# MIMUW-RL/space-gym

Measured on AMD Instinct MI355X. Metric: env-steps/sec at batch=65536, GoalContinuous3P-v0, 1/2/4/8 MI355X, higher is better.
Workload: dtype f32

## Files before the change

space_gym_amd/csrc/sg_device.hpp:

```cpp
#ifndef SG_DEVICE_HPP
#define SG_DEVICE_HPP

#include <math.h>
#include <stdint.h>

#include "sg_config.h"

#if defined(__HIPCC__)
#define SG_FN __device__ __forceinline__
#define SG_MFN __device__ __forceinline__
#else
#define SG_FN static inline
#define SG_MFN inline
#endif

#ifndef SG_STAMP
#define SG_STAMP(slot)
#endif

namespace sg {

#if defined(__HIP_DEVICE_COMPILE__)
SG_FN float rsq(float x) { return __builtin_amdgcn_rsqf(x); }
SG_FN float rcp(float x) { return __builtin_amdgcn_rcpf(x); }
SG_FN float fsqrt(float x) { return __builtin_amdgcn_sqrtf(x); }
SG_FN float flog2(float x) { return __builtin_amdgcn_logf(x); }
SG_FN float fexp2(float x) { return __builtin_amdgcn_exp2f(x); }
#else
SG_FN float rsq(float x) { return 1.0f / sqrtf(x); }
SG_FN float rcp(float x) { return 1.0f / x; }
SG_FN float fsqrt(float x) { return sqrtf(x); }
SG_FN float flog2(float x) { return log2f(x); }
SG_FN float fexp2(float x) { return exp2f(x); }
#endif

constexpr float kTwoPi = 6.283185307179586f;

SG_FN void sincos_poly(float r, float &s, float &c) {
    float z = r * r;
    float ps = fmaf(fmaf(-1.9515295891e-4f, z, 8.3321608736e-3f), z, -1.6666654611e-1f);
    s = fmaf(ps * z, r, r);
    float pc = fmaf(fmaf(2.443315711809948e-5f, z, -1.388731625493765e-3f), z, 4.166664568298827e-2f);
    c = fmaf(pc * z, z, fmaf(-0.5f, z, 1.0f));
}

SG_FN void sincos_small(float r, float &s, float &c) {
    float z = r * r;
    s = fmaf(r * z, fmaf(z, 8.295134641230106e-3f, -1.666649580001831e-1f), r);
    c = fmaf(z, fmaf(z, fmaf(z, -1.3838880180093369e-3f, 4.166642666449376e-2f), -0.5f), 1.0f);
}

#if defined(__HIP_DEVICE_COMPILE__)
typedef float f2 __attribute__((ext_vector_type(2)));
SG_FN f2 mk2(float a, float b) { f2 r; r.x = a; r.y = b; return r; }
SG_FN f2 fma2(f2 a, f2 b, f2 c) { return __builtin_elementwise_fma(a, b, c); }
#else
struct f2 { float x, y; };
SG_FN f2 mk2(float a, float b) { f2 r; r.x = a; r.y = b; return r; }
SG_FN f2 operator+(f2 a, f2 b) { return mk2(a.x + b.x, a.y + b.y); }
SG_FN f2 operator-(f2 a, f2 b) { return mk2(a.x - b.x, a.y - b.y); }
SG_FN f2 operator*(f2 a, f2 b) { return mk2(a.x * b.x, a.y * b.y); }
SG_FN f2 operator*(f2 a, float b) { return mk2(a.x * b, a.y * b); }
SG_FN f2 operator*(float a, f2 b) { return mk2(a * b.x, a * b.y); }
SG_FN f2 fma2(f2 a, f2 b, f2 c) { return mk2(fmaf(a.x, b.x, c.x), fmaf(a.y, b.y, c.y)); }
#endif
SG_FN f2 sp2(float a) { return mk2(a, a); }
SG_FN f2 fma2(float a, f2 b, f2 c) { return fma2(sp2(a), b, c); }
SG_FN f2 fma2(f2 a, float b, f2 c) { return fma2(a, sp2(b), c); }
SG_FN f2 fma2(f2 a, float b, float c) { return fma2(a, sp2(b), sp2(c)); }
SG_FN f2 fma2(f2 a, f2 b, float c) { return fma2(a, b, sp2(c)); }

SG_FN void sincos_small2(f2 r, f2 &s, f2 &c) {
    f2 z = r * r;
    s = fma2(r * z, fma2(z, 8.295134641230106e-3f, -1.666649580001831e-1f), r);
    c = fma2(z, fma2(z, fma2(z, -1.3838880180093369e-3f, 4.166642666449376e-2f), -0.5f), 1.0f);
}

SG_FN void sincos_acc(float a, float &s, float &c) {
    float k = rintf(a * 0.6366197723675814f);
    float r = fmaf(-k, 1.57079637050628662109375f, a);
    r = fmaf(-k, -4.37113900018624283e-8f, r);
    float sr, cr;
    sincos_poly(r, sr, cr);
    int q = (int)k & 3;
    float s1 = (q & 1) ? cr : sr, c1 = (q & 1) ? sr : cr;
    s = (q & 2) ? -s1 : s1;
    c = ((q + 1) & 2) ? -c1 : c1;
}

SG_FN float wrap_two_pi(float th) {
    th = th - kTwoPi * floorf(th * (1.0f / kTwoPi));
    th = (th < 0.0f) ? th + kTwoPi : th;
    return (th >= kTwoPi) ? th - kTwoPi : th;
}

SG_FN double rsqrt_f64(double x) {
    double y = (double)rsq((float)x);
    return y * (1.5 - 0.5 * x * y * y);
}

constexpr float C2 = 1.0f / 5, C3 = 3.0f / 10, C4 = 4.0f / 5, C5 = 8.0f / 9;
constexpr float A21 = 1.0f / 5;
constexpr float A31 = 3.0f / 40, A32 = 9.0f / 40;
constexpr float A41 = 44.0f / 45, A42 = -56.0f / 15, A43 = 32.0f / 9;
constexpr float A51 = 19372.0f / 6561, A52 = -25360.0f / 2187, A53 = 64448.0f / 6561, A54 = -212.0f / 729;
constexpr float A61 = 9017.0f / 3168, A62 = -355.0f / 33, A63 = 46732.0f / 5247, A64 = 49.0f / 176,
                A65 = -5103.0f / 18656;
constexpr float B1 = 35.0f / 384, B3 = 500.0f / 1113, B4 = 125.0f / 192, B5 = -2187.0f / 6784, B6 = 11.0f / 84;
constexpr float BETA1 = 35.0f / 384, BETA3 = 50.0f / 159, BETA4 = 25.0f / 192, BETA5 = -243.0f / 6784;
constexpr float E3 = 71.0f / 16695, E4 = -71.0f / 1920, E5 = 17253.0f / 339200, E6 = -22.0f / 525, E7 = 1.0f / 40;
constexpr float P31 = (float)(131558114200.0 / 32700410799.0), P32 = (float)(-68118460800.0 / 10900136933.0),
                P33 = (float)(87487479700.0 / 32700410799.0);
constexpr float P41 = (float)(-1754552775.0 / 470086768.0), P42 = (float)(14199869525.0 / 1410260304.0),
                P43 = (float)(-10690763975.0 / 1880347072.0);
constexpr float P51 = (float)(127303824393.0 / 49829197408.0), P52 = (float)(-318862633887.0 / 49829197408.0),
                P53 = (float)(701980252875.0 / 199316789632.0);
constexpr float P61 = (float)(-282668133.0 / 205662961.0), P62 = (float)(2019193451.0 / 616988883.0),
                P63 = (float)(-1453857185.0 / 822651844.0);
constexpr float P71 = (float)(40617522.0 / 29380423.0), P72 = (float)(-110615467.0 / 29380423.0),
                P73 = (float)(69997945.0 / 29380423.0);
constexpr float kRtol = 1e-3f, kAtol = 1e-6f;
constexpr float kSafety = 0.9f, kMinFactor = 0.2f, kMaxFactor = 10.0f;
#ifndef SG_PROBE_NORM
#define SG_PROBE_NORM 1e-3f
#endif
constexpr float kProbeNorm = SG_PROBE_NORM;
#ifndef SG_PROBE_POS_ERR
#define SG_PROBE_POS_ERR 2e-8f
#endif
constexpr float kProbePosErr = SG_PROBE_POS_ERR;
#ifndef SG_PROBE_POS_ERR_KEPLER
#define SG_PROBE_POS_ERR_KEPLER 1e-6f
#endif
constexpr float kProbePosErrKepler = SG_PROBE_POS_ERR_KEPLER;
constexpr float N5_C2 = 1.0f / 5, N5_C3 = 2.0f / 3;
constexpr float N5_A21 = 1.0f / 50, N5_A31 = -1.0f / 27, N5_A32 = 7.0f / 27;
constexpr float N5_BB1 = 14.0f / 336, N5_BB2 = 100.0f / 336, N5_BB3 = 54.0f / 336;
constexpr float N5_B1 = 14.0f / 336, N5_B2 = 125.0f / 336, N5_B3 = 162.0f / 336, N5_B4 = 35.0f / 336;
constexpr float N5_D1 = (float)(3.0 / 10 - 14.0 / 336), N5_D2 = (float)(-2.0 / 35 - 100.0 / 336), N5_D3 = (float)(9.0 / 35 - 54.0 / 336);
#ifndef SG_FAST_IND
#define SG_FAST_IND 1.5e-6f
#endif
constexpr float kFastInd = SG_FAST_IND;
#ifndef SG_FAST_IND_KEPLER
#define SG_FAST_IND_KEPLER 1e-5f
#endif
constexpr float kFastIndKepler = SG_FAST_IND_KEPLER;
#ifndef SG_FAST_IND_CROSS
#define SG_FAST_IND_CROSS 3e-5f
#endif
constexpr float kFastIndCross = SG_FAST_IND_CROSS;
constexpr float kFastCrossDepth = 1e-5f;
constexpr int kMaxRkAttempts = 12;
constexpr int kRootIters = 2;
constexpr int kRootMaxIters = 28;

struct StepResult {
    double dXd, dYd;
    float dX, dY;
    float vx, vy;
    float t;
    float dth, om;
    int done;
    int event;
    int n_rk;
    int path;
    float probe_err;
    float probe_ep, probe_ev;
};
enum : int { kPathProbe = 0, kPathProbeTerminal = 1, kPathScipyErr = 2, kPathScipyClear = 3, kPathScipy = 4 };

template <bool SMALL>
SG_FN f2 thrust_at(f2 T, f2 Tp, float delta) {
    float sd, cd;
    if (SMALL) sincos_small(delta, sd, cd); else sincos_poly(delta, sd, cd);
    return fma2(T, sp2(cd), Tp * sd);
}
template <int NG>
SG_FN f2 pull(f2 c0, f2 c1, f2 c2, f2 c3, f2 p, float (&r2)[NG > 0 ? NG : 1]) {
    static_assert(NG <= 4, "at most four gravitating circles");
    f2 s = mk2(0.0f, 0.0f);
    if (NG >= 2) {
        const f2 da = c0 - p, db = c1 - p;
        const float ra = fmaf(da.x, da.x, da.y * da.y), rb = fmaf(db.x, db.x, db.y * db.y);
        r2[0] = ra; r2[NG >= 2 ? 1 : 0] = rb;
        const f2 i = mk2(rsq(ra), rsq(rb));
        const f2 w = i * i * i;
        s = fma2(db, sp2(w.y), da * w.x);
    }
    if (NG == 4) {
        const f2 da = c2 - p, db = c3 - p;
        const float ra = fmaf(da.x, da.x, da.y * da.y), rb = fmaf(db.x, db.x, db.y * db.y);
        r2[NG == 4 ? 2 : 0] = ra; r2[NG == 4 ? 3 : 0] = rb;
        const f2 i = mk2(rsq(ra), rsq(rb));
        const f2 w = i * i * i;
        s = fma2(db, sp2(w.y), fma2(da, sp2(w.x), s));
    }
    if (NG & 1) {
        const f2 dc = (NG == 1 ? c0 : c2) - p;
        const float rc = fmaf(dc.x, dc.x, dc.y * dc.y), ic = rsq(rc);
        r2[NG - 1] = rc;
        const float w = ic * ic * ic;
        s = (NG == 1) ? dc * w : fma2(dc, sp2(w), s);
    }
    return s;
}

enum : int { kRkContinue = 0, kRkFinished = 1, kRkEvent = 2, kRkEventDeferred = 3 };

template <int NC, int NG, bool WALLS, bool ACCEL = false>
struct Integrator {
    float t_end, half_world, gm, F, om, alpha, w_limit, x0, y0, nCF, nSF;
    float cax[NC], cay[NC], cR[NC], cR2[NC];
    f2 cq0, cq1, cq2, cq3;
    SG_MFN f2 cq_at(int k) const { return k == 0 ? cq0 : k == 1 ? cq1 : k == 2 ? cq2 : cq3; }
    double cRd[NC];
    float wxp, wyp, wxm, wym;
    float t, X, Y, vx, vy, h_abs;
    double Xd, Yd;
    float k0[4], g[NC + 2];
    f2 gp0;
    bool rejected, probe;
    bool fast;
    bool probe_crossing;
    float th0;
    int n_rk, attempts, path;
    float probe_err, probe_ep, probe_ev;

    struct EventCase {
        float h, t, X, Y, vx, vy, Xn, Yn;
        double Xd, Yd;
        float k0[4], k2[4], k3[4], k4[4], k5[4], k6[4];
        unsigned mask;
        float s_w;
        int n_rk;
        static constexpr int kWords = 8 + 4 + 24 + 3;
    };

    SG_MFN float phase(float tt) const { return ACCEL ? fmaf(om, tt, 0.5f * alpha * tt * tt) : om * tt; }

    SG_MFN void set_constants(float h_total, float half_world_, float gm_, float F_, float om_, float alpha_, float w_limit_,
                              float x0_, float y0_, const float (&cax_)[NC], const float (&cay_)[NC], const float (&cR_)[NC],
                              const double (&cRd_)[NC]) {
        half_world = half_world_; gm = gm_; F = F_; om = om_; alpha = ACCEL ? alpha_ : 0.0f; w_limit = w_limit_;
        x0 = x0_; y0 = y0_;
#pragma unroll
        for (int k = 0; k < NC; k++) { cax[k] = cax_[k]; cay[k] = cay_[k]; cR[k] = cR_[k]; cR2[k] = cR_[k] * cR_[k]; cRd[k] = cRd_[k]; }
        t_end = h_total;
        {
            float rx[4] = {0.0f, 0.0f, 0.0f, 0.0f}, ry[4] = {0.0f, 0.0f, 0.0f, 0.0f};
#pragma unroll
            for (int k = 0; k < NC; k++) {
                rx[k] = cax_[k]; ry[k] = cay_[k];
#if defined(__HIP_DEVICE_COMPILE__)
                asm volatile("" : "+v"(rx[k]), "+v"(ry[k]));
#endif
            }
            const f2 o = mk2(x0, y0);
            cq0 = mk2(rx[0], ry[0]) - o; cq1 = mk2(rx[1], ry[1]) - o; cq2 = mk2(rx[2], ry[2]) - o; cq3 = mk2(rx[3], ry[3]) - o;
        }
        wxp = half_world - x0; wyp = half_world - y0; wxm = half_world + x0; wym = half_world + y0;
    }

    SG_MFN void begin(float h_total, float half_world_, float gm_, float F_, float om_, float alpha_, float w_limit_,
                      float x0_, float y0_, float th0_, float vx0, float vy0, const float (&cax_)[NC],
                      const float (&cay_)[NC], const float (&cR_)[NC], const double (&cRd_)[NC], bool use_probe = true) {
        SG_STAMP(8);
        set_constants(h_total, half_world_, gm_, F_, om_, alpha_, w_limit_, x0_, y0_, cax_, cay_, cR_, cRd_);
        {
            float S0, C0;
            sincos_acc(th0_, S0, C0);
            nCF = -(C0 * F); nSF = -(S0 * F);
        }
        t = 0.0f; X = 0.0f; Y = 0.0f; vx = vx0; vy = vy0;
        Xd = 0.0; Yd = 0.0;
        const f2 T = mk2(nCF, nSF);

        float r2s[NG > 0 ? NG : 1];
        f2 origin = mk2(0.0f, 0.0f);
#if defined(__HIP_DEVICE_COMPILE__)
        asm volatile("" : "+v"(origin));
#endif
        gp0 = pull<NG>(cq0, cq1, cq2, cq3, origin, r2s);
        const f2 a0 = fma2(gm, gp0, T);
        k0[0] = vx; k0[1] = vy; k0[2] = a0.x; k0[3] = a0.y;
        th0 = th0_;
        probe = kProbeNorm > 0.0f && use_probe;
        fast = !ACCEL && probe;
        probe_crossing = false;
        path = kPathScipy; probe_err = probe_ep = probe_ev = 0.0f;
        if (probe) h_abs = t_end; else initial_step();

        SG_STAMP(9);
    #pragma unroll
        for (int k = 0; k < NG; k++) g[k] = r2s[k] - cR2[k];
    #pragma unroll
        for (int k = NG; k < NC; k++) { const f2 c = cq_at(k); g[k] = fmaf(c.x, c.x, c.y * c.y) - cR2[k]; }
        if (WALLS) { g[NC] = fminf(wxp, wyp); g[NC + 1] = fminf(wxm, wym); }

        rejected = false; n_rk = 0; attempts = 0;
    }

    SG_MFN void initial_step() {
        const f2 T = mk2(nCF, nSF), Tp = mk2(-nSF, nCF), V = mk2(k0[0], k0[1]), a0 = mk2(k0[2], k0[3]);
        const f2 is_p = mk2(rcp(fmaf(fabsf(x0), kRtol, kAtol)), rcp(fmaf(fabsf(y0), kRtol, kAtol)));
        const f2 is_v = mk2(rcp(fmaf(fabsf(V.x), kRtol, kAtol)), rcp(fmaf(fabsf(V.y), kRtol, kAtol)));
        const float isth = rcp(fmaf(fabsf(th0), kRtol, kAtol)), isom = rcp(fmaf(fabsf(om), kRtol, kAtol));
        const f2 y_p = mk2(x0, y0) * is_p, y_v = V * is_v;
        const float y_th = th0 * isth, y_om = om * isom;
        const f2 n0 = fma2(y_v, y_v, y_p * y_p);
        const float d0 = fsqrt(fmaf(y_om, y_om, fmaf(y_th, y_th, n0.x + n0.y)) * (1.0f / 6));
        const f2 f_p = V * is_p, f_v = a0 * is_v;
        const float f_th = om * isth, f_om = ACCEL ? alpha * isom : 0.0f;
        const f2 n1 = fma2(f_v, f_v, f_p * f_p);
        const float d1 = fsqrt(fmaf(f_om, f_om, fmaf(f_th, f_th, n1.x + n1.y)) * (1.0f / 6));
        float h0 = (fminf(d0, d1) < 1e-5f) ? 1e-6f : 0.01f * d0 * rcp(d1);
        h0 = fminf(h0, t_end);
        float r2p[NG > 0 ? NG : 1];
        const f2 a1 = fma2(gm, pull<NG>(cq0, cq1, cq2, cq3, V * h0, r2p), thrust_at<!ACCEL>(T, Tp, h0 * om));
        const f2 e_p = (a0 * h0) * is_p, e_v = (a1 - a0) * is_v;
        const float e_th = ACCEL ? h0 * alpha * isth : 0.0f;
        const f2 n2 = fma2(e_v, e_v, e_p * e_p);
        const float d2 = fsqrt(fmaf(e_th, e_th, n2.x + n2.y) * (1.0f / 6)) * rcp(h0);
        const float dm = fmaxf(d1, d2);
        const float h1 = (dm <= 1e-15f) ? fmaxf(1e-6f, h0 * 1e-3f)
                                        : fexp2(0.2f * flog2(0.01f * rcp(dm)));
        h_abs = fminf(fminf(100.0f * h0, h1), t_end);
    }

    SG_MFN bool no_graze(f2 V, f2 Vn, f2 Pn, float h, const float (&gn)[NC + 2]) const {
        const f2 vv0 = V * V, vv1 = Vn * Vn;
        const float v2max = fmaxf(vv0.x + vv0.y, vv1.x + vv1.y);
        const float ah = 1.2f * h * (F + 1.1f), chord = 0.3f * h * h * v2max;
        bool keep = true;
#pragma unroll
        for (int k = 0; k < NC; k++) {
            const f2 c = cq_at(k), cn = c - Pn;
            const float d0 = fmaf(c.x, V.x, c.y * V.y), d1 = fmaf(cn.x, Vn.x, cn.y * Vn.y);
            const bool mono = d0 * d1 > 0.0f && fabsf(d0 + d1) > fmaf(ah, cR[k], 1.2f * h * v2max);
            const float clear = fmaf(0.25f * h * ah, cR[k], g[k] > 0.0f ? chord : 0.0f);
            const bool near = fminf(fabsf(g[k]), fabsf(gn[k])) <= clear;
            keep = keep && !(near && !mono);
        }
        if (WALLS) {
            const f2 s = V + Vn;
            const float clear = 0.125f * h * ah;
            const bool mono_x = V.x * Vn.x > 0.0f && fabsf(s.x) > ah, mono_y = V.y * Vn.y > 0.0f && fabsf(s.y) > ah;
            const bool near_x = fminf(fminf(wxp, wxp - Pn.x), fminf(wxm, wxm + Pn.x)) <= clear;
            const bool near_y = fminf(fminf(wyp, wyp - Pn.y), fminf(wym, wym + Pn.y)) <= clear;
            keep = keep && !(near_x && !mono_x) && !(near_y && !mono_y);
        }
        return keep;
    }

    SG_MFN void nystrom5(float h, f2 P0, f2 V, f2 T, f2 Tp, f2 g1, f2 &rest, f2 &Vn, f2 &w) const {
        const float hh = h * h, hg = hh * gm;
        const float ph = om * h, z4 = ph * ph;
        const f2 ph23 = mk2(N5_C2, N5_C3) * ph, z23 = ph23 * ph23;
        const f2 A23 = fma2(z23, fma2(z23, 1.0f / 720, -1.0f / 24), 0.5f);
        const f2 B23 = ph23 * fma2(z23, fma2(z23, 1.0f / 5040, -1.0f / 120), 1.0f / 6);
        const float A4 = fmaf(z4, fmaf(z4, 1.0f / 720, -1.0f / 24), 0.5f);
        const float B4 = ph * fmaf(z4, fmaf(z4, 1.0f / 5040, -1.0f / 120), 1.0f / 6);
        const float S4 = fmaf(z4, fmaf(z4, fmaf(z4, -1.0f / 5040, 1.0f / 120), -1.0f / 6), 1.0f);
        const f2 p2 = fma2(T, sp2(A23.x), Tp * B23.x), p3 = fma2(T, sp2(A23.y), Tp * B23.y), p4 = fma2(T, sp2(A4), Tp * B4);
        float r2x[NG > 0 ? NG : 1];
        const f2 g2 = pull<NG>(cq0, cq1, cq2, cq3, fma2(hg * N5_A21, g1, fma2((N5_C2 * N5_C2) * hh, p2, fma2(N5_C2 * h, V, P0))), r2x);
        const f2 g3 = pull<NG>(cq0, cq1, cq2, cq3,
                               fma2(hg, fma2(N5_A32, g2, g1 * N5_A31), fma2((N5_C3 * N5_C3) * hh, p3, fma2(N5_C3 * h, V, P0))), r2x);
        rest = fma2(hg, fma2(N5_BB3, g3, fma2(N5_BB2, g2, g1 * N5_BB1)), p4 * hh);
        w = fma2(N5_D3, g3, fma2(N5_D2, g2, g1 * N5_D1)) * hg;
        const f2 g4 = pull<NG>(cq0, cq1, cq2, cq3, fma2(h, V, P0) + (rest + w), r2x);
        Vn = fma2(h * gm, fma2(N5_B4, g4, fma2(N5_B3, g3, fma2(N5_B2, g2, g1 * N5_B1))),
                  fma2(h, fma2(T, sp2(S4), Tp * (ph * A4)), V));
    }

    template <typename SINK>
    SG_MFN int fast_step(StepResult &o, SINK &&sink) {
        const float h = t_end;
        const f2 V = mk2(vx, vy), T = mk2(nCF, nSF), Tp = mk2(-nSF, nCF);
        f2 rest, Vn, w;
        f2 origin = mk2(0.0f, 0.0f);
#if defined(__HIP_DEVICE_COMPILE__)
        asm volatile("" : "+v"(origin));
#endif
        nystrom5(h, origin, V, T, Tp, gp0, rest, Vn, w);
        double Xdn = (double)h * (double)vx + (double)rest.x, Ydn = (double)h * (double)vy + (double)rest.y;
        float Xn = (float)Xdn, Yn = (float)Ydn;
        float ind2 = fmaf(w.x, w.x, w.y * w.y);

        float gn[NC + 2], ggmin, shallow;
        auto end_events = [&]() __attribute__((always_inline)) {
#pragma unroll
            for (int k = 0; k < NC; k++) {
                const f2 c = cq_at(k);
                const float ex = c.x - Xn, ey = c.y - Yn;
                gn[k] = fmaf(ex, ex, ey * ey) - cR2[k];
            }
            gn[NC] = gn[NC + 1] = 1.0f;
            if (WALLS) { gn[NC] = fminf(wxp - Xn, wyp - Yn); gn[NC + 1] = fminf(wxm + Xn, wym + Yn); }
            ggmin = 1.0f; shallow = 3.0e38f;
#pragma unroll
            for (int k = 0; k < NC + (WALLS ? 2 : 0); k++) {
                const float gg = g[k] * gn[k];
                ggmin = fminf(ggmin, gg);
                shallow = fminf(shallow, gg <= 0.0f ? fabsf(gn[k]) : 3.0e38f);
            }
        };
        end_events();
        const float lim = WALLS ? kFastInd : kFastIndKepler;
        probe_ev = 1.0f;
        if (!(ggmin <= 0.0f) && !(ind2 <= lim * lim)) {
            probe_ev = 2.0f;
            const float hs = 0.5f * h;
            f2 rA, VA, wA, rB, wB;
            nystrom5(hs, origin, V, T, Tp, gp0, rA, VA, wA);
            const double XdA = (double)hs * (double)vx + (double)rA.x, YdA = (double)hs * (double)vy + (double)rA.y;
            const f2 PA = mk2((float)XdA, (float)YdA);
            float sd, cd;
            sincos_small(om * hs, sd, cd);
            const f2 T1 = fma2(T, sp2(cd), Tp * sd), Tp1 = mk2(-T1.y, T1.x);
            float r2a[NG > 0 ? NG : 1];
            const f2 gA = pull<NG>(cq0, cq1, cq2, cq3, PA, r2a);
            nystrom5(hs, PA, VA, T1, Tp1, gA, rB, Vn, wB);
            Xdn = XdA + ((double)hs * (double)VA.x + (double)rB.x); Ydn = YdA + ((double)hs * (double)VA.y + (double)rB.y);
            Xn = (float)Xdn; Yn = (float)Ydn;
            ind2 = 16.0f * fmaxf(fmaf(wA.x, wA.x, wA.y * wA.y), fmaf(wB.x, wB.x, wB.y * wB.y));
            w = mk2(fmaxf(fabsf(wA.x), fabsf(wB.x)), fmaxf(fabsf(wA.y), fabsf(wB.y))) * 4.0f;
            end_events();
        }
        probe_err = ind2; probe_ep = fmaxf(fabsf(w.x), fabsf(w.y));

        const bool crossing = ggmin <= 0.0f;
        probe = false;
        if (!crossing) {
            if (!(ind2 <= lim * lim)) {
                path = kPathScipyErr;
                initial_step();
                return kRkContinue;
            }
            if (no_graze(V, Vn, mk2(Xn, Yn), h, gn)) {
                n_rk = 1; path = kPathProbe;
                t = t_end; X = Xn; Y = Yn; Xd = Xdn; Yd = Ydn; vx = Vn.x; vy = Vn.y;
                return kRkFinished;
            }
            path = kPathScipyClear;
        } else if (ind2 <= kFastIndCross * kFastIndCross && shallow >= kFastCrossDepth) {
            probe_crossing = true; path = kPathProbeTerminal;
            if (sink()) {
                o.dXd = 0.0; o.dYd = 0.0; o.dX = 0.0f; o.dY = 0.0f; o.vx = 0.0f; o.vy = 0.0f; o.t = t_end; o.dth = 0.0f; o.om = om;
                o.done = 1; o.event = -1; o.n_rk = 0; o.path = path;
                return kRkEventDeferred;
            }
        } else {
            path = kPathScipyErr;
        }
        initial_step();
        return kRkContinue;
    }

    struct NoSink { SG_MFN bool operator()() const { return false; } };
    template <typename SINK = NoSink>
    SG_MFN int attempt(StepResult &o, SINK &&sink = NoSink()) {
        const bool probing = probe;
        probe = false;
        attempts++;
        h_abs = fmaxf(h_abs, 1e-9f);
        float t_new = t + h_abs;
        if (t_new - t_end > 0.0f) t_new = t_end;
        const float h = t_new - t;
        h_abs = h;
        const f2 V = mk2(vx, vy), P = mk2(X, Y), a0 = mk2(k0[2], k0[3]);
        f2 th1, th2, th3, th4, th5;
        {
            const f2 T = mk2(nCF, nSF), Tp = mk2(-nSF, nCF);
            if (ACCEL) {
                th1 = thrust_at<false>(T, Tp, phase(fmaf(C2, h, t))); th2 = thrust_at<false>(T, Tp, phase(fmaf(C3, h, t)));
                th3 = thrust_at<false>(T, Tp, phase(fmaf(C4, h, t))); th4 = thrust_at<false>(T, Tp, phase(fmaf(C5, h, t)));
                th5 = thrust_at<false>(T, Tp, phase(t + h));
            } else {
                const float ph0 = om * t, phh = om * h;
                f2 s12, c12, s34, c34;
                sincos_small2(fma2(mk2(C2, C3), phh, ph0), s12, c12);
                sincos_small2(fma2(mk2(C4, C5), phh, ph0), s34, c34);
                th1 = fma2(T, sp2(c12.x), Tp * s12.x); th2 = fma2(T, sp2(c12.y), Tp * s12.y);
                th3 = fma2(T, sp2(c34.x), Tp * s34.x); th4 = fma2(T, sp2(c34.y), Tp * s34.y);
                th5 = thrust_at<true>(T, Tp, ph0 + phh);
            }
        }
        float r2x[NG > 0 ? NG : 1], r2n[NG > 0 ? NG : 1];
        const f2 sa1 = a0 * A21;
        const f2 v1 = fma2(h, sa1, V);
        const f2 g1 = pull<NG>(cq0, cq1, cq2, cq3, fma2(h, V * A21, P), r2x);
        const f2 g2 = pull<NG>(cq0, cq1, cq2, cq3, fma2(h, fma2(A32, v1, V * A31), P), r2x);
        const f2 a1 = fma2(gm, g1, th1), a2 = fma2(gm, g2, th2);
        const f2 sa2 = fma2(A32, a1, a0 * A31);
        const f2 v2 = fma2(h, sa2, V);
        const f2 sa3 = fma2(A43, a2, fma2(A42, a1, a0 * A41));
        const f2 v3 = fma2(h, sa3, V);
        const f2 g3 = pull<NG>(cq0, cq1, cq2, cq3, fma2(h, fma2(A43, v2, fma2(A42, v1, V * A41)), P), r2x);
        const f2 g4 = pull<NG>(cq0, cq1, cq2, cq3, fma2(h, fma2(A54, v3, fma2(A53, v2, fma2(A52, v1, V * A51))), P), r2x);
        const f2 a3 = fma2(gm, g3, th3), a4 = fma2(gm, g4, th4);
        const f2 sa4 = fma2(A54, a3, fma2(A53, a2, fma2(A52, a1, a0 * A51)));
        const f2 v4 = fma2(h, sa4, V);
        const f2 sa5 = fma2(A65, a4, fma2(A64, a3, fma2(A63, a2, fma2(A62, a1, a0 * A61))));
        const f2 v5 = fma2(h, sa5, V);
        const f2 nys = fma2(BETA5, a4, fma2(BETA4, a3, fma2(BETA3, a2, a0 * BETA1))) * (h * h);
        const double Xdn = Xd + ((double)h * (double)vx + (double)nys.x);
        const double Ydn = Yd + ((double)h * (double)vy + (double)nys.y);
        const float Xn = (float)Xdn, Yn = (float)Ydn;
        const f2 Pn = mk2(Xn, Yn);
        const f2 g5 = pull<NG>(cq0, cq1, cq2, cq3, fma2(h, fma2(A65, v4, fma2(A64, v3, fma2(A63, v2, fma2(A62, v1, V * A61)))), P), r2x);
        const f2 g6 = pull<NG>(cq0, cq1, cq2, cq3, Pn, r2n);
        const f2 a5 = fma2(gm, g5, th5), a6 = fma2(gm, g6, th5);
        const f2 sa6 = fma2(B6, a5, fma2(B5, a4, fma2(B4, a3, fma2(B3, a2, a0 * B1))));
        const f2 v6 = fma2(h, sa6, V);
        const float vxn = v6.x, vyn = v6.y;

        float err2, abs_ep, abs_ev;
        {
            const f2 e_p = fma2(E7, sa6, fma2(E6, sa5, fma2(E5, sa4, fma2(E4, sa3, sa2 * E3)))) * h;
            const f2 e_v = fma2(E7, a6 - a0, fma2(E6, a5 - a0, fma2(E5, a4 - a0, fma2(E4, a3 - a0, (a2 - a0) * E3))));
            const f2 p0 = mk2(x0, y0) + P, p1 = mk2(x0, y0) + Pn;
            const f2 sc_p = fma2(mk2(fmaxf(fabsf(p0.x), fabsf(p1.x)), fmaxf(fabsf(p0.y), fabsf(p1.y))), kRtol, kAtol);
            const f2 sc_v = fma2(mk2(fmaxf(fabsf(vx), fabsf(vxn)), fmaxf(fabsf(vy), fabsf(vyn))), kRtol, kAtol);
            const f2 q_p = (e_p * h) * mk2(rcp(sc_p.x), rcp(sc_p.y)), q_v = (e_v * h) * mk2(rcp(sc_v.x), rcp(sc_v.y));
            const f2 n = fma2(q_v, q_v, q_p * q_p);
            err2 = n.x + n.y;
            abs_ep = fmaxf(fabsf(e_p.x), fabsf(e_p.y)) * h; abs_ev = fmaxf(fabsf(e_v.x), fabsf(e_v.y)) * h;
        }
        const float err = err2 * (1.0f / 6);

        float gn[NC + 2], gg[NC + 2], ggmin = 1.0f;
        auto end_events = [&]() __attribute__((always_inline)) {
#pragma unroll
            for (int k = 0; k < NG; k++) gn[k] = r2n[k] - cR2[k];
#pragma unroll
            for (int k = NG; k < NC; k++) {
                const f2 c = cq_at(k);
                float ex = c.x - Xn, ey = c.y - Yn;
                gn[k] = fmaf(ex, ex, ey * ey) - cR2[k];
            }
            if (WALLS) { gn[NC] = fminf(wxp - Xn, wyp - Yn); gn[NC + 1] = fminf(wxm + Xn, wym + Yn); }
#pragma unroll
            for (int k = 0; k < NC + (WALLS ? 2 : 0); k++) { gg[k] = g[k] * gn[k]; ggmin = fminf(ggmin, gg[k]); }
        };
        end_events();
        float s_w = 2.0f;
        bool w_event = false;
        if constexpr (ACCEL) {
            const float w0 = fmaf(alpha, t, om), w1 = fmaf(alpha, t_new, om);
            const float gw0 = w_limit - fabsf(w0), gw1 = w_limit - fabsf(w1);
            if ((gw0 <= 0.0f && gw1 >= 0.0f) || (gw0 >= 0.0f && gw1 <= 0.0f)) {
                const float lim = (fabsf(w1) >= fabsf(w0) ? w1 : w0) >= 0.0f ? w_limit : -w_limit;
                const float dw = w1 - w0;
                s_w = (dw != 0.0f) ? fminf(fmaxf((lim - w0) * rcp(dw), 0.0f), 1.0f) : 0.0f;
                w_event = true;
            }
        }

        if (probing) {
            probe_err = err; probe_ep = abs_ep; probe_ev = abs_ev;
            const bool small = err <= kProbeNorm * kProbeNorm && abs_ep <= (WALLS ? kProbePosErr : kProbePosErrKepler);
            const bool crossing = ggmin <= 0.0f || w_event;
            if (small && !crossing) {
                if (no_graze(V, v6, Pn, h, gn)) {
                    n_rk = 1; path = kPathProbe;
                    t = t_new; X = Xn; Y = Yn; Xd = Xdn; Yd = Ydn; vx = vxn; vy = vyn;
                    return kRkFinished;
                }
                path = kPathScipyClear;
            } else if (small) {
                probe_crossing = true; path = kPathProbeTerminal;
                if (sink()) {
                    o.dXd = 0.0; o.dYd = 0.0; o.dX = 0.0f; o.dY = 0.0f; o.vx = 0.0f; o.vy = 0.0f; o.t = t_end; o.dth = 0.0f; o.om = om;
                    o.done = 1; o.event = -1; o.n_rk = 0; o.path = path;
                    return kRkEventDeferred;
// ... 285 lines not shown
    double ir = rsqrt_f64(rx * rx + py_ * py_);
    double v2 = c.k_gm * (2.0 * ir - ob.inv_a);
    double speed = v2 > 0 ? v2 * rsqrt_f64(v2) : 0.0;
    double it = rsqrt_f64(tx * tx + ty * ty);
    double ux = tx * it * speed, uy = ty * it * speed;
    double Vx = ob.cosphi * ux - ob.sinphi * uy, Vy = ob.sinphi * ux + ob.cosphi * uy;
    double rad_pen = fabs(cur_rad - target_rad);
    double vxp = fabs(Vx - (double)vx), vyp = fabs(Vy - (double)vy);
    float act = c.k_Ca * fsqrt(fmaf(engine, engine, thruster * thruster));
    return (float)(c.k_C / (c.k_Cr * rad_pen + vxp + vyp + (double)act + c.k_C));
}

SG_FN Orbit make_orbit(double a, double ecc, double cosphi, double sinphi) {
    Orbit ob;
    ob.a = a; ob.ecc = ecc; ob.cosphi = cosphi; ob.sinphi = sinphi;
    double b2 = a * a * (1.0 - ecc * ecc);
    ob.b = b2 * rsqrt_f64(b2);
    double c2 = a * a - b2;
    ob.c = c2 > 0 ? c2 * rsqrt_f64(c2) : 0.0;
    ob.a_over_b = a / ob.b; ob.b_over_a = ob.b / a; ob.inv_a = 1.0 / a;
    return ob;
}

SG_FN uint32_t mulhi32(uint32_t a, uint32_t b) {
#if defined(__HIP_DEVICE_COMPILE__)
    return __umulhi(a, b);
#else
    return (uint32_t)(((uint64_t)a * b) >> 32);
#endif
}

SG_FN void philox4x32_10(uint32_t k0, uint32_t k1, uint32_t c0, uint32_t c1, uint32_t c2, uint32_t c3, uint32_t (&out)[4]) {
#pragma unroll
    for (int r = 0; r < 10; r++) {
        uint32_t h0 = mulhi32(0xD2511F53u, c0), l0 = 0xD2511F53u * c0;
        uint32_t h1 = mulhi32(0xCD9E8D57u, c2), l1 = 0xCD9E8D57u * c2;
        c0 = h1 ^ c1 ^ k0; c1 = l1;
        c2 = h0 ^ c3 ^ k1; c3 = l0;
        k0 += 0x9E3779B9u; k1 += 0xBB67AE85u;
    }
    out[0] = c0; out[1] = c1; out[2] = c2; out[3] = c3;
}

constexpr uint32_t kStreamReset = 0u, kStreamGoal = 1u, kStreamAction = 2u;

constexpr int kGoalResetBlocks = 5, kKeplerResetBlocks = 3;

SG_FN float u23(uint32_t w) { return ((float)(w >> 9) + 0.5f) * (1.0f / 8388608.0f); }
SG_FN float u16(uint32_t h) { return ((float)(h & 0xffffu) + 0.5f) * (1.0f / 65536.0f); }
SG_FN uint32_t below16(uint32_t h, uint32_t n) { return ((h & 0xffffu) * n) >> 16; }

struct Tiling {
    uint32_t episode, goal_draws;
    uint32_t ship_tile, goal_tile, case_b, flip;
    uint64_t free_counts;
    float cs0, cs1, cs2, cs3;
};

SG_FN uint32_t free_total(uint64_t f) {
    uint64_t s = (f & 0x0f0f0f0f0f0f0f0full) + ((f >> 4) & 0x0f0f0f0f0f0f0f0full);
    return (uint32_t)((s * 0x0101010101010101ull) >> 56);
}
struct FreePrefix { uint64_t even, odd; };
SG_FN FreePrefix free_prefix(uint64_t f) {
    const uint64_t e = f & 0x0f0f0f0f0f0f0f0full, o = (f >> 4) & 0x0f0f0f0f0f0f0f0full;
    const uint64_t pe = e * 0x0101010101010101ull, po = o * 0x0101010101010101ull;
    FreePrefix p;
    p.even = pe + (po << 8);
    p.odd = pe + po;
    return p;
}
SG_FN uint32_t bytes_above(uint64_t x, uint32_t pos) {
    const uint64_t H = 0x8080808080808080ull, L = 0x0101010101010101ull;
    const uint64_t low_gt = (((x & ~H) + (uint64_t)(127u - (pos & 127u)) * L) & H);
    const uint64_t hi = x & H;
    const uint64_t gt = (pos < 128u) ? (hi | low_gt) : (hi & low_gt);
#if defined(__HIP_DEVICE_COMPILE__)
    return (uint32_t)__popcll(gt);
#else
    return (uint32_t)__builtin_popcountll(gt);
#endif
}
SG_FN uint32_t free_at(const FreePrefix &p, uint32_t pos) { return 16u - bytes_above(p.even, pos) - bytes_above(p.odd, pos); }
SG_FN uint64_t free_add(uint64_t f, uint32_t tile) {
    uint32_t cnt = (uint32_t)(f >> (4 * tile)) & 15u;
    return cnt < 15u ? f + (1ull << (4 * tile)) : f;
}
SG_FN uint64_t free_remove(uint64_t f, uint32_t tile) { return f - (1ull << (4 * tile)); }

SG_FN void tile_center(const SgDev &c, const Tiling &T, uint32_t tile, float &x, float &y) {
    uint32_t row = (tile * c.t_cols_rcp16) >> 16, col = tile - row * (uint32_t)c.t_cols;
    const float shift = (col == 1u) ? T.cs1 : (col == 2u) ? T.cs2 : (col == 3u) ? T.cs3 : T.cs0;
    float tx = c.t_x0 + (float)col * 1.5f * c.t_a + shift;
    float y0 = T.case_b ? c.t_y0 - 0.5f * c.t_hex_h : c.t_y0;
    float ycol = (col & 1u) ? 0.5f * c.t_hex_h : 0.0f;
    float ty = y0 - (float)row * c.t_hex_h + (T.case_b ? ycol : -ycol);
    x = T.flip ? ty : tx;
    y = T.flip ? tx : ty;
}

SG_FN void disc_in_tile(const SgDev &c, const Tiling &T, uint32_t tile, float noise_radius, uint32_t w, float &x, float &y) {
    float s, co;
    sincos_acc(kTwoPi * u16(w >> 16), s, co);
    float r = noise_radius * fsqrt(u16(w));
    tile_center(c, T, tile, x, y);
    x = fmaf(r, co, x);
    y = fmaf(r, s, y);
}

SG_FN void choose_goal_tile(const SgDev &c, Tiling &T, bool first, const uint32_t (&w)[4]) {
    if (!first) {
        T.free_counts = free_add(T.free_counts, T.ship_tile);
        T.ship_tile = T.goal_tile;
    }
    if ((w[0] & 0xffu) < 64u) {
        T.goal_tile = T.ship_tile;
    } else {
        const uint32_t n = free_total(T.free_counts), n_cand = n < 3u ? n : 3u;
        const uint32_t cols = (uint32_t)c.t_cols, sr = (T.ship_tile * c.t_cols_rcp16) >> 16, sc = T.ship_tile - sr * cols;
        const uint32_t draws[3] = {w[1] >> 16, w[1], w[2] >> 16};
        uint32_t chosen[3] = {0u, 0u, 0u};
        const uint32_t j0 = below16(draws[0], n);
        chosen[0] = j0;
        const uint32_t v1_old = (j0 == 1u) ? 0u : 1u;
        uint32_t j1 = 0xffffffffu;
        if (n_cand > 1) {
            j1 = 1u + below16(draws[1], n - 1u);
            chosen[1] = (j1 == j0) ? 0u : j1;
        }
        if (n_cand > 2) {
            const uint32_t j2 = 2u + below16(draws[2], n - 2u);
            chosen[2] = (j2 == j1) ? v1_old : (j2 == j0) ? 0u : j2;
        }
        uint32_t best_tile = 0;
        int best_dist = -1;
        const FreePrefix fp = free_prefix(T.free_counts);
#pragma unroll
        for (uint32_t i = 0; i < 3; i++) {
            if (i < n_cand) {
                uint32_t tile = free_at(fp, chosen[i]);
                uint32_t r = (tile * c.t_cols_rcp16) >> 16, cc = tile - r * cols;
                int dist = abs((int)r - (int)sr) + abs((int)cc - (int)sc);
                if (dist > best_dist) { best_dist = dist; best_tile = tile; }
            }
        }
        T.goal_tile = best_tile;
        T.free_counts = free_remove(T.free_counts, best_tile);
    }
}

SG_FN void choose_goal(const SgDev &c, Tiling &T, bool first, const uint32_t (&w)[4], float &gx, float &gy) {
    choose_goal_tile(c, T, first, w);
    disc_in_tile(c, T, T.goal_tile, c.noise_goal, w[3], gx, gy);
}

SG_FN void box_muller(uint32_t w1, uint32_t w2, float &z0, float &z1) {
    float r = fsqrt(-2.0f * 0.6931471805599453f * flog2(u23(w1)));
    float s, co;
    sincos_acc(kTwoPi * u23(w2), s, co);
    z0 = r * co;
    z1 = r * s;
}

struct ShipInit { float x, y, th, vx, vy, om; };

SG_FN void layout_from_words(const SgDev &c, uint32_t flags, uint32_t c01, uint32_t c23, Tiling &T) {
    T.case_b = flags & 1u; T.flip = (flags >> 1) & 1u;
    const float a0 = u16(c01 >> 16), a1 = a0 + u16(c01);
    const float a2 = (c.t_cols > 2) ? a1 + u16(c23 >> 16) : a1, a3 = (c.t_cols > 3) ? a2 + u16(c23) : a2;
    const float k = c.t_free_x * rcp(a3);
    T.cs0 = a0 * k; T.cs1 = a1 * k;
    T.cs2 = (c.t_cols > 2) ? a2 * k : 0.0f; T.cs3 = (c.t_cols > 3) ? a3 * k : 0.0f;
}

template <int N>
SG_FN void tiles_from_words(const SgDev &c, uint32_t flags, uint32_t t01, uint32_t t23, uint32_t t45, Tiling &T,
                            uint32_t (&tiles)[N + 1]) {
    const uint32_t draws[6] = {t01 >> 16, t01, t23 >> 16, t23, t45 >> 16, t45};
    uint64_t perm = 0xfedcba9876543210ull;
    const uint32_t nt = (uint32_t)c.t_tiles;
#pragma unroll
    for (uint32_t i = 0; i <= (uint32_t)N; i++) {
        uint32_t j = i + below16(draws[i], nt - i);
        uint64_t vi = (perm >> (4 * i)) & 15ull, vj = (perm >> (4 * j)) & 15ull;
        perm = (perm & ~((15ull << (4 * i)) | (15ull << (4 * j)))) | (vj << (4 * i)) | (vi << (4 * j));
        tiles[i] = (uint32_t)vj;
    }
    if (N == 2 && ((flags >> 8) & 0xffu) < 64u) {
        const uint32_t d = (flags >> 16) & 3u;
        tiles[0] = (d == 0) ? 1u : (d == 1) ? 2u : (d == 2) ? 0u : 3u;
        tiles[1] = (d < 2) ? 0u : 1u;
        tiles[2] = (d < 2) ? 3u : 2u;
    }
    uint64_t used = 0;
#pragma unroll
    for (int i = 0; i <= N; i++) used |= 1ull << (4 * tiles[i]);
    const uint64_t all = (nt >= 16u) ? 0x1111111111111111ull : (0x1111111111111111ull & ((1ull << (4 * nt)) - 1ull));
    T.free_counts = all & ~used;
    T.ship_tile = tiles[0];
}

SG_FN void kinematics_from_words(const SgDev &c, uint32_t wth, uint32_t b0, uint32_t b1, uint32_t b2, uint32_t b3, ShipInit &s) {
    s.th = kTwoPi * u23(wth);
    float z0, z1, z2, z3;
    box_muller(b0, b1, z0, z1);
    box_muller(b2, b3, z2, z3);
    s.vx = z0 * c.vel_std; s.vy = z1 * c.vel_std;
    s.om = fminf(fmaxf(z2 * c.omega_std, -c.omega_max), c.omega_max);
}

template <int N>
SG_FN void goal_reset(const SgDev &c, uint32_t env_global, Tiling &T, ShipInit &s, float (&px)[N], float (&py)[N],
                      float &gx, float &gy) {
    uint32_t w[4 * kGoalResetBlocks];
#pragma unroll
    for (uint32_t b = 0; b < (uint32_t)kGoalResetBlocks; b++) {
        uint32_t o[4];
        philox4x32_10(c.seed_lo, c.seed_hi, env_global, T.episode, b, kStreamReset, o);
        w[4 * b] = o[0]; w[4 * b + 1] = o[1]; w[4 * b + 2] = o[2]; w[4 * b + 3] = o[3];
    }
    T.goal_draws = 0;
    const uint32_t flags = w[0];
    layout_from_words(c, flags, w[1], w[2], T);
    uint32_t tiles[N + 1];
    tiles_from_words<N>(c, flags, w[3], w[4], w[5], T, tiles);
    disc_in_tile(c, T, tiles[0], c.noise_ship, w[8], s.x, s.y);
#pragma unroll
    for (int j = 0; j < N; j++) disc_in_tile(c, T, tiles[j + 1], c.noise_planet, w[9 + j], px[j], py[j]);
    const uint32_t gw[4] = {flags >> 24, w[6], w[7], w[13]};
    T.goal_tile = 0xffu;
    choose_goal(c, T, true, gw, gx, gy);
    kinematics_from_words(c, w[14], w[16], w[17], w[18], w[19], s);
}

SG_FN void goal_resample(const SgDev &c, uint32_t env_global, Tiling &T, float &gx, float &gy) {
    uint32_t w[4];
    T.goal_draws += 1;
    philox4x32_10(c.seed_lo, c.seed_hi, env_global, T.episode, T.goal_draws, kStreamGoal, w);
    choose_goal(c, T, false, w, gx, gy);
}

SG_FN void kepler_reset(const SgDev &c, uint32_t env_global, uint32_t episode, ShipInit &s, float &phi, float &ecc) {
    uint32_t w[4 * kKeplerResetBlocks];
#pragma unroll
    for (uint32_t b = 0; b < (uint32_t)kKeplerResetBlocks; b++) {
        uint32_t o[4];
        philox4x32_10(c.seed_lo, c.seed_hi, env_global, episode, b, kStreamReset, o);
        w[4 * b] = o[0]; w[4 * b + 1] = o[1]; w[4 * b + 2] = o[2]; w[4 * b + 3] = o[3];
    }
    float sa, ca;
    sincos_acc(kTwoPi * u23(w[0]), sa, ca);
    float dist = fmaf(c.kep_rmax - c.kep_rmin, u23(w[1]), c.kep_rmin);
    s.x = ca * dist; s.y = sa * dist;
    if (c.randomize_orbit) { ecc = u23(w[3]) * 0.7f; phi = u23(w[4]) * kTwoPi; }
    kinematics_from_words(c, w[2], w[8], w[9], w[10], w[11], s);
}

SG_FN void random_action_words(uint32_t seed_lo, uint32_t seed_hi, uint32_t env_global, uint64_t step, uint32_t &w0, uint32_t &w1) {
    uint32_t o[4];
    const uint64_t p = step >> 1;
    philox4x32_10(seed_lo, seed_hi, env_global, (uint32_t)p, (uint32_t)(p >> 32), kStreamAction, o);
    w0 = (step & 1u) ? o[2] : o[0];
    w1 = (step & 1u) ? o[3] : o[1];
}

template <int N>
struct GoalEnv {
    float x, y, th, vx, vy, om;
    float gx, gy;
    float px[N], py[N];
};
struct KeplerEnv {
    float x, y, th, vx, vy, om;
    float phi, ecc;
};

SG_FN void translate_action(float &a0, float &a1, float max_engine_force, float &engine, float &F, float &om) {
    a0 = fminf(fmaxf(a0, -1.0f), 1.0f);
    a1 = fminf(fmaxf(a1, -1.0f), 1.0f);
    engine = (a0 + 1.0f) * 0.5f;
    F = engine * max_engine_force;
    om = a1 * 5.0f;
}

template <bool ACCEL>
SG_FN void steering(const SgDev &c, float a1, float om_cmd, float om_state, float &om0, float &alpha) {
    if (ACCEL && c.steering_acceleration) { om0 = om_state; alpha = (a1 * c.max_thruster_force) * c.inv_moi; }
    else { om0 = om_cmd; alpha = 0.0f; }
}

SG_FN void load_action(bool discrete, const void *actions, int64_t idx, float &a0, float &a1) {
    if (discrete) {
        const int k = static_cast<const int32_t *>(actions)[idx];
        const bool engine = (k == 1) | (k == 4) | (k == 5);
        a0 = engine ? 1.0f : -1.0f;
        a1 = (k == 2 || k == 4) ? -1.0f : (k == 3 || k == 5) ? 1.0f : 0.0f;
    } else {
        const float *p = static_cast<const float *>(actions) + 2 * idx;
        a0 = p[0]; a1 = p[1];
    }
}

template <int N, typename CFG>
SG_FN void goal_observe(const CFG &c, const GoalEnv<N> &e, float (&obs)[7 + 2 * N + 2]) {
    float s, co;
    sincos_acc(e.th, s, co);
    obs[0] = e.x; obs[1] = e.y; obs[2] = co; obs[3] = s; obs[4] = e.vx; obs[5] = e.vy; obs[6] = e.om;
#pragma unroll
    for (int j = 0; j < N; j++) lidar(e.px[j] - e.x, e.py[j] - e.y, c.planet_r, c.two_over_world, obs[7 + 2 * j], obs[8 + 2 * j]);
    obs[7 + 2 * N] = (e.gx - e.x) * c.two_over_world;
    obs[8 + 2 * N] = (e.gy - e.y) * c.two_over_world;
}

template <typename CFG>
SG_FN void kepler_observe(const CFG &c, const KeplerEnv &e, float (&obs)[10]) {
    float s, co;
    sincos_acc(e.th, s, co);
    obs[0] = e.x; obs[1] = e.y; obs[2] = co; obs[3] = s; obs[4] = e.vx; obs[5] = e.vy; obs[6] = e.om;
    obs[7] = c.randomize_orbit ? e.phi : (float)c.k_phi;
    obs[8] = c.randomize_orbit ? e.ecc : (float)c.k_ecc;
    obs[9] = (float)c.k_a;
}

template <int N, bool ACCEL = false>
SG_FN void goal_env_begin(const SgDev &c, const GoalEnv<N> &e, float a0, float a1, Integrator<N, N, true, ACCEL> &I,
                          bool use_probe = true) {
    float engine, F, om, om0, alpha;
    translate_action(a0, a1, c.max_engine_force, engine, F, om);
    steering<ACCEL>(c, a1, om, e.om, om0, alpha);
    float cR[N];
    double cRd[N];
#pragma unroll
    for (int j = 0; j < N; j++) { cR[j] = c.planet_r; cRd[j] = c.planet_r_d; }
    I.begin(c.h, c.half_world, c.gm, F, om0, alpha, c.omega_limit, e.x, e.y, e.th, e.vx, e.vy, e.px, e.py, cR, cRd, use_probe);
}

struct GoalStepConsts {
    double goal_r2, danger_r2, survival, goal_scale, safety_scale, sparse;
    float planet_r, two_over_world;
};
SG_FN GoalStepConsts goal_step_consts(const SgDev &c) {
    GoalStepConsts k;
    k.goal_r2 = c.goal_r2; k.danger_r2 = c.danger_r2; k.survival = c.survival; k.goal_scale = c.goal_scale;
    k.safety_scale = c.safety_scale; k.sparse = c.sparse; k.planet_r = c.planet_r; k.two_over_world = c.two_over_world;
    return k;
}

struct KeplerStepConsts {
    double k_gm, k_C, k_Cr, k_phi, k_ecc, k_a;
    float k_Ca;
    int32_t randomize_orbit;
};
SG_FN KeplerStepConsts kepler_step_consts(const SgDev &c) {
    KeplerStepConsts k;
    k.k_gm = c.k_gm; k.k_C = c.k_C; k.k_Cr = c.k_Cr; k.k_phi = c.k_phi; k.k_ecc = c.k_ecc; k.k_a = c.k_a; k.k_Ca = c.k_Ca;
    k.randomize_orbit = c.randomize_orbit;
    return k;
}

struct GoalRewardProfile {
    double danger_r2, survival, goal_scale, safety_scale, sparse;
};
struct KeplerRewardProfile {
    double k_C, k_Cr;
    float k_Ca;
};
struct GoalRewardView {
    double goal_r2, danger_r2, survival, goal_scale, safety_scale, sparse;
};
SG_FN GoalRewardView goal_reward_view(const SgDev &c, const GoalRewardProfile &p) {
    GoalRewardView v;
    v.goal_r2 = c.goal_r2; v.danger_r2 = p.danger_r2; v.survival = p.survival; v.goal_scale = p.goal_scale;
    v.safety_scale = p.safety_scale; v.sparse = p.sparse;
    return v;
}
struct KeplerRewardView {
    double k_gm, k_C, k_Cr;
    float k_Ca;
};
SG_FN KeplerRewardView kepler_reward_view(const SgDev &c, const KeplerRewardProfile &p) {
    KeplerRewardView v;
    v.k_gm = c.k_gm; v.k_C = p.k_C; v.k_Cr = p.k_Cr; v.k_Ca = p.k_Ca;
    return v;
}

struct StepConsts {
    float max_engine_force, h, half_world, gm, omega_limit, planet_r, max_thruster_force, inv_moi;
    double planet_r_d;
    int32_t steering_acceleration;
};
SG_FN StepConsts step_consts(const SgDev &c) {
    StepConsts k;
    k.max_engine_force = c.max_engine_force; k.h = c.h; k.half_world = c.half_world; k.gm = c.gm; k.omega_limit = c.omega_limit;
    k.planet_r = c.planet_r; k.max_thruster_force = c.max_thruster_force; k.inv_moi = c.inv_moi; k.planet_r_d = c.planet_r_d;
    k.steering_acceleration = c.steering_acceleration;
    return k;
}
template <int N, bool ACCEL = false>
SG_FN void goal_env_begin(const StepConsts &k, const GoalEnv<N> &e, float a0, float a1, Integrator<N, N, true, ACCEL> &I,
                          bool use_probe = true) {
    float engine, F, om, om0, alpha;
    translate_action(a0, a1, k.max_engine_force, engine, F, om);
    if (ACCEL && k.steering_acceleration) { om0 = e.om; alpha = (a1 * k.max_thruster_force) * k.inv_moi; }
    else { om0 = om; alpha = 0.0f; }
    float cR[N];
    double cRd[N];
#pragma unroll
    for (int j = 0; j < N; j++) { cR[j] = k.planet_r; cRd[j] = k.planet_r_d; }
    I.begin(k.h, k.half_world, k.gm, F, om0, alpha, k.omega_limit, e.x, e.y, e.th, e.vx, e.vy, e.px, e.py, cR, cRd, use_probe);
}

template <int N, typename RC>
SG_FN void goal_env_finish_r(const SgDev &c, const RC &rc, GoalEnv<N> &e, const StepResult &r, float (&obs)[7 + 2 * N + 2],
                             float &reward, int &done, int &hit) {
    SG_STAMP(11);
    reward = goal_reward<N>(rc, e.x, e.y, r.dXd, r.dYd, e.px, e.py, e.gx, e.gy, hit);
    SG_STAMP(12);
    e.x = (float)((double)e.x + r.dXd); e.y = (float)((double)e.y + r.dYd); e.vx = r.vx; e.vy = r.vy; e.om = r.om;
    e.th = wrap_two_pi(e.th + r.dth);
    done = r.done;
    goal_observe<N>(c, e, obs);
}
template <int N>
SG_FN void goal_env_finish(const SgDev &c, GoalEnv<N> &e, const StepResult &r, float (&obs)[7 + 2 * N + 2],
                           float &reward, int &done, int &hit) {
    SG_STAMP(11);
    reward = goal_reward<N>(c, e.x, e.y, r.dXd, r.dYd, e.px, e.py, e.gx, e.gy, hit);
    SG_STAMP(12);
    e.x = (float)((double)e.x + r.dXd); e.y = (float)((double)e.y + r.dYd); e.vx = r.vx; e.vy = r.vy; e.om = r.om;
    e.th = wrap_two_pi(e.th + r.dth);
    done = r.done;
    goal_observe<N>(c, e, obs);
}

template <int N, bool ACCEL = false>
SG_FN void goal_env_step(const SgDev &c, GoalEnv<N> &e, float a0, float a1, float (&obs)[7 + 2 * N + 2], float &reward,
                         int &done, int &hit, StepResult &r) {
    Integrator<N, N, true, ACCEL> I;
    goal_env_begin<N, ACCEL>(c, e, a0, a1, I);
    I.run(r);
    goal_env_finish<N>(c, e, r, obs, reward, done, hit);
}

template <int NC, int NG, bool ACCEL>
SG_FN void vector_field(const SgDev &c, float x, float y, float th, float vx, float vy, float om_state, float a0, float a1,
                        const float (&cax)[NC], const float (&cay)[NC], float (&f)[6]) {
    float engine, F, om, om0, alpha, S0, C0;
    static_assert(NC <= 4, "at most four circles");
    translate_action(a0, a1, c.max_engine_force, engine, F, om);
    steering<ACCEL>(c, a1, om, om_state, om0, alpha);
    sincos_acc(th, S0, C0);
    const f2 o = mk2(x, y);
    const f2 cq0 = mk2(cax[0], cay[0]) - o, cq1 = mk2(cax[NC > 1 ? 1 : 0], cay[NC > 1 ? 1 : 0]) - o,
             cq2 = mk2(cax[NC > 2 ? 2 : 0], cay[NC > 2 ? 2 : 0]) - o, cq3 = mk2(cax[NC > 3 ? 3 : 0], cay[NC > 3 ? 3 : 0]) - o;
    f[0] = vx; f[1] = vy; f[2] = om0; f[5] = alpha;
    float r2[NG > 0 ? NG : 1];
    const f2 a = fma2(c.gm, pull<NG>(cq0, cq1, cq2, cq3, mk2(0.0f, 0.0f), r2), mk2(-(C0 * F), -(S0 * F)));
    f[3] = a.x; f[4] = a.y;
}

SG_FN Orbit fixed_orbit(const SgDev &c) {
    Orbit ob;
    ob.a = c.k_a; ob.b = c.k_b; ob.c = c.k_c; ob.ecc = c.k_ecc; ob.cosphi = c.k_cos; ob.sinphi = c.k_sin;
    ob.a_over_b = c.k_a / c.k_b; ob.b_over_a = c.k_b / c.k_a; ob.inv_a = 1.0 / c.k_a;
    return ob;
}

template <bool ACCEL, typename RC>
SG_FN void kepler_env_step_r(const SgDev &c, const RC &rc, const Orbit &ob, KeplerEnv &e, float a0, float a1, float (&obs)[10],
                             float &reward, int &done, StepResult &r, bool use_probe) {
    float engine, F, om, om0, alpha;
    translate_action(a0, a1, c.max_engine_force, engine, F, om);
    steering<ACCEL>(c, a1, om, e.om, om0, alpha);
    const float cax[2] = {0.0f, 0.0f}, cay[2] = {0.0f, 0.0f}, cR[2] = {c.planet_r, c.border_r};
    const double cRd[2] = {c.planet_r_d, (double)c.border_r};
    make_step<2, 1, false, ACCEL>(c.h, c.half_world, c.gm, F, om0, alpha, c.omega_limit, e.x, e.y, e.th, e.vx, e.vy, cax, cay,
                                  cR, cRd, r, use_probe);
    reward = kepler_reward(rc, ob, e.x, e.y, r.dXd, r.dYd, r.vx, r.vy, engine, a1);
    e.x = (float)((double)e.x + r.dXd); e.y = (float)((double)e.y + r.dYd); e.vx = r.vx; e.vy = r.vy; e.om = r.om;
    e.th = wrap_two_pi(e.th + r.dth);
    done = r.done;
    kepler_observe(c, e, obs);
}
template <bool ACCEL = false>
SG_FN void kepler_env_step(const SgDev &c, const Orbit &ob, KeplerEnv &e, float a0, float a1, float (&obs)[10],
                           float &reward, int &done, StepResult &r, bool use_probe = true) {
    kepler_env_step_r<ACCEL>(c, c, ob, e, a0, a1, obs, reward, done, r, use_probe);
}

}
#endif
```

space_gym_amd/csrc/sg_engine.hip:

```cpp
#include <hip/hip_runtime.h>
#include <hip/hip_ext.h>

#include <algorithm>
#include <cmath>
#include <cstdarg>
#include <cstdio>
#include <cstdlib>
#include <cstring>
#include <limits>
#include <new>
#include <string>
#include <tuple>
#include <type_traits>
#include <utility>
#include <vector>

#include "../../include/spacegym.h"

#ifdef SG_STAMPS
constexpr int kStampSlots = 16, kStampWaves = 4096;
__device__ unsigned long long sg_dbg_stamps[kStampSlots * kStampWaves];
#ifdef SG_STAMPS_ACC_ONLY
#define SG_STAMP(slot)
#else
// ... 464 lines not shown
            SG_PASS(0);
#endif
            __builtin_amdgcn_fence(__ATOMIC_SEQ_CST, "wavefront");
            drain(true);
            sub += stride;
            if (sub < sub_end) load_inputs(sub);
            SG_STAMP(1);
            SG_PASS(1);
            StepResult sr = {};
            const int rk = F::first(c, e_cur, a_cur, sr);
            SG_STAMP(2);
            SG_PASS(2);
            const bool deferred = live && rk != kRkFinished;
            const bool full = deferred && (rk != kRkEventDeferred || !auto_reset);
            const bool kept = live && !deferred;
            {
                const uint32_t s = w_rec.slot(deferred, wave);
                if (deferred) Rec::put(rec, s, (uint32_t)i | (full ? kRecFull : 0u) | (rk == kRkEventDeferred ? kRecTerminal : 0u), e_cur, a_cur, ct_cur);
            }
            const int hit = fam.finish(c, b, i, e_cur, a_cur, sr, kept, pend.o, pend.r);
            SG_STAMP(15);
            SG_PASS(3);
            const uint32_t el = ct_cur.x + 1u;
            const int trunc = kept && (int)el >= max_steps;
            const bool known = deferred && !full;
            const bool restart = known || (trunc && auto_reset);
            pend.i = i;
            pend.what = (kept ? 1u : 0u) | (kept && !restart ? 2u : 0u) | (kept || known ? 4u : 0u) | (trunc ? 8u : 0u) |
                        (i - lane + 64 <= num_envs ? 16u : 0u);
            pend.x = e_cur.x; pend.y = e_cur.y; pend.th = e_cur.th; pend.vx = e_cur.vx; pend.vy = e_cur.vy; pend.om = e_cur.om;
            const float2 hi = F::q1_hi(e_cur);
            pend.z = hi.x; pend.w = hi.y;
            pend.el = el; pend.episode = ct_cur.y;
            pend.fin = (uint8_t)(known | trunc); pend.trunc = (uint8_t)trunc;
            {
                const bool resample = kept && hit && !restart;
                const uint32_t s0 = w_rs0.slot(restart, wave);
                uint32_t s1 = 0u;
                if constexpr (F::kResample) s1 = w_sm0.slot(resample, wave);
                if (restart) { L.env[0][s0] = (uint32_t)i; L.episode[0][s0] = ct_cur.y; }
                if (resample) { L.env[1][s1] = (uint32_t)i; L.episode[1][s1] = ct_cur.y; }
            }
            SG_STAMP(3);
            SG_PASS(4);
            continue;
        }
        drain(!more);
        __builtin_amdgcn_fence(__ATOMIC_SEQ_CST, "wavefront");
        const bool pooled = !more;
        if (pooled) {
            if (lane == 0) {
                L.n[0][wave] = w_rec.n; L.n[1][wave] = w_rs0.n;
                if constexpr (F::kResample) L.n[2][wave] = w_sm0.n;
            }
            __syncthreads();
        }
        SG_STAMP(4);
        SG_STAMP_VAL(11, w_rec.n | (w_rs0.n << 16) | ((unsigned long long)w_sm0.n << 32));
        const int role = (wave + (int)blockIdx.x) & 3;
        const uint32_t step = pooled ? kBlock : 64u;
        const uint32_t first_rec = pooled ? (uint32_t)role * 64u : 0u, first_rs = pooled ? (uint32_t)((role + 3) & 3) * 64u : 0u,
                       first_sm = pooled ? (uint32_t)((role + 2) & 3) * 64u : 0u;
#pragma unroll 1
        for (int round = 0; round < 2; round++) {
            if (round == 0) {
                const Pool P = Pool::of(L.n[0], pooled, wave, w_rec.n);
#pragma unroll 1
                for (uint32_t lo = first_rec; lo < P.total; lo += step) {
                    const bool have = lo + (uint32_t)lane < P.total;
                    uint32_t ef;
                    Env e2;
                    float2 a2;
                    uint2 ct2;
                    Rec::get(rec, P.slot(lo + (have ? (uint32_t)lane : 0u)), ef, e2, a2, ct2);
                    const int env = (int)(ef & kRecEnvMask);
                    const bool full2 = (ef & kRecFull) != 0u;
                    float o2[D], rw;
                    int dn2;
                    const int hit2 = fam.replay(c, b, env, e2, a2, (ef & kRecTerminal) != 0u, have, o2, rw, dn2);
                    const uint32_t el = ct2.x + 1u;
                    const int trunc = !dn2 && (int)el >= max_steps;
                    const int fin = dn2 | trunc;
                    const bool restart = have && full2 && fin && auto_reset;
                    if (have) {
                        reward[env] = rw;
                        if (fin && terminal_obs) store_row(terminal_obs, env, o2);
                        if (full2) {
                            if (!restart) {
                                b.q0[env] = make_float4(e2.x, e2.y, e2.th, e2.vx);
                                reinterpret_cast<float2 *>(b.q1 + env)[0] = make_float2(e2.vy, e2.om);
                                b.ctr[env] = make_uint2(el, ct2.y);
                                store_row(obs, env, o2);
                            }
                            done[env] = (uint8_t)fin;
                            truncated[env] = (uint8_t)trunc;
                        }
                    }
                    const bool resample = have && full2 && hit2 && !restart;
                    const uint32_t s0 = w_rs1.slot(restart, wave);
                    uint32_t s1 = 0u;
                    if constexpr (F::kResample) s1 = w_sm1.slot(resample, wave);
                    if (restart) { L.env[2][s0] = (uint32_t)env; L.episode[2][s0] = ct2.y; }
                    if (resample) { L.env[3][s1] = (uint32_t)env; L.episode[3][s1] = ct2.y; }
                }
                SG_STAMP(8);
            } else {
                if (pooled) {
                    if (lane == 0) {
                        L.n[3][wave] = w_rs1.n;
                        if constexpr (F::kResample) L.n[4][wave] = w_sm1.n;
                    }
                    __syncthreads();
                }
                if (!__any(pooled ? (L.n[3][lane & 3] | (F::kResample ? L.n[4][lane & 3] : 0u)) != 0u : (w_rs1.n | w_sm1.n) != 0u)) break;
            }
            const Pool Pr = Pool::of(L.n[1 + 2 * round], pooled, wave, round ? w_rs1.n : w_rs0.n);
#pragma unroll 1
            for (uint32_t lo = first_rs; lo < Pr.total; lo += step) {
                const uint32_t item = lo + (uint32_t)lane;
                if (item < Pr.total) {
                    const uint32_t sl = Pr.slot(item);
                    restart_env(fam, c, b, (int)L.env[2 * round][sl], L.episode[2 * round][sl] + 1u, obs);
                }
            }
            if (round == 0) { SG_STAMP(9); }
            if constexpr (F::kResample) {
                const Pool Ps = Pool::of(L.n[2 + 2 * round], pooled, wave, round ? w_sm1.n : w_sm0.n);
#pragma unroll 1
                for (uint32_t lo = first_sm; lo < Ps.total; lo += step) {
                    const uint32_t item = lo + (uint32_t)lane;
                    if (item < Ps.total) {
                        const uint32_t sl = Ps.slot(item);
                        F::resample(c, b, (int)L.env[2 * round + 1][sl], L.episode[2 * round + 1][sl]);
                    }
                }
            }
            if (round == 0) { SG_STAMP(10); }
        }
        if (pooled) break;
        w_rec.n = 0u; w_rs0.n = 0u; w_sm0.n = 0u; w_rs1.n = 0u; w_sm1.n = 0u;
    }
    SG_STAMP(5);
    SG_STAMP_REAL(7);
    SG_PASS_WRITE();
}

template <int N, bool ACCEL>
struct GoalStep {
    using Env = GoalEnv<N>;
    using Rec = StepRecord<N>;
    using Integ = Integrator<N, N, true, ACCEL>;
    static constexpr int D = 7 + 2 * N + 2;
    static constexpr int kPre = 320, kWordsAt = 256;
    static constexpr bool kResample = true;
    static constexpr bool kTouchParams = true, kFinishAction = false;
    __device__ __forceinline__ explicit GoalStep(const SgDev &) {}
    __device__ __forceinline__ void load(const SgBuffers &b, int jj, float4 *base) const {
        __builtin_amdgcn_global_load_lds((gbl_void *)(b.pl[0] + jj), (lds_void *)(base + 128), 16, 0, 0);
        if constexpr (N > 2) __builtin_amdgcn_global_load_lds((gbl_void *)(b.pl[1] + jj), (lds_void *)(base + 192), 16, 0, 0);
    }
    __device__ __forceinline__ void read(const float4 *blk, int lane, Env &e) const {
        const float4 q0 = blk[lane], q1 = blk[64 + lane], p0 = blk[128 + lane];
        float4 p1 = {};
        if constexpr (N > 2) p1 = blk[192 + lane];
        e.x = q0.x; e.y = q0.y; e.th = q0.z; e.vx = q0.w;
        e.vy = q1.x; e.om = q1.y; e.gx = q1.z; e.gy = q1.w;
        e.px[0] = p0.x; e.py[0] = p0.y; e.px[1] = p0.z; e.py[1] = p0.w;
        if constexpr (N > 2) { e.px[2] = p1.x; e.py[2] = p1.y; }
        if constexpr (N > 3) { e.px[3] = p1.z; e.py[3] = p1.w; }
    }
    __device__ __forceinline__ static float2 q1_hi(const Env &e) { return make_float2(e.gx, e.gy); }
    __device__ __forceinline__ static int first(const SgDev &c, const Env &e, float2 a, StepResult &sr) {
        Integ I;
        goal_env_begin<N, ACCEL>(c, e, a.x, a.y, I);
        return I.first(sr, []() __attribute__((always_inline)) -> bool { return true; });
    }
    __device__ __forceinline__ static void integrate(const SgDev &c, const Env &e, float2 a, StepResult &sr) {
        Integ I;
        goal_env_begin<N, ACCEL>(c, e, a.x, a.y, I);
        I.run(sr);
    }
    __device__ __forceinline__ static void load_env(const SgBuffers &b, int i, Env &e) { load_goal_env<N>(b, i, e); }
    struct Ready {};
    __device__ __forceinline__ Ready load_finisher(const SgDev &, const SgBuffers &, int, const Env &) const { return {}; }
    __device__ __forceinline__ int pair_finish(const SgDev &c, const SgBuffers &b, Ready, Env &e, float2 a, const PairHand &h, bool live,
                                               float (&o)[D], float &r) const {
        return pair_finish_r(c, c, b, Ready{}, e, a, h, live, o, r);
    }
    template <typename RC>
    __device__ __forceinline__ static int pair_finish_r(const SgDev &c, const RC &rc, const SgBuffers &b, Ready, Env &e, float2,
                                                        const PairHand &h, bool live, float (&o)[D], float &r) {
        int hit;
        r = goal_reward<N>(rc, e.x, e.y, h.dXd, h.dYd, e.px, e.py, e.gx, e.gy, hit);
        e.x = (float)((double)e.x + h.dXd); e.y = (float)((double)e.y + h.dYd);
        e.th = h.th; e.vx = h.vx; e.vy = h.vy; e.om = h.om;
        goal_observe<N>(c, e, o);
        count_hits(b.cnt, live && hit);
        return hit;
    }
    __device__ __forceinline__ int finish(const SgDev &c, const SgBuffers &b, int, Env &e, float2, const StepResult &sr, bool kept,
                                          float (&o)[D], float &r) const {
        int dn, hit;
        goal_env_finish<N>(c, e, sr, o, r, dn, hit);
        count_hits(b.cnt, kept && hit);
        return hit;
    }
    template <typename RC>
    __device__ __forceinline__ static int finish_r(const SgDev &c, const RC &rc, const SgBuffers &b, Env &e, float2, const StepResult &sr,
                                                   bool kept, float (&o)[D], float &r) {
        int dn, hit;
        goal_env_finish_r<N>(c, rc, e, sr, o, r, dn, hit);
        count_hits(b.cnt, kept && hit);
        return hit;
    }
    __device__ __forceinline__ int replay(const SgDev &c, const SgBuffers &b, int, Env &e, float2 a, bool terminal, bool have,
                                          float (&o)[D], float &r, int &dn) const {
        StepResult r2;
        {
            Integ I;
            goal_env_begin<N, ACCEL>(c, e, a.x, a.y, I, false);
            I.run(r2);
        }
        if (terminal) r2.done = 1;
        int hit;
        goal_env_finish<N>(c, e, r2, o, r, dn, hit);
        count_hits(b.cnt, have && hit);
        return hit;
    }
    template <typename RC>
    __device__ __forceinline__ static int replay_r(const SgDev &c, const RC &rc, const SgBuffers &b, Env &e, float2 a, bool terminal,
                                                   bool have, float (&o)[D], float &r, int &dn) {
        StepResult r2;
        {
            Integ I;
            goal_env_begin<N, ACCEL>(c, e, a.x, a.y, I, false);
            I.run(r2);
        }
        if (terminal) r2.done = 1;
        int hit;
        goal_env_finish_r<N>(c, rc, e, r2, o, r, dn, hit);
        count_hits(b.cnt, have && hit);
        return hit;
    }
    struct Next {
        Tiling T;
        ShipInit s;
        float px[N], py[N], gx, gy;
    };
    __device__ __forceinline__ static float2 kept_orbit(const SgBuffers &, int) { return make_float2(0.0f, 0.0f); }
    __device__ __forceinline__ static float2 reset_orbit(const SgDev &) { return make_float2(0.0f, 0.0f); }
    __device__ __forceinline__ static void next(const SgDev &c, int env, uint32_t episode, float2, Next &n) {
        n.T.episode = episode;
        goal_reset<N>(c, c.env_index_base + (uint32_t)env, n.T, n.s, n.px, n.py, n.gx, n.gy);
    }
    __device__ __forceinline__ void install(const SgDev &c, const SgBuffers &b, int env, uint32_t episode, const Next &n, Env &e,
                                            float (&o)[D]) const {
        e.x = n.s.x; e.y = n.s.y; e.th = n.s.th; e.vx = n.s.vx; e.vy = n.s.vy; e.om = n.s.om; e.gx = n.gx; e.gy = n.gy;
#pragma unroll
        for (int j = 0; j < N; j++) { e.px[j] = n.px[j]; e.py[j] = n.py[j]; }
        store_goal_ship<N>(b, env, e);
        store_goal_planets<N>(b, env, e);
        store_tiling(b, env, n.T);
        b.ctr[env] = make_uint2(0u, episode);
        goal_observe<N>(c, e, o);
    }
    __device__ __forceinline__ static void empty_queue(const SgBuffers &b, int env, uint32_t episode) { b.ephi[env] = episode; }
    __device__ __forceinline__ static void restart_group(const SgDev &c, const SgBuffers &b, int env, uint32_t episode, int sub,
                                                         float *obs, float2) {
        Env ne;
        goal_restart_group<N>(c, b, env, episode, sub, obs, ne);
    }
    __device__ __forceinline__ static void resample(const SgDev &c, const SgBuffers &b, int env, uint32_t episode) {
        Tiling T = load_tiling(b, env, episode);
        float gx, gy;
        goal_resample(c, c.env_index_base + (uint32_t)env, T, gx, gy);
        reinterpret_cast<float2 *>(b.q1 + env)[1] = make_float2(gx, gy);
        b.aux[env] = pack_aux(T);
    }
    __device__ __forceinline__ static void resample_wave(const SgDev &c, const SgBuffers &b, int i, bool want, uint32_t episode) {
        const unsigned long long need = __ballot(want);
        if (!need) return;
        const int lane = threadIdx.x & 63, grp = lane >> 3, sub = lane & (kGroup - 1);
        const int n_items = __popcll(need), wave_env0 = i - lane;
        for (int base = 0; base < n_items; base += 64 / kGroup) {
            const int item = base + grp;
            const int src = nth_set_lane(need, item < n_items ? item : 0);
            const uint32_t ep = __shfl(episode, src);
            if (item < n_items && sub == 0) resample(c, b, wave_env0 + src, ep);
        }
    }
};

template <int N, bool ACCEL>
__global__ __launch_bounds__(kBlock) void goal_step_kernel(const SgDev *__restrict__ cfg, SgBuffers b, int n_subtiles,
                                                          const void *__restrict__ actions, float *__restrict__ obs,
                                                          float *__restrict__ reward, uint8_t *__restrict__ done,
                                                          uint8_t *__restrict__ truncated, float *__restrict__ terminal_obs,
                                                          int stream_out) {
    step_subtiles<GoalStep<N, ACCEL>>(cfg, b, n_subtiles, actions, obs, reward, done, truncated, terminal_obs, stream_out);
}

template <int N>
struct SpareEpisode {
    static constexpr int kFields = 6 + 2 * N + 2 + 7;
    __device__ __forceinline__ static void put(float *base, int slot, int tid, const ShipInit &s, const float (&px)[N],
                                               const float (&py)[N], float gx, float gy, const Tiling &T) {
        float *p = base + (slot * kFields) * kBlock + tid;
        int f = 0;
        auto w = [&](float v) { p[(f++) * kBlock] = v; };
        w(s.x); w(s.y); w(s.th); w(s.vx); w(s.vy); w(s.om); w(gx); w(gy);
#pragma unroll
        for (int j = 0; j < N; j++) { w(px[j]); w(py[j]); }
        const uint4 a = pack_aux(T);
        w(__uint_as_float(a.y)); w(__uint_as_float(a.z)); w(__uint_as_float(a.w));
        w(T.cs0); w(T.cs1); w(T.cs2); w(T.cs3);
    }
    __device__ __forceinline__ static void put_record(float *base, int slot, int tid, const float4 (&r)[6]) {
        float *p = base + (slot * kFields) * kBlock + tid;
        int f = 0;
        auto w = [&](float v) { p[(f++) * kBlock] = v; };
        w(r[0].x); w(r[0].y); w(r[0].z); w(r[0].w); w(r[1].x); w(r[1].y); w(r[1].z); w(r[1].w);
        w(r[2].x); w(r[2].y); w(r[2].z); w(r[2].w);
        if constexpr (N > 2) { w(r[3].x); w(r[3].y); }
        if constexpr (N > 3) { w(r[3].z); w(r[3].w); }
        w(r[4].x); w(r[4].y); w(r[4].z);
        w(r[5].x); w(r[5].y); w(r[5].z); w(r[5].w);
    }
    __device__ __forceinline__ static void get(const float *base, int slot, int tid, GoalEnv<N> &e, uint4 &aux, float4 &cs) {
        const float *p = base + (slot * kFields) * kBlock + tid;
        int f = 0;
        auto r = [&]() { return p[(f++) * kBlock]; };
        e.x = r(); e.y = r(); e.th = r(); e.vx = r(); e.vy = r(); e.om = r(); e.gx = r(); e.gy = r();
#pragma unroll
        for (int j = 0; j < N; j++) { e.px[j] = r(); e.py[j] = r(); }
        aux.x = 0u;
        aux.y = __float_as_uint(r()); aux.z = __float_as_uint(r()); aux.w = __float_as_uint(r());
        cs.x = r(); cs.y = r(); cs.z = r(); cs.w = r();
    }
};

template <int N, bool ACCEL, int kSpare>
__global__ __launch_bounds__(kBlock) __attribute__((amdgpu_waves_per_eu(2))) void goal_rollout_kernel(const SgDev *__restrict__ cfg, SgBuffers b, int n_steps,
                                                             const void *__restrict__ actions, float *__restrict__ obs,
                                                             float *__restrict__ reward, uint8_t *__restrict__ done,
                                                             uint8_t *__restrict__ truncated, TermList tl) {
    __shared__ float spare[kSpare * SpareEpisode<N>::kFields * kBlock];
    const SgDev &c = *cfg;
    const bool discrete = c.discrete_actions != 0;
    constexpr int D = 7 + 2 * N + 2;
    const int i = blockIdx.x * kBlock + threadIdx.x, tid = threadIdx.x;
    const bool live = i < c.num_envs;
    const int ii = live ? i : 0;
    const int64_t B = c.num_envs;
    GoalEnv<N> e;
    load_goal_env<N>(b, ii, e);
    uint2 ct = b.ctr[ii];
    int n_spare = 0;
    auto refill = [&]() {
        if (n_spare < kSpare) {
            Tiling T;
            T.episode = ct.y + (uint32_t)n_spare + 1u;
            ShipInit s;
            float px[N], py[N], gx, gy;
            goal_reset<N>(c, c.env_index_base + (uint32_t)ii, T, s, px, py, gx, gy);
            SpareEpisode<N>::put(spare, (int)(T.episode % (uint32_t)kSpare), tid, s, px, py, gx, gy, T);
            n_spare++;
        }
    };
    uint4 aux = b.aux[ii];
    float4 cs = b.cshift[ii];
    float2 a_next = load_action_raw(discrete, actions, ii);
    for (int t = 0; t < n_steps; t++) {
        const float2 a = decode_action(discrete, a_next);
        if (t + 1 < n_steps) a_next = load_action_raw(discrete, actions, (int64_t)(t + 1) * B + ii);
        StepResult sr;
        {
            Integrator<N, N, true, ACCEL> I;
            goal_env_begin<N, ACCEL>(c, e, a.x, a.y, I);
            I.run(sr);
        }
        float o[D], r;
        int hit;
        r = goal_reward<N>(c, e.x, e.y, sr.dXd, sr.dYd, e.px, e.py, e.gx, e.gy, hit);
        count_hits(b.cnt, live && hit);
        e.x = (float)((double)e.x + sr.dXd); e.y = (float)((double)e.y + sr.dYd); e.vx = sr.vx; e.vy = sr.vy; e.om = sr.om;
        e.th = wrap_two_pi(e.th + sr.dth);
        const uint32_t el = ct.x + 1u;
        const int trunc = !sr.done && (int)el >= c.max_episode_steps;
        const int fin = sr.done | trunc;
        const bool restart = live && fin && c.auto_reset;
        if (live) ct.x = el;
        if (tl.count && __any(restart)) {
            goal_observe<N>(c, e, o);
            term_append<D>(tl, restart, t, i, o);
        }
        if (__any(restart && n_spare == 0)) refill();
        if (restart) {
            ct = make_uint2(0u, ct.y + 1u);
            SpareEpisode<N>::get(spare, (int)(ct.y % (uint32_t)kSpare), tid, e, aux, cs);
            n_spare--;
        }
        goal_observe<N>(c, e, o);
        if (live) {
            const int64_t row = (int64_t)t * B + i;
            store_row(obs, row, o);
            reward[row] = r;
            done[row] = (uint8_t)fin;
            truncated[row] = (uint8_t)trunc;
        }
        if (live && hit && !restart) {
            Tiling T;
            T.episode = ct.y; T.goal_draws = aux.x;
            T.ship_tile = aux.y & 0xffu; T.goal_tile = (aux.y >> 8) & 0xffu; T.case_b = (aux.y >> 16) & 1u; T.flip = (aux.y >> 17) & 1u;
            T.free_counts = (uint64_t)aux.z | ((uint64_t)aux.w << 32);
            T.cs0 = cs.x; T.cs1 = cs.y; T.cs2 = cs.z; T.cs3 = cs.w;
            goal_resample(c, c.env_index_base + (uint32_t)i, T, e.gx, e.gy);
            aux = pack_aux(T);
        }
    }
    if (live) {
        store_goal_ship<N>(b, i, e);
        store_goal_planets<N>(b, i, e);
        b.ctr[i] = ct;
        b.aux[i] = aux;
        b.cshift[i] = cs;
    }
}

constexpr int kPairBlock = 2 * kBlock;
#ifndef SG_RING
#define SG_RING 5
#endif
constexpr int kRing = SG_RING;
constexpr int kHand = 9;
constexpr int kReplayCap = 128;
#ifndef SG_REPLAY_AT
#define SG_REPLAY_AT 56
#endif
#ifndef SG_PILOT_SLEEP
#define SG_PILOT_SLEEP 40
#endif
constexpr int kReplayAt = SG_REPLAY_AT;
constexpr uint32_t kSpinLimit = 1u << 21;

constexpr int kQDepth = 4;
constexpr int kQCols = 6;
template <int N>
struct EpisodeQueue {
    __device__ __forceinline__ static float4 *slot(float4 *q, int64_t B, int i, uint32_t episode) {
        return q + ((episode % (uint32_t)kQDepth) * (uint32_t)kQCols * (uint32_t)B + (uint32_t)i);
    }
    __device__ __forceinline__ static void put(float4 *q, int64_t B, int i, const ShipInit &s, const float (&px)[N],
                                               const float (&py)[N], float gx, float gy, const Tiling &T) {
        float4 *p = slot(q, B, i, T.episode);
        p[0] = make_float4(s.x, s.y, s.th, s.vx);
        p[B] = make_float4(s.vy, s.om, gx, gy);
        p[2 * B] = make_float4(px[0], py[0], px[1], py[1]);
        if constexpr (N == 3) p[3 * B] = make_float4(px[2], py[2], 0.0f, 0.0f);
        if constexpr (N == 4) p[3 * B] = make_float4(px[2], py[2], px[3], py[3]);
        const uint4 a = pack_aux(T);
        p[4 * B] = make_float4(__uint_as_float(a.y), __uint_as_float(a.z), __uint_as_float(a.w), 0.0f);
        p[5 * B] = make_float4(T.cs0, T.cs1, T.cs2, T.cs3);
    }
};

__device__ __forceinline__ uint32_t flag_load(const uint32_t *p) {
    return __hip_atomic_load(p, __ATOMIC_ACQUIRE, __HIP_MEMORY_SCOPE_WORKGROUP);
}
__device__ __forceinline__ void flag_store(uint32_t *p, uint32_t v) {
    __hip_atomic_store(p, v, __ATOMIC_RELEASE, __HIP_MEMORY_SCOPE_WORKGROUP);
}
__device__ __forceinline__ uint32_t lds_flag_load(const uint32_t *p) {
    const uint32_t v = __hip_atomic_load(p, __ATOMIC_RELAXED, __HIP_MEMORY_SCOPE_WORKGROUP);
    __builtin_amdgcn_fence(__ATOMIC_ACQUIRE, "workgroup", "local");
    return v;
}
__device__ __forceinline__ uint32_t lds_flag_peek(const uint32_t *p) {
    return __hip_atomic_load(p, __ATOMIC_RELAXED, __HIP_MEMORY_SCOPE_WORKGROUP);
}
__device__ __forceinline__ void lds_flag_store(uint32_t *p, uint32_t v) {
    __builtin_amdgcn_fence(__ATOMIC_RELEASE, "workgroup", "local");
    __hip_atomic_store(p, v, __ATOMIC_RELAXED, __HIP_MEMORY_SCOPE_WORKGROUP);
}
__device__ __forceinline__ uint32_t lds_flag_load_uniform(const uint32_t *p) {
    return (uint32_t)__builtin_amdgcn_readfirstlane((int)lds_flag_load(p));
}
template <int kSleep = 1>
__device__ __forceinline__ bool wait_flag(const uint32_t *flag, uint32_t want, uint32_t *seen = nullptr) {
    uint32_t v = lds_flag_load_uniform(flag);
    if ((int32_t)(v - want) < 0) {
#pragma unroll 1
        for (uint32_t n = 0; n < kSpinLimit; n++) {
            __builtin_amdgcn_s_sleep(kSleep);
            v = lds_flag_load_uniform(flag);
            if ((int32_t)(v - want) >= 0) break;
        }
        if ((int32_t)(v - want) < 0) return false;
    }
    if (seen) *seen = v;
    return true;
}

template <int N>
struct GoalReplay {
    static constexpr int kWords = 13 + 2 * N;
    __device__ __forceinline__ static void put(float *rb, uint32_t slot, uint32_t step_lane, const GoalEnv<N> &e, float2 a) {
        float *q = rb + slot;
        int f = 0;
        auto w = [&](float v) { q[(f++) * kReplayCap] = v; };
        w(__uint_as_float(step_lane));
        w(e.x); w(e.y); w(e.th); w(e.vx); w(e.vy); w(e.om); w(a.x); w(a.y);
#pragma unroll
        for (int j = 0; j < N; j++) { w(e.px[j]); w(e.py[j]); }
    }
    __device__ __forceinline__ static void put_goal(float *rb, uint32_t slot, float gx, float gy) {
        rb[(9 + 2 * N) * kReplayCap + slot] = gx; rb[(10 + 2 * N) * kReplayCap + slot] = gy;
    }
    __device__ __forceinline__ static void get(const float *rb, uint32_t slot, uint32_t &step_lane, GoalEnv<N> &e, float2 &a) {
        const float *q = rb + slot;
        int f = 0;
        auto r = [&]() { return q[(f++) * kReplayCap]; };
        step_lane = __float_as_uint(r());
        e.x = r(); e.y = r(); e.th = r(); e.vx = r(); e.vy = r(); e.om = r(); a.x = r(); a.y = r();
#pragma unroll
        for (int j = 0; j < N; j++) { e.px[j] = r(); e.py[j] = r(); }
        e.gx = r(); e.gy = r();
    }
    __device__ __forceinline__ static void put_result(float *rb, uint32_t slot, const StepResult &r, float th) {
        float *q = rb + slot;
        const uint64_t ux = __double_as_longlong(r.dXd), uy = __double_as_longlong(r.dYd);
        q[3 * kReplayCap] = th; q[4 * kReplayCap] = r.vx; q[5 * kReplayCap] = r.vy; q[6 * kReplayCap] = r.om;
        q[7 * kReplayCap] = __uint_as_float((uint32_t)ux); q[8 * kReplayCap] = __uint_as_float((uint32_t)(ux >> 32));
        q[(11 + 2 * N) * kReplayCap] = __uint_as_float((uint32_t)uy); q[(12 + 2 * N) * kReplayCap] = __uint_as_float((uint32_t)(uy >> 32));
    }
    __device__ __forceinline__ static void get_result(const float *rb, uint32_t slot, double &dXd, double &dYd) {
        const float *q = rb + slot;
        const uint64_t ux = (uint64_t)__float_as_uint(q[7 * kReplayCap]) | ((uint64_t)__float_as_uint(q[8 * kReplayCap]) << 32);
        const uint64_t uy = (uint64_t)__float_as_uint(q[(11 + 2 * N) * kReplayCap]) | ((uint64_t)__float_as_uint(q[(12 + 2 * N) * kReplayCap]) << 32);
        dXd = __longlong_as_double((long long)ux); dYd = __longlong_as_double((long long)uy);
    }
};

struct NoTermList {};
struct NoProfileSource {
    static constexpr bool kOn = false;
};
struct ProfileSource {
    static constexpr bool kOn = true;
    const void *table;
    const uint8_t *idx;
    __device__ __forceinline__ GoalRewardView goal(const SgDev &c, int env) const {
        return goal_reward_view(c, static_cast<const GoalRewardProfile *>(table)[idx[env]]);
    }
    __device__ __forceinline__ KeplerRewardView kepler(const SgDev &c, int env) const {
        return kepler_reward_view(c, static_cast<const KeplerRewardProfile *>(table)[idx[env]]);
    }
};

template <int N, bool ACCEL, bool TOBS, typename TL, typename RS = NoProfileSource>
__device__ __forceinline__ void goal_replay_pass(const SgDev &c, const float *rb, uint32_t lo, uint32_t n, int lane, int wave_env0,
                                                 int64_t B, float *__restrict__ reward, const TL &tl, uint32_t *tail,
                                                 unsigned long long *cnt, const RS &rs = RS{}) {
    constexpr int D = 7 + 2 * N + 2;
    const bool have = (uint32_t)lane < n;
    const uint32_t slot = (lo + (have ? (uint32_t)lane : 0u)) % (uint32_t)kReplayCap;
    uint32_t step_lane;
    GoalEnv<N> e;
    float2 a;
    GoalReplay<N>::get(rb, slot, step_lane, e, a);
    lds_flag_store(tail, lo + n);
    StepResult r;
    {
        Integrator<N, N, true, ACCEL> I;
        goal_env_begin<N, ACCEL>(c, e, a.x, a.y, I, false);
        I.run(r);
    }
    int hit;
    float rew;
    if constexpr (RS::kOn) rew = goal_reward<N>(rs.goal(c, wave_env0 + (int)(step_lane & 63u)), e.x, e.y, r.dXd, r.dYd, e.px, e.py, e.gx, e.gy, hit);
    else rew = goal_reward<N>(c, e.x, e.y, r.dXd, r.dYd, e.px, e.py, e.gx, e.gy, hit);
    count_hits(cnt, have && hit);
    const int t = (int)(step_lane >> 6), env = wave_env0 + (int)(step_lane & 63u);
    if (have) reward[(int64_t)t * B + env] = rew;
    if constexpr (TOBS) {
        e.x = (float)((double)e.x + r.dXd); e.y = (float)((double)e.y + r.dYd); e.vx = r.vx; e.vy = r.vy; e.om = r.om;
        e.th = wrap_two_pi(e.th + r.dth);
        float o[D];
        goal_observe<N>(c, e, o);
        term_append<D>(tl, have, t, env, o);
    }
}

template <int N, bool ACCEL>
__device__ __forceinline__ void goal_replay_integrate(const SgDev &c, float *rb, uint32_t lo, uint32_t n, int lane) {
    const bool have = (uint32_t)lane < n;
    const uint32_t slot = (lo + (have ? (uint32_t)lane : 0u)) % (uint32_t)kReplayCap;
    uint32_t step_lane;
    GoalEnv<N> e;
    float2 a;
    GoalReplay<N>::get(rb, slot, step_lane, e, a);
    StepResult r;
    {
        Integrator<N, N, true, ACCEL> I;
        goal_env_begin<N, ACCEL>(c, e, a.x, a.y, I, false);
        I.run(r);
    }
    if (have) GoalReplay<N>::put_result(rb, slot, r, wrap_two_pi(e.th + r.dth));
}
template <int N, bool TOBS, typename TL, typename RS = NoProfileSource>
__device__ __forceinline__ void goal_replay_reward(const SgDev &c, const float *rb, uint32_t lo, uint32_t n, int lane, int wave_env0,
                                                   int64_t B, float *__restrict__ reward, const TL &tl, unsigned long long *cnt,
                                                   const RS &rs = RS{}) {
    constexpr int D = 7 + 2 * N + 2;
    const bool have = (uint32_t)lane < n;
    const uint32_t slot = (lo + (have ? (uint32_t)lane : 0u)) % (uint32_t)kReplayCap;
    uint32_t step_lane;
    GoalEnv<N> e;
    float2 a;
    GoalReplay<N>::get(rb, slot, step_lane, e, a);
    double dXd, dYd;
    GoalReplay<N>::get_result(rb, slot, dXd, dYd);
    int hit;
    float rew;
    if constexpr (RS::kOn) rew = goal_reward<N>(rs.goal(c, wave_env0 + (int)(step_lane & 63u)), e.x, e.y, dXd, dYd, e.px, e.py, e.gx, e.gy, hit);
    else rew = goal_reward<N>(c, e.x, e.y, dXd, dYd, e.px, e.py, e.gx, e.gy, hit);
    count_hits(cnt, have && hit);
    const int t = (int)(step_lane >> 6), env = wave_env0 + (int)(step_lane & 63u);
    if (have) reward[(int64_t)t * B + env] = rew;
    if constexpr (TOBS) {
        e.x = (float)((double)e.x + dXd); e.y = (float)((double)e.y + dYd);
        float o[D];
        goal_observe<N>(c, e, o);
        term_append<D>(tl, have, t, env, o);
    }
}

template <int N, bool ACCEL, int kSpare, bool TOBS>
__global__ __launch_bounds__(kPairBlock) void goal_pair_rollout_kernel(const SgDev *__restrict__ cfg, const SgBuffers *__restrict__ bufs,
                                                                    int num_envs, int n_steps,
                                                                    const void *__restrict__ actions, float *__restrict__ obs,
                                                                    float *__restrict__ reward, uint8_t *__restrict__ done,
                                                                    uint8_t *__restrict__ truncated,
                                                                    typename std::conditional<TOBS, TermList, NoTermList>::type tl,
                                                                    int *__restrict__ status) {
#define SG_ROLLOUT_PROFILED 0
#define SG_ROLLOUT_RS
#include "sg_goal_pair_rollout.inc"
#undef SG_ROLLOUT_RS
#undef SG_ROLLOUT_PROFILED
}
template <int N, bool ACCEL, int kSpare, bool TOBS>
__global__ __launch_bounds__(kPairBlock) void goal_pair_rollout_profiled_kernel(const SgDev *__restrict__ cfg,
                                                                             const SgBuffers *__restrict__ bufs, int num_envs, int n_steps,
                                                                             const void *__restrict__ actions, float *__restrict__ obs,
                                                                             float *__restrict__ reward, uint8_t *__restrict__ done,
                                                                             uint8_t *__restrict__ truncated,
                                                                             typename std::conditional<TOBS, TermList, NoTermList>::type tl,
                                                                             int *__restrict__ status, ProfileSource rs) {
#define SG_ROLLOUT_PROFILED 1
#define SG_ROLLOUT_RS , rs
#include "sg_goal_pair_rollout.inc"
#undef SG_ROLLOUT_RS
#undef SG_ROLLOUT_PROFILED
}

template <typename F, typename... X>
__device__ __forceinline__ void pair_step(const SgDev *cfg, SgBuffers b, int num_envs, const void *actions, float *obs,
                                          float *reward, uint8_t *done, uint8_t *truncated, float *terminal_obs, X... extra) {
    __shared__ float hand[kHand * kBlock];
    const int tid = threadIdx.x & (kBlock - 1);
    const bool pilot = threadIdx.x < kBlock;
    const int i = blockIdx.x * kBlock + tid;
    const bool live = i < num_envs;
    const int ii = live ? i : 0;
    typename F::Env e;
    F::load_env(b, ii, e);
    const SgDev &c = *cfg;
    if constexpr (F::kTouchParams) {
        const uint32_t *cw = reinterpret_cast<const uint32_t *>(cfg);
        uint32_t touch = 0u;
#pragma unroll
        for (int k = 0; k < (int)(sizeof(SgDev) / 4); k += 16) touch ^= cw[k];
        touch ^= cw[sizeof(SgDev) / 4 - 1];
        asm volatile("" ::"s"(touch));
    }
    const bool discrete = c.discrete_actions != 0;
    float2 a = make_float2(0.0f, 0.0f);
    if constexpr (F::kFinishAction) load_action(discrete, actions, ii, a.x, a.y);
    float *q = hand + tid;
    if (pilot) {
        if constexpr (!F::kFinishAction) load_action(discrete, actions, ii, a.x, a.y);
        StepResult r;
        F::integrate(c, e, a, r);
        const uint64_t ux = __double_as_longlong(r.dXd), uy = __double_as_longlong(r.dYd);
        q[0 * kBlock] = __uint_as_float((uint32_t)ux); q[1 * kBlock] = __uint_as_float((uint32_t)(ux >> 32));
        q[2 * kBlock] = __uint_as_float((uint32_t)uy); q[3 * kBlock] = __uint_as_float((uint32_t)(uy >> 32));
        q[4 * kBlock] = wrap_two_pi(e.th + r.dth); q[5 * kBlock] = r.vx; q[6 * kBlock] = r.vy; q[7 * kBlock] = r.om;
        q[8 * kBlock] = __uint_as_float((uint32_t)r.done);
        __syncthreads();
        return;
    }
    const F fam(c, extra...);
    const uint2 ct = b.ctr[ii];
    const typename F::Ready ready = fam.load_finisher(c, b, ii, e);
    typename F::Next n;
    if (c.auto_reset) F::next(c, ii, ct.y + 1u, F::kept_orbit(b, ii), n);
    __syncthreads();
    PairHand h;
    const uint64_t ux = (uint64_t)__float_as_uint(q[0 * kBlock]) | ((uint64_t)__float_as_uint(q[1 * kBlock]) << 32);
    const uint64_t uy = (uint64_t)__float_as_uint(q[2 * kBlock]) | ((uint64_t)__float_as_uint(q[3 * kBlock]) << 32);
    h.dXd = __longlong_as_double((long long)ux); h.dYd = __longlong_as_double((long long)uy);
    h.th = q[4 * kBlock]; h.vx = q[5 * kBlock]; h.vy = q[6 * kBlock]; h.om = q[7 * kBlock];
    h.done = (int)__float_as_uint(q[8 * kBlock]);
    float o[F::D], r;
    const int hit = fam.pair_finish(c, b, ready, e, a, h, live, o, r);
    const uint32_t el = ct.x + 1u;
    const int trunc = !h.done && (int)el >= c.max_episode_steps;
    const int fin = h.done | trunc;
    const bool restart = fin && c.auto_reset;
    if (live) {
        if (fin && terminal_obs) store_row(terminal_obs, i, o);
        reward[i] = r;
        done[i] = (uint8_t)fin;
        truncated[i] = (uint8_t)trunc;
        if (restart) {
            fam.install(c, b, i, ct.y + 1u, n, e, o);
        } else {
            b.q0[i] = make_float4(e.x, e.y, e.th, e.vx);
            reinterpret_cast<float2 *>(b.q1 + i)[0] = make_float2(e.vy, e.om);
            b.ctr[i] = make_uint2(el, ct.y);
        }
        store_row(obs, i, o);
    }
    if constexpr (F::kResample) F::resample_wave(c, b, i, live && hit && !restart, ct.y);
}

template <int N, bool ACCEL>
// ... 294 lines not shown
            const double *src = static_cast<const double *>(rp.table);
            const int words = rp.n * (int)(sizeof(Prof) / sizeof(double));
            for (int k = (int)threadIdx.x; k < words; k += kBlock) sg_profile_lds[k] = src[k];
            __syncthreads();
            tab = reinterpret_cast<const Prof *>(sg_profile_lds);
        }
    }
    __device__ __forceinline__ void load(const SgBuffers &b, int jj, float4 *base) const {
        P::load(b, jj, base);
        __builtin_amdgcn_global_load_lds((gbl_void *)(reinterpret_cast<const uint32_t *>(idx) + (jj >> 2)), (lds_void *)(base + kIdxAt), 4, 0, 0);
    }
    __device__ __forceinline__ void read(const float4 *blk, int lane, Env &e) const {
        P::read(blk, lane, e);
        e.prof = (reinterpret_cast<const uint32_t *>(blk + kIdxAt)[lane] >> (8 * (lane & 3))) & 0xffu;
    }
    __device__ __forceinline__ int finish(const SgDev &c, const SgBuffers &b, int, Env &e, float2 a, const StepResult &sr, bool kept,
                                          float (&o)[P::D], float &r) const {
        const View v = reward_view(c, tab[e.prof]);
        return P::finish_r(c, v, b, e, a, sr, kept, o, r);
    }
    __device__ __forceinline__ int replay(const SgDev &c, const SgBuffers &b, int env, Env &e, float2 a, bool terminal, bool have,
                                          float (&o)[P::D], float &r, int &dn) const {
        const View v = reward_view(c, tab[idx[env]]);
        return P::replay_r(c, v, b, e, a, terminal, have, o, r, dn);
    }
    struct Ready {
        typename P::Ready base;
        View v;
    };
    __device__ __forceinline__ Ready load_finisher(const SgDev &c, const SgBuffers &b, int i, const Env &e) const {
        Ready rd;
        rd.base = P::load_finisher(c, b, i, e);
        rd.v = reward_view(c, tab[idx[i]]);
        return rd;
    }
    __device__ __forceinline__ int pair_finish(const SgDev &c, const SgBuffers &b, const Ready &rd, Env &e, float2 a, const PairHand &h,
                                               bool live, float (&o)[P::D], float &r) const {
        return P::pair_finish_r(c, rd.v, b, rd.base, e, a, h, live, o, r);
    }
};

template <int N, bool ACCEL>
__global__ __launch_bounds__(kBlock) __attribute__((amdgpu_waves_per_eu(2))) void goal_step_profiled_kernel(const SgDev *__restrict__ cfg, SgBuffers b, int n_subtiles,
                                                                   const void *__restrict__ actions, float *__restrict__ obs,
                                                                   float *__restrict__ reward, uint8_t *__restrict__ done,
                                                                   uint8_t *__restrict__ truncated, float *__restrict__ terminal_obs,
                                                                   int stream_out, RewardProfiles rp) {
    step_subtiles<Profiled<GoalStep<N, ACCEL>, GoalRewardProfile, true>>(cfg, b, n_subtiles, actions, obs, reward, done, truncated,
                                                                        terminal_obs, stream_out, rp);
}
template <bool ACCEL>
__global__ __launch_bounds__(kBlock) __attribute__((amdgpu_waves_per_eu(2))) void kepler_step_profiled_kernel(const SgDev *__restrict__ cfg, SgBuffers b, int n_subtiles,
                                                                     const void *__restrict__ actions, float *__restrict__ obs,
                                                                     float *__restrict__ reward, uint8_t *__restrict__ done,
                                                                     uint8_t *__restrict__ truncated, float *__restrict__ terminal_obs,
                                                                     int stream_out, RewardProfiles rp) {
    step_subtiles<Profiled<KeplerStep<ACCEL>, KeplerRewardProfile, true>>(cfg, b, n_subtiles, actions, obs, reward, done, truncated,
                                                                         terminal_obs, stream_out, rp);
}
template <int N, bool ACCEL>
__global__ __launch_bounds__(kPairBlock) void goal_pair_step_profiled_kernel(const SgDev *__restrict__ cfg, SgBuffers b, int num_envs,
                                                                          const void *__restrict__ actions, float *__restrict__ obs,
                                                                          float *__restrict__ reward, uint8_t *__restrict__ done,
                                                                          uint8_t *__restrict__ truncated, float *__restrict__ terminal_obs,
                                                                          RewardProfiles rp) {
    pair_step<Profiled<GoalStep<N, ACCEL>, GoalRewardProfile, false>>(cfg, b, num_envs, actions, obs, reward, done, truncated, terminal_obs, rp);
}
template <bool ACCEL>
__global__ __launch_bounds__(kPairBlock) void kepler_pair_step_profiled_kernel(const SgDev *__restrict__ cfg, SgBuffers b, int num_envs,
                                                                            const void *__restrict__ actions, float *__restrict__ obs,
                                                                            float *__restrict__ reward, uint8_t *__restrict__ done,
                                                                            uint8_t *__restrict__ truncated, float *__restrict__ terminal_obs,
                                                                            RewardProfiles rp) {
    pair_step<Profiled<KeplerStep<ACCEL>, KeplerRewardProfile, false>>(cfg, b, num_envs, actions, obs, reward, done, truncated, terminal_obs, rp);
}

constexpr int kStatusProfileIndex = 5;
__global__ __launch_bounds__(kBlock) void profile_index_kernel(const uint8_t *__restrict__ src, uint8_t *__restrict__ dst, int num_envs,
                                                               int n, int *__restrict__ status) {
    const int i = (int)blockIdx.x * kBlock + (int)threadIdx.x;
    if (i >= num_envs) return;
    const uint32_t p = src[i];
    const bool bad = p >= (uint32_t)n;
    dst[i] = bad ? (uint8_t)0 : (uint8_t)p;
    if (bad) *status = kStatusProfileIndex;
}

template <typename F>
__device__ __forceinline__ void reset_envs(const SgDev *cfg, SgBuffers b, int fresh, float *obs) {
    const SgDev &c = *cfg;
    const int i = blockIdx.x * kBlock + threadIdx.x;
    if (i >= c.num_envs) return;
    const uint32_t episode = fresh ? 0u : b.ctr[i].y + 1u;
    typename F::Next n;
    F::next(c, i, episode, F::reset_orbit(c), n);
    typename F::Env e;
    float o[F::D];
    F(c).install(c, b, i, episode, n, e, o);
    F::empty_queue(b, i, episode);
    if (obs) store_row(obs, i, o);
}

template <typename F>
__device__ __forceinline__ void reset_masked(const SgDev *cfg, SgBuffers b, const uint8_t *mask, float *obs, double *ep_ret,
                                             int32_t *ep_len) {
    const SgDev &c = *cfg;
    const int i = blockIdx.x * kBlock + threadIdx.x;
    const bool sel = i < c.num_envs && mask[i] != 0;
    const unsigned long long need = __ballot(sel);
    if (!need) return;
    uint32_t episode = 0u;
    float2 orbit = make_float2(0.0f, 0.0f);
    if (sel) {
        episode = b.ctr[i].y + 1u;
        orbit = F::kept_orbit(b, i);
    }
    const int lane = threadIdx.x & 63, grp = lane >> 3, sub = lane & (kGroup - 1);
    const int n_items = __popcll(need), wave_env0 = i - lane;
    for (int base = 0; base < n_items; base += 64 / kGroup) {
        const int item = base + grp;
        const int src = nth_set_lane(need, item < n_items ? item : 0);
        const uint32_t ep = __shfl(episode, src);
        const float2 ob = make_float2(__shfl(orbit.x, src), __shfl(orbit.y, src));
        if (item < n_items) F::restart_group(c, b, wave_env0 + src, ep, sub, obs, ob);
    }
    if (sel) {
        F::empty_queue(b, i, episode);
        if (ep_ret) { ep_ret[i] = 0.0; ep_len[i] = 0; }
    }
}

template <int N>
__global__ __launch_bounds__(kBlock) void goal_reset_kernel(const SgDev *__restrict__ cfg, SgBuffers b, int fresh, float *obs) {
    reset_envs<GoalStep<N, false>>(cfg, b, fresh, obs);
}
__global__ __launch_bounds__(kBlock) void kepler_reset_kernel(const SgDev *__restrict__ cfg, SgBuffers b, int fresh, float *obs) {
    reset_envs<KeplerStep<false>>(cfg, b, fresh, obs);
}
template <int N>
__global__ __launch_bounds__(kBlock) void goal_reset_masked_kernel(const SgDev *__restrict__ cfg, SgBuffers b,
                                                                  const uint8_t *__restrict__ mask, float *__restrict__ obs,
                                                                  double *__restrict__ ep_ret, int32_t *__restrict__ ep_len) {
    reset_masked<GoalStep<N, false>>(cfg, b, mask, obs, ep_ret, ep_len);
}
__global__ __launch_bounds__(kBlock) void kepler_reset_masked_kernel(const SgDev *__restrict__ cfg, SgBuffers b,
                                                                    const uint8_t *__restrict__ mask, float *__restrict__ obs,
                                                                    double *__restrict__ ep_ret, int32_t *__restrict__ ep_len) {
    reset_masked<KeplerStep<false>>(cfg, b, mask, obs, ep_ret, ep_len);
}

constexpr uint32_t kDevSnapMagic = 0x53444753u;
constexpr uint32_t kDevSnapEpisodes = 1u, kDevSnapReturns = 2u;
constexpr int kStatusSnapshot = 6;
constexpr uint32_t kRenderRestoreEpoch = 0x10000u;
struct DevSnapHeader {
    uint32_t magic;
    int32_t family, n_planets, randomize_orbit, num_envs;
    uint32_t flags, pad0, pad1;
};
static_assert(sizeof(DevSnapHeader) == 32, "the columns start 16-byte aligned");
struct StateCols {
    float4 *q0, *q1;
    uint2 *ctr;
    uint4 *aux;
    float4 *pl0, *pl1, *cshift;
    double2 *orbd;
    double *ep_ret;
    int32_t *ep_len;
    double *returns;
};
struct EnvRecord {
    float4 q0, q1, pl0, pl1;
    uint2 ctr;
};
__device__ __forceinline__ EnvRecord copy_env(const StateCols &has, const StateCols &from, int j, const StateCols &to, int i) {
    const float4 zero = make_float4(0.0f, 0.0f, 0.0f, 0.0f);
    const float4 q0 = from.q0[j], q1 = from.q1[j];
    const uint2 ctr = from.ctr[j];
    const uint4 aux = from.aux[j];
    float4 pl0 = zero, pl1 = zero, cshift = zero;
    double2 orbd = make_double2(0.0, 0.0);
    double ep_ret = 0.0, returns = 0.0;
    int32_t ep_len = 0;
    if (has.pl0) pl0 = from.pl0[j];
    if (has.pl1) pl1 = from.pl1[j];
    if (has.cshift) cshift = from.cshift[j];
    if (has.orbd) orbd = from.orbd[j];
    if (has.ep_ret) { ep_ret = from.ep_ret[j]; ep_len = from.ep_len[j]; }
    if (has.returns) returns = from.returns[j];
    to.q0[i] = q0; to.q1[i] = q1; to.ctr[i] = ctr; to.aux[i] = aux;
    if (has.pl0) to.pl0[i] = pl0;
    if (has.pl1) to.pl1[i] = pl1;
    if (has.cshift) to.cshift[i] = cshift;
    if (has.orbd) to.orbd[i] = orbd;
    if (has.ep_ret) { to.ep_ret[i] = ep_ret; to.ep_len[i] = ep_len; }
    if (has.returns) to.returns[i] = returns;
    return {q0, q1, pl0, pl1, ctr};
}

__global__ __launch_bounds__(kBlock) void snapshot_kernel(StateCols h, StateCols s, DevSnapHeader hd, DevSnapHeader *__restrict__ out) {
    const int i = blockIdx.x * kBlock + threadIdx.x;
    if (i == 0) {
        uint4 *o = reinterpret_cast<uint4 *>(out);
        o[0] = make_uint4(hd.magic, (uint32_t)hd.family, (uint32_t)hd.n_planets, (uint32_t)hd.randomize_orbit);
        o[1] = make_uint4((uint32_t)hd.num_envs, hd.flags, 0u, 0u);
    }
    if (i >= hd.num_envs) return;
    copy_env(h, h, i, s, i);
}

template <int N>
struct GoalRestore {
    static constexpr int D = 7 + 2 * N + 2;
    __device__ __forceinline__ static void observe(const SgDev &c, const EnvRecord &r, float (&o)[D]) {
        GoalEnv<N> e;
        e.x = r.q0.x; e.y = r.q0.y; e.th = r.q0.z; e.vx = r.q0.w; e.vy = r.q1.x; e.om = r.q1.y; e.gx = r.q1.z; e.gy = r.q1.w;
        e.px[0] = r.pl0.x; e.py[0] = r.pl0.y; e.px[1] = r.pl0.z; e.py[1] = r.pl0.w;
        if constexpr (N > 2) { e.px[2] = r.pl1.x; e.py[2] = r.pl1.y; }
        if constexpr (N > 3) { e.px[3] = r.pl1.z; e.py[3] = r.pl1.w; }
        goal_observe<N>(c, e, o);
    }
};
struct KeplerRestore {
    static constexpr int D = 10;
    __device__ __forceinline__ static void observe(const SgDev &c, const EnvRecord &r, float (&o)[D]) {
        KeplerEnv e;
        e.x = r.q0.x; e.y = r.q0.y; e.th = r.q0.z; e.vx = r.q0.w; e.vy = r.q1.x; e.om = r.q1.y; e.phi = r.q1.z; e.ecc = r.q1.w;
        kepler_observe(c, e, o);
    }
};

template <typename F>
__device__ __forceinline__ void restore_envs(const SgDev *cfg, uint32_t *ephi, StateCols h, StateCols s, const DevSnapHeader *hdr,
                                             DevSnapHeader want, const uint8_t *mask, const int32_t *src, float *obs, uint8_t *sel,
                                             uint32_t *epoch, int *status) {
    const int i = blockIdx.x * kBlock + threadIdx.x;
    const DevSnapHeader hd = *hdr;
    if (hd.magic != want.magic || hd.family != want.family || hd.n_planets != want.n_planets ||
        hd.randomize_orbit != want.randomize_orbit || hd.num_envs != want.num_envs || hd.flags != want.flags) {
        if (i == 0) *status = kStatusSnapshot;
        if (sel && i < want.num_envs) sel[i] = 0;
        return;
    }
    if (i == 0 && epoch) *epoch += kRenderRestoreEpoch;
    const bool chosen = i < want.num_envs && (!mask || mask[i] != 0);
    int j = i;
    if (chosen && src) j = src[i];
    const bool take = chosen && (uint32_t)j < (uint32_t)want.num_envs;
    if (chosen && !take) *status = kStatusSnapshot;
    if (sel && i < want.num_envs) sel[i] = take;
    if (!__ballot(take)) return;
    if (!take) return;
    const EnvRecord r = copy_env(h, s, j, h, i);
    if (ephi) ephi[i] = r.ctr.y;
    if (obs) {
        float o[F::D];
        F::observe(*cfg, r, o);
        store_row(obs, i, o);
    }
}
template <int N>
__global__ __launch_bounds__(kBlock) void goal_restore_kernel(const SgDev *__restrict__ cfg, uint32_t *__restrict__ ephi, StateCols h,
                                                             StateCols s, const DevSnapHeader *__restrict__ hdr, DevSnapHeader want,
                                                             const uint8_t *__restrict__ mask, const int32_t *__restrict__ src,
                                                             float *__restrict__ obs, uint8_t *__restrict__ sel,
                                                             uint32_t *__restrict__ epoch, int *__restrict__ status) {
    restore_envs<GoalRestore<N>>(cfg, ephi, h, s, hdr, want, mask, src, obs, sel, epoch, status);
}
__global__ __launch_bounds__(kBlock) void kepler_restore_kernel(const SgDev *__restrict__ cfg, uint32_t *__restrict__ ephi, StateCols h,
                                                               StateCols s, const DevSnapHeader *__restrict__ hdr, DevSnapHeader want,
                                                               const uint8_t *__restrict__ mask, const int32_t *__restrict__ src,
                                                               float *__restrict__ obs, uint8_t *__restrict__ sel,
                                                               uint32_t *__restrict__ epoch, int *__restrict__ status) {
    restore_envs<KeplerRestore>(cfg, ephi, h, s, hdr, want, mask, src, obs, sel, epoch, status);
}

template <bool ACCEL>
__global__ __launch_bounds__(kBlock) void kepler_rollout_kernel(const SgDev *__restrict__ cfg, SgBuffers b, int n_steps,
                                                               const void *__restrict__ actions, float *__restrict__ obs,
                                                               float *__restrict__ reward, uint8_t *__restrict__ done,
                                                               uint8_t *__restrict__ truncated, TermList tl) {
    const SgDev &c = *cfg;
    const bool discrete = c.discrete_actions != 0;
    const int i = blockIdx.x * kBlock + threadIdx.x;
    const bool live = i < c.num_envs;
    const int ii = live ? i : 0;
    const int64_t B = c.num_envs;
    KeplerEnv e;
    load_kepler_env(b, ii, e);
    uint2 ct = b.ctr[ii];
    float2 a_next = load_action_raw(discrete, actions, ii);
    for (int t = 0; t < n_steps; t++) {
        const float2 a = decode_action(discrete, a_next);
        if (t + 1 < n_steps) a_next = load_action_raw(discrete, actions, (int64_t)(t + 1) * B + ii);
        kepler_step_body<ACCEL>(c, b, i, ii, live, e, ct, a, obs + (int64_t)t * B * 10, reward + (int64_t)t * B,
                               done + (int64_t)t * B, truncated + (int64_t)t * B, nullptr, tl.count ? &tl : nullptr, t);
    }
    if (live) {
        store_kepler_env(b, i, e);
        b.ctr[i] = ct;
    }
}

constexpr int kKeplerSpareFields = 12;
constexpr int kKeplerReplayWords = 15;

template <bool ACCEL, typename RS = NoProfileSource>
__device__ __forceinline__ void kepler_replay_pass(const SgDev &c, const float *rb, uint32_t lo, uint32_t n, int lane, int wave_env0,
                                                   int64_t B, float *__restrict__ reward, const TermList &tl, uint32_t *tail,
                                                   const RS &rs = RS{}) {
    const bool have = (uint32_t)lane < n;
    const float *q = rb + (lo + (have ? (uint32_t)lane : 0u)) % (uint32_t)kReplayCap;
    const uint32_t step_lane = __float_as_uint(q[0]);
    KeplerEnv e;
    e.x = q[1 * kReplayCap]; e.y = q[2 * kReplayCap]; e.th = q[3 * kReplayCap]; e.vx = q[4 * kReplayCap]; e.vy = q[5 * kReplayCap];
    e.om = q[6 * kReplayCap];
    const float a0 = q[7 * kReplayCap], a1 = q[8 * kReplayCap];
    e.phi = q[9 * kReplayCap]; e.ecc = q[10 * kReplayCap];
    const uint64_t uc = (uint64_t)__float_as_uint(q[11 * kReplayCap]) | ((uint64_t)__float_as_uint(q[12 * kReplayCap]) << 32);
    const uint64_t us = (uint64_t)__float_as_uint(q[13 * kReplayCap]) | ((uint64_t)__float_as_uint(q[14 * kReplayCap]) << 32);
    if (tail) lds_flag_store(tail, lo + n);
    Orbit ob = fixed_orbit(c);
    if (c.randomize_orbit) ob = make_orbit(c.k_a, (double)e.ecc, __longlong_as_double((long long)uc), __longlong_as_double((long long)us));
    float o[10], rew;
    int dn;
    StepResult r;
    if constexpr (RS::kOn)
        kepler_env_step_r<ACCEL>(c, rs.kepler(c, wave_env0 + (int)(step_lane & 63u)), ob, e, a0, a1, o, rew, dn, r, false);
    else kepler_env_step<ACCEL>(c, ob, e, a0, a1, o, rew, dn, r, false);
    const int t = (int)(step_lane >> 6), env = wave_env0 + (int)(step_lane & 63u);
    if (have) reward[(int64_t)t * B + env] = rew;
    if (tl.count) term_append<10>(tl, have, t, env, o);
}

template <bool ACCEL, int kSpare>
__global__ __launch_bounds__(kPairBlock) void kepler_pair_rollout_kernel(const SgDev *__restrict__ cfg, SgBuffers b, int n_steps,
                                                                      const void *__restrict__ actions, float *__restrict__ obs,
                                                                      float *__restrict__ reward, uint8_t *__restrict__ done,
                                                                      uint8_t *__restrict__ truncated, TermList tl, int *__restrict__ status) {
#define SG_ROLLOUT_PROFILED 0
#define SG_ROLLOUT_RS
#include "sg_kepler_pair_rollout.inc"
#undef SG_ROLLOUT_RS
#undef SG_ROLLOUT_PROFILED
}
template <bool ACCEL, int kSpare>
__global__ __launch_bounds__(kPairBlock) void kepler_pair_rollout_profiled_kernel(const SgDev *__restrict__ cfg, SgBuffers b, int n_steps,
                                                                               const void *__restrict__ actions, float *__restrict__ obs,
                                                                               float *__restrict__ reward, uint8_t *__restrict__ done,
                                                                               uint8_t *__restrict__ truncated, TermList tl,
                                                                               int *__restrict__ status, ProfileSource rs) {
#define SG_ROLLOUT_PROFILED 1
#define SG_ROLLOUT_RS , rs
#include "sg_kepler_pair_rollout.inc"
#undef SG_ROLLOUT_RS
#undef SG_ROLLOUT_PROFILED
}

__global__ __launch_bounds__(kBlock) void random_actions_kernel(const SgDev *__restrict__ cfg, uint32_t seed_lo, uint32_t seed_hi,
                                                               uint64_t first_step, int n_steps, void *__restrict__ actions) {
    const SgDev &c = *cfg;
    const int i = blockIdx.x * kBlock + threadIdx.x;
    if (i >= c.num_envs) return;
    const int64_t B = c.num_envs;
    for (int t = blockIdx.y; t < n_steps; t += gridDim.y) {
        uint32_t w0, w1;
        random_action_words(seed_lo, seed_hi, c.env_index_base + (uint32_t)i, first_step + (uint64_t)t, w0, w1);
        if (c.discrete_actions) static_cast<int32_t *>(actions)[t * B + i] = (int32_t)__umulhi(w0, 6u);
        else reinterpret_cast<float2 *>(actions)[t * B + i] = make_float2(fmaf(u23(w0), 2.0f, -1.0f), fmaf(u23(w1), 2.0f, -1.0f));
    }
}

__global__ __launch_bounds__(kBlock) void state_io_kernel(const SgDev *__restrict__ cfg, SgBuffers b, int mode, float *ship,
                                                         float *planets, float *goal, int32_t *elapsed) {
    const SgDev &c = *cfg;
    const int i = blockIdx.x * kBlock + threadIdx.x;
    if (i >= c.num_envs) return;
    const int N = c.family == SG_FAMILY_GOAL ? c.n_planets : 0;
    float4 a = b.q0[i], q = b.q1[i];
    if (mode == 0) {
        if (ship) { float *s = ship + 6 * i; s[0] = a.x; s[1] = a.y; s[2] = a.z; s[3] = a.w; s[4] = q.x; s[5] = q.y; }
        if (goal) { goal[2 * i] = q.z; goal[2 * i + 1] = q.w; }
        if (planets)
            for (int j = 0; j < N; j++) {
                const float4 p = b.pl[j >> 1][i];
                planets[(i * N + j) * 2] = (j & 1) ? p.z : p.x;
                planets[(i * N + j) * 2 + 1] = (j & 1) ? p.w : p.y;
            }
        if (elapsed) elapsed[i] = (int32_t)b.ctr[i].x;
    } else {
        if (ship) { const float *s = ship + 6 * i; a = make_float4(s[0], s[1], s[2], s[3]); q.x = s[4]; q.y = s[5]; }
        if (goal) { q.z = goal[2 * i]; q.w = goal[2 * i + 1]; }
        b.q0[i] = a; b.q1[i] = q;
        if (planets)
            for (int k = 0; k < (N + 1) / 2; k++) {
                float4 p = make_float4(0.f, 0.f, 0.f, 0.f);
                p.x = planets[(i * N + 2 * k) * 2]; p.y = planets[(i * N + 2 * k) * 2 + 1];
                if (2 * k + 1 < N) { p.z = planets[(i * N + 2 * k + 1) * 2]; p.w = planets[(i * N + 2 * k + 1) * 2 + 1]; }
                b.pl[k][i] = p;
            }
        if (elapsed) reinterpret_cast<uint32_t *>(b.ctr + i)[0] = (uint32_t)elapsed[i];
        if (goal && c.family == SG_FAMILY_KEPLER && c.randomize_orbit) b.orbd[i] = make_double2(cos((double)q.z), sin((double)q.z));
    }
}

__global__ __launch_bounds__(kBlock) void vector_field_kernel(const SgDev *__restrict__ cfg, SgBuffers b, const void *__restrict__ actions,
                                                             const float *__restrict__ ship, float *__restrict__ out) {
    const SgDev &c = *cfg;
    const bool discrete = c.discrete_actions != 0;
    const int i = blockIdx.x * kBlock + threadIdx.x;
    if (i >= c.num_envs) return;
    float a0, a1, f[6];
    load_action(discrete, actions, i, a0, a1);
    float4 q0 = b.q0[i], q1 = b.q1[i];
    if (ship) { const float *s = ship + 6 * i; q0 = make_float4(s[0], s[1], s[2], s[3]); q1.x = s[4]; q1.y = s[5]; }
    const bool acc = c.steering_acceleration != 0;
    if (c.family == SG_FAMILY_GOAL) {
        float px[4] = {0.f, 0.f, 0.f, 0.f}, py[4] = {0.f, 0.f, 0.f, 0.f};
        const float4 p0 = b.pl[0][i];
        px[0] = p0.x; py[0] = p0.y; px[1] = p0.z; py[1] = p0.w;
        if (c.n_planets > 2) { const float4 p1 = b.pl[1][i]; px[2] = p1.x; py[2] = p1.y; px[3] = p1.z; py[3] = p1.w; }
#define SG_VF(NP)                                                                                                              \
    {                                                                                                                         \
        float cx[NP], cy[NP];                                                                                                 \
        for (int k = 0; k < NP; k++) { cx[k] = px[k]; cy[k] = py[k]; }                                                        \
        if (acc) vector_field<NP, NP, true>(c, q0.x, q0.y, q0.z, q0.w, q1.x, q1.y, a0, a1, cx, cy, f);                        \
        else vector_field<NP, NP, false>(c, q0.x, q0.y, q0.z, q0.w, q1.x, q1.y, a0, a1, cx, cy, f);                           \
    }
        if (c.n_planets == 2) SG_VF(2) else if (c.n_planets == 3) SG_VF(3) else SG_VF(4)
#undef SG_VF
    } else {
        const float cx[1] = {0.0f}, cy[1] = {0.0f};
        if (acc) vector_field<1, 1, true>(c, q0.x, q0.y, q0.z, q0.w, q1.x, q1.y, a0, a1, cx, cy, f);
        else vector_field<1, 1, false>(c, q0.x, q0.y, q0.z, q0.w, q1.x, q1.y, a0, a1, cx, cy, f);
    }
    float *o = out + 6 * i;
#pragma unroll
    for (int k = 0; k < 6; k++) o[k] = f[k];
}

__global__ __launch_bounds__(kBlock) void queue_clear_kernel(const SgDev *__restrict__ cfg, SgBuffers b) {
    const int i = blockIdx.x * kBlock + threadIdx.x;
    if (i < cfg->num_envs) b.ephi[i] = b.ctr[i].y;
}

__global__ __launch_bounds__(kBlock) void term_compact_kernel(const SgDev *__restrict__ cfg, const uint8_t *__restrict__ done_row,
                                                             const float *__restrict__ tobs, int t, int D, TermList tl) {
    const int i = blockIdx.x * kBlock + threadIdx.x;
    const bool want = i < cfg->num_envs && done_row[i < cfg->num_envs ? i : 0] != 0;
    const unsigned long long m = __ballot(want);
    if (!m) return;
    const int lane = threadIdx.x & 63, leader = __ffsll((long long)m) - 1;
    uint32_t base = 0;
    if (lane == leader) base = atomicAdd(tl.count, (uint32_t)__popcll(m));
    base = __shfl(base, leader);
    const uint32_t idx = base + (uint32_t)__popcll(m & ((1ull << lane) - 1ull));
    if (want && idx < tl.capacity) {
        tl.step_env[2 * (int64_t)idx] = t; tl.step_env[2 * (int64_t)idx + 1] = i;
        for (int k = 0; k < D; k++) tl.obs[(int64_t)idx * D + k] = tobs[(int64_t)i * D + k];
    }
}

__global__ __launch_bounds__(kBlock) void count_flags_kernel(const uint8_t *__restrict__ done, const uint8_t *__restrict__ trunc, int64_t n,
                                                            unsigned long long *cnt) {
    if (blockIdx.x == 0 && threadIdx.x == 0) atomicAdd(cnt + 3, (unsigned long long)n);
    unsigned int nd = 0, nt = 0;
    for (int64_t k = (int64_t)blockIdx.x * kBlock + threadIdx.x; k < n; k += (int64_t)gridDim.x * kBlock) { nd += done[k] != 0; nt += trunc[k] != 0; }
#pragma unroll
    for (int o = 32; o > 0; o >>= 1) { nd += __shfl_down(nd, o); nt += __shfl_down(nt, o); }
    if ((threadIdx.x & 63) == 0) {
        if (nd) atomicAdd(cnt, (unsigned long long)nd);
        if (nt) atomicAdd(cnt + 1, (unsigned long long)nt);
    }
}

struct EpList {
    uint32_t *count;
    int32_t *step_env;
    double *ret;
    int32_t *length;
    uint8_t *truncated;
    uint32_t capacity;
};

constexpr int kEpAhead = 16;

__device__ __forceinline__ uint32_t nonzero_bytes(uint32_t w) {
    const uint32_t z = ~(((w & 0x7f7f7f7fu) + 0x7f7f7f7fu) | w | 0x7f7f7f7fu);
    return 4u - (uint32_t)__popc(z);
}

__device__ __forceinline__ uint32_t wave_done_count(int num_envs, int n_steps, const uint8_t *__restrict__ done, int e0) {
    const int lane = threadIdx.x & 63;
    uint32_t c = 0;
    if (num_envs - e0 >= 64 && (num_envs & 15) == 0 && ((uintptr_t)done & 15) == 0) {
        const int seg = lane & 3;
#pragma unroll 8
        for (int t = lane >> 2; t < n_steps; t += 16) {
            const uint4 w = *reinterpret_cast<const uint4 *>(done + (int64_t)t * num_envs + e0 + 16 * seg);
            c += nonzero_bytes(w.x) + nonzero_bytes(w.y) + nonzero_bytes(w.z) + nonzero_bytes(w.w);
        }
    } else if (e0 + lane < num_envs) {
        for (int t = 0; t < n_steps; t++) c += done[(int64_t)t * num_envs + e0 + lane] != 0;
    }
#pragma unroll
    for (int o = 32; o > 0; o >>= 1) c += __shfl_xor(c, o);
    return c;
}

struct EpChunk {
    float r[kEpAhead];
    uint8_t d[kEpAhead], tr[kEpAhead];
};

__global__ __launch_bounds__(kBlock) void episode_stats_kernel(int num_envs, int n_steps, const float *__restrict__ reward,
                                                              const uint8_t *__restrict__ done, const uint8_t *__restrict__ trunc,
                                                              double *__restrict__ ep_ret, int32_t *__restrict__ ep_len,
                                                              double *__restrict__ row_ret, int32_t *__restrict__ row_len, int fill_rows,
                                                              EpList el) {
    const int i = blockIdx.x * kBlock + threadIdx.x;
    const bool live = i < num_envs;
    const int j = live ? i : 0;
    const int lane = threadIdx.x & 63;
    const unsigned long long below = (1ull << lane) - 1ull;
    uint32_t base = 0;
    if (el.count) {
        __shared__ uint32_t wave_n[kBlock / 64 + 1];
        const int w = threadIdx.x >> 6;
        const uint32_t n = wave_done_count(num_envs, n_steps, done, i - lane);
        if (lane == 0) wave_n[w] = n;
        __syncthreads();
        if (threadIdx.x == 0) {
            uint32_t tot = 0;
            for (int k = 0; k < kBlock / 64; k++) tot += wave_n[k];
            wave_n[kBlock / 64] = tot ? atomicAdd(el.count, tot) : 0u;
        }
        __syncthreads();
        base = wave_n[kBlock / 64];
        for (int k = 0; k < w; k++) base += wave_n[k];
    }
    double ret = ep_ret[j];
    int32_t len = ep_len[j];
    auto load = [&](EpChunk &c, int t0) {
#pragma unroll
        for (int u = 0; u < kEpAhead; u++) {
            const int t = t0 + u < n_steps ? t0 + u : n_steps - 1;
            const int64_t k = (int64_t)t * num_envs + j;
            c.r[u] = reward[k]; c.d[u] = done[k]; c.tr[u] = trunc[k];
        }
    };
    auto walk = [&](const EpChunk &c, int t0) {
#pragma unroll
        for (int u = 0; u < kEpAhead; u++) {
            if (t0 + u >= n_steps) break;
            ret += (double)c.r[u];
            len += 1;
            const bool fin = live && c.d[u] != 0;
            if (row_ret) {
                if (fin) { row_ret[i] = ret; row_len[i] = len; }
                else if (live && fill_rows) { row_ret[i] = __builtin_nan(""); row_len[i] = -1; }
            }
            if (el.count) {
                const unsigned long long m = __ballot(fin);
                const uint32_t idx = base + (uint32_t)__popcll(m & below);
                if (fin && idx < el.capacity) {
                    el.step_env[2 * (int64_t)idx] = t0 + u; el.step_env[2 * (int64_t)idx + 1] = i;
                    el.ret[idx] = ret; el.length[idx] = len; el.truncated[idx] = c.tr[u] != 0;
                }
                base += (uint32_t)__popcll(m);
            }
            if (fin) { ret = 0.0; len = 0; }
        }
    };
    if (n_steps == 1) {
        const bool fin = live && done[j] != 0;
        ret += (double)reward[j];
        len += 1;
        if (row_ret && live) {
            if (fin) { row_ret[i] = ret; row_len[i] = len; }
            else if (fill_rows) { row_ret[i] = __builtin_nan(""); row_len[i] = -1; }
        }
        if (el.count) {
            const unsigned long long m = __ballot(fin);
            const uint32_t idx = base + (uint32_t)__popcll(m & below);
            if (fin && idx < el.capacity) {
                el.step_env[2 * (int64_t)idx] = 0; el.step_env[2 * (int64_t)idx + 1] = i;
                el.ret[idx] = ret; el.length[idx] = len; el.truncated[idx] = trunc[j] != 0;
            }
        }
        if (fin) { ret = 0.0; len = 0; }
    } else {
        EpChunk a, b;
        load(a, 0);
        for (int t0 = 0; t0 < n_steps; t0 += 2 * kEpAhead) {
            load(b, t0 + kEpAhead);
            walk(a, t0);
            if (t0 + 2 * kEpAhead < n_steps) load(a, t0 + 2 * kEpAhead);
            walk(b, t0 + kEpAhead);
        }
    }
    if (live) { ep_ret[i] = ret; ep_len[i] = len; }
}

constexpr int kNormMaxStats = 18;

__device__ __forceinline__ double wave_sum_f64(double v) {
#pragma unroll
// ... 2951 lines not shown
```

space_gym_amd/csrc/sg_goal_pair_rollout.inc:

```

    const SgBuffers &b = *bufs;
    using Spare = SpareEpisode<N>;
    using Queue = EpisodeQueue<N>;
    using Integ = Integrator<N, N, true, ACCEL>;
    using Replay = GoalReplay<N>;
    __shared__ float spare[kSpare * Spare::kFields * kBlock];
    __shared__ float ring[kRing * kHand * kBlock];
    __shared__ float rbuf[(kBlock / 64) * Replay::kWords * kReplayCap];
    __shared__ uint32_t spare_hi[kBlock];
    __shared__ uint32_t handed[kBlock / 64], taken[kBlock / 64];
    __shared__ uint32_t rp_tail[kBlock / 64];
    __shared__ uint32_t rp_claim[kBlock / 64], rp_done[kBlock / 64];
    constexpr int D = 7 + 2 * N + 2;
    SG_REAL(0);
    const int tid = threadIdx.x & (kBlock - 1), pair = tid >> 6, lane = tid & 63;
    const bool pilot = threadIdx.x < kBlock;
    const int i = blockIdx.x * kBlock + tid;
    const bool live = i < num_envs;
    const int ii = live ? i : 0;
    const int64_t B = num_envs;
    GoalEnv<N> e;
    load_goal_env<N>(b, ii, e);
    uint2 ct = b.ctr[ii];
    const SgDev &c = *cfg;
    {
        const uint32_t *cw = reinterpret_cast<const uint32_t *>(cfg);
        uint32_t touch = 0u;
#pragma unroll
        for (int k = 0; k < (int)(sizeof(SgDev) / 4); k += 16) touch ^= cw[k];
        touch ^= cw[sizeof(SgDev) / 4 - 1];
        asm volatile("" ::"s"(touch));
    }
    const bool discrete = c.discrete_actions != 0;
    float *const rb = rbuf + pair * Replay::kWords * kReplayCap;
    if (!pilot) spare_hi[tid] = ct.y;
    if (threadIdx.x < kBlock / 64) { handed[threadIdx.x] = 0u; taken[threadIdx.x] = 0u; rp_tail[threadIdx.x] = 0u; rp_claim[threadIdx.x] = 0u; rp_done[threadIdx.x] = 0u; }
    __syncthreads();
    SG_REAL(1);

    if (pilot) {
        SG_ACC_DECL;
        __builtin_amdgcn_s_setprio(3);
        const bool hand_over = c.auto_reset && live;
        const bool auto_reset = c.auto_reset != 0;
        StepConsts kc = step_consts(c);
        asm volatile("" : "+v"(kc.max_engine_force), "+v"(kc.h), "+v"(kc.half_world), "+v"(kc.gm), "+v"(kc.omega_limit), "+v"(kc.planet_r),
                          "+v"(kc.max_thruster_force), "+v"(kc.inv_moi), "+v"(kc.planet_r_d));
        int max_steps = c.max_episode_steps;
        asm volatile("" : "+v"(max_steps));
        float2 a_next = load_action_raw(discrete, actions, ii);
        uint32_t taken_seen = 0u;
        uint32_t head = 0u, tail_seen = 0u;
        for (int t = 0; t < n_steps; t++) {
            const float2 a = decode_action(discrete, a_next);
            if (t + 1 < n_steps) a_next = load_action_raw(discrete, actions, (int64_t)(t + 1) * B + ii);
            if (t - (int)taken_seen >= kRing && !wait_flag<SG_PILOT_SLEEP>(&taken[pair], (uint32_t)(t - kRing + 1), &taken_seen)) { *status = 1; break; }
            if (head + 64u - tail_seen > (uint32_t)kReplayCap) tail_seen = lds_flag_load_uniform(&rp_tail[pair]);
            const bool defer = hand_over && head + 64u - tail_seen <= (uint32_t)kReplayCap;

            const int slot = t % kRing;
            StepResult r;
            int rk;
            {
                Integ I;
                SG_ACC(0);
                goal_env_begin<N, ACCEL>(kc, e, a.x, a.y, I);
                SG_ACC(1);
                rk = I.run(r, [&]() __attribute__((always_inline)) -> bool { return defer; });
                SG_ACC_ADD(7, __any(r.done) ? 1 : 0);
                SG_ACC_ADD(10, __any(r.path == kPathScipyErr || r.path == kPathScipyClear) ? 1 : 0);
                SG_ACC_ADD(11, __any((r.path == kPathScipyErr || r.path == kPathScipyClear) && r.n_rk > 1) ? 1 : 0);
                SG_ACC(2);
            }
            const bool replayed = rk == kRkEventDeferred;
            uint32_t rslot = 0u;
            {
                const unsigned long long dm = __ballot(replayed);
                if (dm) {
                    rslot = (head + (uint32_t)__popcll(dm & ((1ull << lane) - 1ull))) % (uint32_t)kReplayCap;
                    if (replayed) Replay::put(rb, rslot, ((uint32_t)t << 6) | (uint32_t)lane, e, a);
                    head += (uint32_t)__popcll(dm);
                }
            }
            e.x = (float)((double)e.x + r.dXd); e.y = (float)((double)e.y + r.dYd); e.vx = r.vx; e.vy = r.vy; e.om = r.om;
            e.th = wrap_two_pi(e.th + r.dth);
            SG_ACC(3);
            SG_ACC(4);
            {
                float *q = ring + (slot * kHand) * kBlock + tid;
                const uint64_t ux = __double_as_longlong(r.dXd), uy = __double_as_longlong(r.dYd);
                q[0 * kBlock] = __uint_as_float((uint32_t)ux); q[1 * kBlock] = __uint_as_float((uint32_t)(ux >> 32));
                q[2 * kBlock] = __uint_as_float((uint32_t)uy); q[3 * kBlock] = __uint_as_float((uint32_t)(uy >> 32));
                q[4 * kBlock] = e.th; q[5 * kBlock] = e.vx; q[6 * kBlock] = e.vy; q[7 * kBlock] = e.om;
                q[8 * kBlock] = __uint_as_float((uint32_t)r.done | (replayed ? 2u | (rslot << 8) : 0u));
            }
            lds_flag_store(&handed[pair], (uint32_t)(t + 1));
            SG_ACC(5);
            const uint32_t el = ct.x + 1u;
            const int trunc = !r.done && (int)el >= max_steps;
            const bool restart = live && (r.done | trunc) && auto_reset;
            if (live) ct.x = el;
            if (restart) {
                const uint32_t k = ct.y + 1u;
                if ((int32_t)(lds_flag_load(&spare_hi[tid]) - k) >= 0) {
                    const float *q = spare + ((int)(k % (uint32_t)kSpare) * Spare::kFields) * kBlock + tid;
                    e.x = q[0 * kBlock]; e.y = q[1 * kBlock]; e.th = q[2 * kBlock]; e.vx = q[3 * kBlock];
                    e.vy = q[4 * kBlock]; e.om = q[5 * kBlock];
#pragma unroll
                    for (int j = 0; j < N; j++) { e.px[j] = q[(8 + 2 * j) * kBlock]; e.py[j] = q[(9 + 2 * j) * kBlock]; }
                } else {
                    Tiling T;
                    T.episode = k;
                    ShipInit s;
                    float gx, gy;
                    goal_reset<N>(c, c.env_index_base + (uint32_t)i, T, s, e.px, e.py, gx, gy);
                    e.x = s.x; e.y = s.y; e.th = s.th; e.vx = s.vx; e.vy = s.vy; e.om = s.om;
                }
                ct = make_uint2(0u, k);
            }
            SG_ACC(8);
        }
        SG_ACC_WRITE(blockIdx.x * 8 + pair);
        SG_REAL(2);
        if (live) {
            b.q0[i] = make_float4(e.x, e.y, e.th, e.vx);
            reinterpret_cast<float2 *>(b.q1 + i)[0] = make_float2(e.vy, e.om);
            store_goal_planets<N>(b, i, e);
            b.ctr[i] = ct;
        }
        {
            uint32_t lo = 0u;
            if (lane == 0) lo = atomicMax(&rp_claim[pair], head);
            lo = (uint32_t)__builtin_amdgcn_readfirstlane((int)lo);
            __builtin_amdgcn_fence(__ATOMIC_SEQ_CST, "wavefront");
#pragma unroll 1
            while ((int32_t)(head - lo) > 0) {
                const uint32_t n = min(head - lo, 64u);
                goal_replay_integrate<N, ACCEL>(c, rb, lo, n, lane);
                lo += n;
            }
            lds_flag_store(&rp_done[pair], 1u);
        }
        SG_REAL(3);
        return;
    }

    SG_ACC_DECL;
    const bool auto_reset = c.auto_reset != 0;
    const int wave_env0 = i - lane;
    unsigned long long *const cnt = b.cnt;
    GoalStepConsts fc = goal_step_consts(c);
#if SG_ROLLOUT_PROFILED
    {
        const GoalRewardView v = rs.goal(c, ii);
        fc.danger_r2 = v.danger_r2; fc.survival = v.survival; fc.goal_scale = v.goal_scale; fc.safety_scale = v.safety_scale;
        fc.sparse = v.sparse;
    }
#endif
    asm volatile("" : "+v"(fc.goal_r2), "+v"(fc.danger_r2), "+v"(fc.survival), "+v"(fc.goal_scale), "+v"(fc.safety_scale),
                      "+v"(fc.sparse), "+v"(fc.planet_r), "+v"(fc.two_over_world));
    int max_steps = c.max_episode_steps;
    asm volatile("" : "+v"(max_steps));
    uint32_t hi = ct.y;
    uint4 aux = b.aux[ii];
    float4 cs = b.cshift[ii];
    if (auto_reset) {
        const uint32_t q_hi = b.ephi[ii];
        const int n_have = live ? min(max((int32_t)(q_hi - ct.y), 0), kSpare) : 0;
        float4 rec[kSpare][kQCols];
#pragma unroll
        for (int s = 0; s < kSpare; s++)
            if (s < n_have) {
                const float4 *p = Queue::slot(b.epq, B, i, ct.y + 1u + (uint32_t)s);
#pragma unroll
                for (int col = 0; col < kQCols; col++)
                    if (col != 3 || N > 2) rec[s][col] = p[(uint32_t)col * (uint32_t)B];
            }
#pragma unroll
        for (int s = 0; s < kSpare; s++)
            if (s < n_have) Spare::put_record(spare, (int)((ct.y + 1u + (uint32_t)s) % (uint32_t)kSpare), tid, rec[s]);
        hi = ct.y + (uint32_t)n_have;
        lds_flag_store(&spare_hi[tid], hi);
    }
    auto refill = [&]() {
        SG_ACC_ADD(10, 1);
        if (live && hi - ct.y < (uint32_t)kSpare) {
            Tiling T;
            T.episode = hi + 1u;
            ShipInit s;
            float px[N], py[N], gx, gy;
            goal_reset<N>(c, c.env_index_base + (uint32_t)i, T, s, px, py, gx, gy);
            Spare::put(spare, (int)(T.episode % (uint32_t)kSpare), tid, s, px, py, gx, gy, T);
            Queue::put(b.epq, B, i, s, px, py, gx, gy, T);
            hi = T.episode;
            lds_flag_store(&spare_hi[tid], hi);
        }
    };
    constexpr uint32_t kKeep = 1u;
    if (auto_reset && __any(live && hi - ct.y < kKeep)) refill();
    uint32_t tail = 0u, complete = 0u;
    bool mine = true;
    typedef __attribute__((address_space(1))) float gfloat;
    typedef __attribute__((address_space(1))) uint8_t gbyte;
    gfloat *obs_p = (gfloat *)obs + (int64_t)ii * D, *rew_p = (gfloat *)reward + ii;
    gbyte *done_p = (gbyte *)done + ii, *trunc_p = (gbyte *)truncated + ii;
    asm volatile("" : "+v"(obs_p), "+v"(rew_p), "+v"(done_p), "+v"(trunc_p));
    for (int t = 0; t < n_steps; t++) {
        SG_ACC(0);
        if (!wait_flag(&handed[pair], (uint32_t)(t + 1))) { *status = 2; break; }
        SG_ACC(1);
        double dXd, dYd;
        float th, vx, vy, om;
        int dn;
        bool replayed;
        {
            const int slot = t % kRing;
            const float *q = ring + (slot * kHand) * kBlock + tid;
            const uint64_t ux = (uint64_t)__float_as_uint(q[0 * kBlock]) | ((uint64_t)__float_as_uint(q[1 * kBlock]) << 32);
            const uint64_t uy = (uint64_t)__float_as_uint(q[2 * kBlock]) | ((uint64_t)__float_as_uint(q[3 * kBlock]) << 32);
            dXd = __longlong_as_double((long long)ux); dYd = __longlong_as_double((long long)uy);
            th = q[4 * kBlock]; vx = q[5 * kBlock]; vy = q[6 * kBlock]; om = q[7 * kBlock];
            const uint32_t w8 = __float_as_uint(q[8 * kBlock]);
            dn = (int)(w8 & 1u);
            replayed = (w8 & 2u) != 0u;
            if (replayed) Replay::put_goal(rb, w8 >> 8, e.gx, e.gy);
            complete += (uint32_t)__popcll(__ballot(replayed));
        }
        lds_flag_store(&taken[pair], (uint32_t)(t + 1));
        SG_ACC(3);
        float o[D], r;
        int hit;
        r = goal_reward<N>(fc, e.x, e.y, dXd, dYd, e.px, e.py, e.gx, e.gy, hit);
        count_hits(cnt, live && hit && !replayed);
        e.x = (float)((double)e.x + dXd); e.y = (float)((double)e.y + dYd); e.vx = vx; e.vy = vy; e.om = om; e.th = th;
        const uint32_t el = ct.x + 1u;
        const int trunc = !dn && (int)el >= max_steps;
        const int fin = dn | trunc;
        const bool restart = live && fin && auto_reset;
        if (live) ct.x = el;
        SG_ACC(4);
        if constexpr (TOBS) {
            if (__any(restart && !replayed)) {
                goal_observe<N>(fc, e, o);
                term_append<D>(tl, restart && !replayed, t, i, o);
            }
        }
        const uint32_t keep = t + 1 < n_steps ? kKeep : 0u;
        if (auto_reset && __any(live && hi - ct.y < (restart ? keep + 1u : keep))) refill();
        SG_ACC(6);
        if (restart) {
            ct = make_uint2(0u, ct.y + 1u);
            Spare::get(spare, (int)(ct.y % (uint32_t)kSpare), tid, e, aux, cs);
        }
        SG_ACC(12);
        goal_observe<N>(fc, e, o);
        SG_ACC(13);
        if (live) {
#pragma unroll
            for (int k = 0; k < D; k++) obs_p[k] = o[k];
            if (!replayed) *rew_p = r;
            *done_p = (uint8_t)fin;
            *trunc_p = (uint8_t)trunc;
        }
        obs_p += B * D; rew_p += B; done_p += B; trunc_p += B;
        asm volatile("" : "+v"(obs_p), "+v"(rew_p), "+v"(done_p), "+v"(trunc_p));
        SG_ACC(5);
        SG_ACC(7);
        SG_ACC_ADD(11, __any(live && hit && !restart) ? 1 : 0);
        if (live && hit && !restart) {
            Tiling T;
            T.episode = ct.y; T.goal_draws = aux.x;
            T.ship_tile = aux.y & 0xffu; T.goal_tile = (aux.y >> 8) & 0xffu; T.case_b = (aux.y >> 16) & 1u; T.flip = (aux.y >> 17) & 1u;
            T.free_counts = (uint64_t)aux.z | ((uint64_t)aux.w << 32);
            T.cs0 = cs.x; T.cs1 = cs.y; T.cs2 = cs.z; T.cs3 = cs.w;
            goal_resample(c, c.env_index_base + (uint32_t)i, T, e.gx, e.gy);
            aux = pack_aux(T);
        }
        SG_ACC(2);
        if (complete - tail >= (uint32_t)kReplayAt && mine) {
            const uint32_t n = min(complete - tail, 64u);
            uint32_t got = 0u;
            if (lane == 0) got = atomicCAS(&rp_claim[pair], tail, tail + n);
            mine = (uint32_t)__builtin_amdgcn_readfirstlane((int)got) == tail;
            if (mine) {
                __builtin_amdgcn_fence(__ATOMIC_ACQ_REL, "workgroup", "local");
                goal_replay_pass<N, ACCEL, TOBS>(c, rb, tail, n, lane, wave_env0, B, reward, tl, &rp_tail[pair], cnt SG_ROLLOUT_RS);
                tail += n;
            }
        }
        SG_ACC(9);
    }
    SG_ACC_WRITE(blockIdx.x * 8 + 4 + pair);
    SG_REAL(2);
    if (live) {
        reinterpret_cast<float2 *>(b.q1 + i)[1] = make_float2(e.gx, e.gy);
        b.aux[i] = aux;
        b.cshift[i] = cs;
        if (auto_reset) b.ephi[i] = hi;
    }
    if (tail != complete) {
        if (!wait_flag(&rp_done[pair], 1u)) *status = 3;
#pragma unroll 1
        while (tail != complete) {
            const uint32_t n = min(complete - tail, 64u);
            goal_replay_reward<N, TOBS>(c, rb, tail, n, lane, wave_env0, B, reward, tl, cnt SG_ROLLOUT_RS);
            tail += n;
        }
    }
    SG_REAL(3);
```

space_gym_amd/csrc/sg_kepler_pair_rollout.inc:

```

    using Integ = Integrator<2, 1, false, ACCEL>;
    __shared__ float spare[kSpare * kKeplerSpareFields * kBlock];
    __shared__ float ring[kRing * kHand * kBlock];
    __shared__ float rbuf[(kBlock / 64) * kKeplerReplayWords * kReplayCap];
    __shared__ uint32_t spare_hi[kBlock];
    __shared__ uint32_t handed[kBlock / 64], taken[kBlock / 64];
    __shared__ uint32_t rp_tail[kBlock / 64], rp_claim[kBlock / 64];
    const SgDev &c = *cfg;
    const bool discrete = c.discrete_actions != 0;
    const int tid = threadIdx.x & (kBlock - 1), pair = tid >> 6, lane = tid & 63;
    const bool pilot = threadIdx.x < kBlock;
    const int i = blockIdx.x * kBlock + tid;
    const bool live = i < c.num_envs;
    const int ii = live ? i : 0;
    const int64_t B = c.num_envs;
    KeplerEnv e;
    load_kepler_env(b, ii, e);
    uint2 ct = b.ctr[ii];
    float *const rb = rbuf + pair * kKeplerReplayWords * kReplayCap;
    if (!pilot) spare_hi[tid] = ct.y;
    if (threadIdx.x < kBlock / 64) { handed[threadIdx.x] = 0u; taken[threadIdx.x] = 0u; rp_tail[threadIdx.x] = 0u; rp_claim[threadIdx.x] = 0u; }
    __syncthreads();

    if (pilot) {
        __builtin_amdgcn_s_setprio(3);
        const bool hand_over = c.auto_reset && live;
        const bool auto_reset = c.auto_reset != 0;
        const bool rnd_orbit = c.randomize_orbit != 0;
        StepConsts kc = step_consts(c);
        float border_r = c.border_r;
        int max_steps = c.max_episode_steps;
        asm volatile("" : "+v"(kc.max_engine_force), "+v"(kc.h), "+v"(kc.half_world), "+v"(kc.gm), "+v"(kc.omega_limit), "+v"(kc.planet_r),
                          "+v"(kc.max_thruster_force), "+v"(kc.inv_moi), "+v"(kc.planet_r_d), "+v"(border_r), "+v"(max_steps));
        double2 orb = rnd_orbit ? b.orbd[ii] : make_double2(1.0, 0.0);
        float2 a_next = load_action_raw(discrete, actions, ii);
        uint32_t taken_seen = 0u;
        uint32_t head = 0u, tail_seen = 0u;
        for (int t = 0; t < n_steps; t++) {
            const float2 a_raw = decode_action(discrete, a_next);
            float a0 = a_raw.x, a1 = a_raw.y;
            if (t + 1 < n_steps) a_next = load_action_raw(discrete, actions, (int64_t)(t + 1) * B + ii);
            if (t - (int)taken_seen >= kRing && !wait_flag<SG_PILOT_SLEEP>(&taken[pair], (uint32_t)(t - kRing + 1), &taken_seen)) { *status = 1; break; }
            if (head + 64u - tail_seen > (uint32_t)kReplayCap) tail_seen = lds_flag_load_uniform(&rp_tail[pair]);
            const bool defer = hand_over && head + 64u - tail_seen <= (uint32_t)kReplayCap;
            const int slot = t % kRing;
            StepResult r;
            int rk;
            {
                float engine, F, om, om0, alpha;
                translate_action(a0, a1, kc.max_engine_force, engine, F, om);
                if (ACCEL && kc.steering_acceleration) { om0 = e.om; alpha = (a1 * kc.max_thruster_force) * kc.inv_moi; }
                else { om0 = om; alpha = 0.0f; }
                const float cax[2] = {0.0f, 0.0f}, cay[2] = {0.0f, 0.0f}, cR[2] = {kc.planet_r, border_r};
                const double cRd[2] = {kc.planet_r_d, (double)border_r};
                Integ I;
                I.begin(kc.h, kc.half_world, kc.gm, F, om0, alpha, kc.omega_limit, e.x, e.y, e.th, e.vx, e.vy, cax, cay, cR, cRd);
                rk = I.run(r, [&]() __attribute__((always_inline)) -> bool { return defer; });
            }
            const bool replayed = rk == kRkEventDeferred;
            {
                const unsigned long long dm = __ballot(replayed);
                if (dm) {
                    if (replayed) {
                        float *q = rb + (head + (uint32_t)__popcll(dm & ((1ull << lane) - 1ull))) % (uint32_t)kReplayCap;
                        const uint64_t uc = __double_as_longlong(orb.x), us = __double_as_longlong(orb.y);
                        q[0] = __uint_as_float(((uint32_t)t << 6) | (uint32_t)lane);
                        q[1 * kReplayCap] = e.x; q[2 * kReplayCap] = e.y; q[3 * kReplayCap] = e.th; q[4 * kReplayCap] = e.vx;
                        q[5 * kReplayCap] = e.vy; q[6 * kReplayCap] = e.om; q[7 * kReplayCap] = a_raw.x; q[8 * kReplayCap] = a_raw.y;
                        q[9 * kReplayCap] = e.phi; q[10 * kReplayCap] = e.ecc;
                        q[11 * kReplayCap] = __uint_as_float((uint32_t)uc); q[12 * kReplayCap] = __uint_as_float((uint32_t)(uc >> 32));
                        q[13 * kReplayCap] = __uint_as_float((uint32_t)us); q[14 * kReplayCap] = __uint_as_float((uint32_t)(us >> 32));
                    }
                    head += (uint32_t)__popcll(dm);
                }
            }
            e.x = (float)((double)e.x + r.dXd); e.y = (float)((double)e.y + r.dYd); e.vx = r.vx; e.vy = r.vy; e.om = r.om;
            e.th = wrap_two_pi(e.th + r.dth);
            {
                float *q = ring + (slot * kHand) * kBlock + tid;
                const uint64_t ux = __double_as_longlong(r.dXd), uy = __double_as_longlong(r.dYd);
                q[0 * kBlock] = __uint_as_float((uint32_t)ux); q[1 * kBlock] = __uint_as_float((uint32_t)(ux >> 32));
                q[2 * kBlock] = __uint_as_float((uint32_t)uy); q[3 * kBlock] = __uint_as_float((uint32_t)(uy >> 32));
                q[4 * kBlock] = e.th; q[5 * kBlock] = e.vx; q[6 * kBlock] = e.vy; q[7 * kBlock] = e.om;
                q[8 * kBlock] = __uint_as_float((uint32_t)r.done | (replayed ? 2u : 0u));
            }
            lds_flag_store(&handed[pair], (uint32_t)(t + 1));
            const uint32_t el = ct.x + 1u;
            const int trunc = !r.done && (int)el >= max_steps;
            const bool restart = live && (r.done | trunc) && auto_reset;
            if (live) ct.x = el;
            if (restart) {
                const uint32_t k = ct.y + 1u;
                if ((int32_t)(lds_flag_load(&spare_hi[tid]) - k) >= 0) {
                    const float *q = spare + ((int)(k % (uint32_t)kSpare) * kKeplerSpareFields) * kBlock + tid;
                    e.x = q[0 * kBlock]; e.y = q[1 * kBlock]; e.th = q[2 * kBlock]; e.vx = q[3 * kBlock];
                    e.vy = q[4 * kBlock]; e.om = q[5 * kBlock];
                    if (rnd_orbit) {
                        e.phi = q[6 * kBlock]; e.ecc = q[7 * kBlock];
                        const uint64_t uc = (uint64_t)__float_as_uint(q[8 * kBlock]) | ((uint64_t)__float_as_uint(q[9 * kBlock]) << 32);
                        const uint64_t us = (uint64_t)__float_as_uint(q[10 * kBlock]) | ((uint64_t)__float_as_uint(q[11 * kBlock]) << 32);
                        orb = make_double2(__longlong_as_double((long long)uc), __longlong_as_double((long long)us));
                    }
                } else {
                    ShipInit s;
                    kepler_reset(c, c.env_index_base + (uint32_t)i, k, s, e.phi, e.ecc);
                    e.x = s.x; e.y = s.y; e.th = s.th; e.vx = s.vx; e.vy = s.vy; e.om = s.om;
                    if (rnd_orbit) orb = make_double2(cos((double)e.phi), sin((double)e.phi));
                }
                ct = make_uint2(0u, k);
            }
        }
        if (live) {
            b.q0[i] = make_float4(e.x, e.y, e.th, e.vx);
            reinterpret_cast<float2 *>(b.q1 + i)[0] = make_float2(e.vy, e.om);
            b.ctr[i] = ct;
        }
        {
            uint32_t lo = 0u;
            if (lane == 0) lo = atomicMax(&rp_claim[pair], head);
            lo = (uint32_t)__builtin_amdgcn_readfirstlane((int)lo);
            __builtin_amdgcn_fence(__ATOMIC_SEQ_CST, "wavefront");
#pragma unroll 1
            while ((int32_t)(head - lo) > 0) {
                const uint32_t n = min(head - lo, 64u);
                kepler_replay_pass<ACCEL>(c, rb, lo, n, lane, i - lane, B, reward, tl, nullptr SG_ROLLOUT_RS);
                lo += n;
            }
        }
        return;
    }

    const int wave_env0 = i - lane;
    KeplerStepConsts fc = kepler_step_consts(c);
#if SG_ROLLOUT_PROFILED
    {
        const KeplerRewardView v = rs.kepler(c, ii);
        fc.k_C = v.k_C; fc.k_Cr = v.k_Cr; fc.k_Ca = v.k_Ca;
    }
#endif
    asm volatile("" : "+v"(fc.k_gm), "+v"(fc.k_C), "+v"(fc.k_Cr), "+v"(fc.k_phi), "+v"(fc.k_ecc), "+v"(fc.k_a), "+v"(fc.k_Ca));
    Orbit ob_fixed = fixed_orbit(c);
    asm volatile("" : "+v"(ob_fixed.a), "+v"(ob_fixed.b), "+v"(ob_fixed.c), "+v"(ob_fixed.ecc), "+v"(ob_fixed.cosphi), "+v"(ob_fixed.sinphi),
                      "+v"(ob_fixed.a_over_b), "+v"(ob_fixed.b_over_a), "+v"(ob_fixed.inv_a));
    float max_engine_force = c.max_engine_force;
    int max_steps = c.max_episode_steps;
    asm volatile("" : "+v"(max_engine_force), "+v"(max_steps));
    const bool rnd_orbit = c.randomize_orbit != 0, auto_reset = c.auto_reset != 0;
    uint32_t hi = ct.y;
    double2 orb = c.randomize_orbit ? b.orbd[ii] : make_double2(1.0, 0.0);
    auto refill = [&]() {
        if (hi - ct.y < (uint32_t)kSpare) {
            ShipInit s;
            float phi = e.phi, ecc = e.ecc;
            kepler_reset(c, c.env_index_base + (uint32_t)ii, hi + 1u, s, phi, ecc);
            float *q = spare + ((int)((hi + 1u) % (uint32_t)kSpare) * kKeplerSpareFields) * kBlock + tid;
            q[0 * kBlock] = s.x; q[1 * kBlock] = s.y; q[2 * kBlock] = s.th; q[3 * kBlock] = s.vx; q[4 * kBlock] = s.vy;
            q[5 * kBlock] = s.om; q[6 * kBlock] = phi; q[7 * kBlock] = ecc;
            if (c.randomize_orbit) {
                const uint64_t uc = __double_as_longlong(cos((double)phi)), us = __double_as_longlong(sin((double)phi));
                q[8 * kBlock] = __uint_as_float((uint32_t)uc); q[9 * kBlock] = __uint_as_float((uint32_t)(uc >> 32));
                q[10 * kBlock] = __uint_as_float((uint32_t)us); q[11 * kBlock] = __uint_as_float((uint32_t)(us >> 32));
            }
            hi += 1u;
            lds_flag_store(&spare_hi[tid], hi);
        }
    };
    constexpr uint32_t kKeep = 1u;
    if (c.auto_reset) refill();
    uint32_t tail = 0u, complete = 0u;
    bool mine = true;
    for (int t = 0; t < n_steps; t++) {
        float a0, a1;
        load_action(discrete, actions, (int64_t)t * B + ii, a0, a1);
        if (!wait_flag(&handed[pair], (uint32_t)(t + 1))) { *status = 2; break; }
        double dXd, dYd;
        float th, vx, vy, om;
        int dn;
        bool replayed;
        {
            const int slot = t % kRing;
            const float *q = ring + (slot * kHand) * kBlock + tid;
            const uint64_t ux = (uint64_t)__float_as_uint(q[0 * kBlock]) | ((uint64_t)__float_as_uint(q[1 * kBlock]) << 32);
            const uint64_t uy = (uint64_t)__float_as_uint(q[2 * kBlock]) | ((uint64_t)__float_as_uint(q[3 * kBlock]) << 32);
            dXd = __longlong_as_double((long long)ux); dYd = __longlong_as_double((long long)uy);
            th = q[4 * kBlock]; vx = q[5 * kBlock]; vy = q[6 * kBlock]; om = q[7 * kBlock];
            const uint32_t w8 = __float_as_uint(q[8 * kBlock]);
            dn = (int)(w8 & 1u);
            replayed = (w8 & 2u) != 0u;
            complete += (uint32_t)__popcll(__ballot(replayed));
        }
        lds_flag_store(&taken[pair], (uint32_t)(t + 1));
        float engine, F, om_cmd;
        translate_action(a0, a1, max_engine_force, engine, F, om_cmd);
        Orbit ob = ob_fixed;
        if (rnd_orbit) ob = make_orbit(fc.k_a, (double)e.ecc, orb.x, orb.y);
        const float r = kepler_reward(fc, ob, e.x, e.y, dXd, dYd, vx, vy, engine, a1);
        e.x = (float)((double)e.x + dXd); e.y = (float)((double)e.y + dYd); e.vx = vx; e.vy = vy; e.om = om; e.th = th;
        const uint32_t el = ct.x + 1u;
        const int trunc = !dn && (int)el >= max_steps;
        const int fin = dn | trunc;
        const bool restart = live && fin && auto_reset;
        ct.x = el;
        if (tl.count && __any(restart && !replayed)) {
            float ot[10];
            kepler_observe(fc, e, ot);
            term_append<10>(tl, restart && !replayed, t, i, ot);
        }
        if (auto_reset && __any(live && hi - ct.y < (restart ? kKeep + 1u : kKeep))) refill();
        if (restart) {
            ct = make_uint2(0u, ct.y + 1u);
            const float *q = spare + ((int)(ct.y % (uint32_t)kSpare) * kKeplerSpareFields) * kBlock + tid;
            e.x = q[0 * kBlock]; e.y = q[1 * kBlock]; e.th = q[2 * kBlock]; e.vx = q[3 * kBlock]; e.vy = q[4 * kBlock];
            e.om = q[5 * kBlock]; e.phi = q[6 * kBlock]; e.ecc = q[7 * kBlock];
            if (rnd_orbit) {
                const uint64_t uc = (uint64_t)__float_as_uint(q[8 * kBlock]) | ((uint64_t)__float_as_uint(q[9 * kBlock]) << 32);
                const uint64_t us = (uint64_t)__float_as_uint(q[10 * kBlock]) | ((uint64_t)__float_as_uint(q[11 * kBlock]) << 32);
                orb = make_double2(__longlong_as_double((long long)uc), __longlong_as_double((long long)us));
            }
        }
        float o[10];
        kepler_observe(fc, e, o);
        if (live) {
            const int64_t row = (int64_t)t * B + i;
            store_row(obs, row, o);
            if (!replayed) reward[row] = r;
            done[row] = (uint8_t)fin;
            truncated[row] = (uint8_t)trunc;
        }
        if (complete - tail >= (uint32_t)kReplayAt && mine) {
            const uint32_t n = min(complete - tail, 64u);
            uint32_t got = 0u;
            if (lane == 0) got = atomicCAS(&rp_claim[pair], tail, tail + n);
            mine = (uint32_t)__builtin_amdgcn_readfirstlane((int)got) == tail;
            if (mine) {
                __builtin_amdgcn_fence(__ATOMIC_ACQUIRE, "workgroup", "local");
                kepler_replay_pass<ACCEL>(c, rb, tail, n, lane, wave_env0, B, reward, tl, &rp_tail[pair] SG_ROLLOUT_RS);
                tail += n;
            }
        }
    }
    if (live && c.randomize_orbit) b.orbd[i] = orb;
    if (live) reinterpret_cast<float2 *>(b.q1 + i)[1] = make_float2(e.phi, e.ecc);
```

Before: 31.09 billion.

## Compute heading sin/cos once per step and hand it through ring and spares

Each step's heading sin/cos is computed once by the integrating (pilot) wave after updating theta. It is reused for the next step's integrator begin and passed through the LDS handoff ring and spare-episode slots, so the consumer wave no longer recomputes it for observations. This moves transcendental work off the consumer side and removes a duplicate sincos per step. In exchange the ring grows from 9 to 10 words per slot, and spare records grow by two fields. To limit the larger LDS footprint, the goal ring depth is capped at 4 when N>3, which may reduce pilot/consumer slack.

After: 29.36 billion. -5.6%, worse.

```diff
diff --git a/space_gym_amd/csrc/sg_device.hpp b/space_gym_amd/csrc/sg_device.hpp
--- a/space_gym_amd/csrc/sg_device.hpp
+++ b/space_gym_amd/csrc/sg_device.hpp
@@ -265,13 +265,16 @@
     SG_MFN void begin(float h_total, float half_world_, float gm_, float F_, float om_, float alpha_, float w_limit_,
                       float x0_, float y0_, float th0_, float vx0, float vy0, const float (&cax_)[NC],
                       const float (&cay_)[NC], const float (&cR_)[NC], const double (&cRd_)[NC], bool use_probe = true) {
+        float S0, C0;
+        sincos_acc(th0_, S0, C0);
+        begin(h_total, half_world_, gm_, F_, om_, alpha_, w_limit_, x0_, y0_, th0_, S0, C0, vx0, vy0, cax_, cay_, cR_, cRd_, use_probe);
+    }
+    SG_MFN void begin(float h_total, float half_world_, float gm_, float F_, float om_, float alpha_, float w_limit_,
+                      float x0_, float y0_, float th0_, float S0, float C0, float vx0, float vy0, const float (&cax_)[NC],
+                      const float (&cay_)[NC], const float (&cR_)[NC], const double (&cRd_)[NC], bool use_probe = true) {
         SG_STAMP(8);
         set_constants(h_total, half_world_, gm_, F_, om_, alpha_, w_limit_, x0_, y0_, cax_, cay_, cR_, cRd_);
-        {
-            float S0, C0;
-            sincos_acc(th0_, S0, C0);
-            nCF = -(C0 * F); nSF = -(S0 * F);
-        }
+        nCF = -(C0 * F); nSF = -(S0 * F);
         t = 0.0f; X = 0.0f; Y = 0.0f; vx = vx0; vy = vy0;
         Xd = 0.0; Yd = 0.0;
         const f2 T = mk2(nCF, nSF);
@@ -1163,29 +1166,37 @@
 }
 
 template <int N, typename CFG>
+SG_FN void goal_observe(const CFG &c, const GoalEnv<N> &e, float s, float co, float (&obs)[7 + 2 * N + 2]) {
+    obs[0] = e.x; obs[1] = e.y; obs[2] = co; obs[3] = s; obs[4] = e.vx; obs[5] = e.vy; obs[6] = e.om;
+#pragma unroll
+    for (int j = 0; j < N; j++) lidar(e.px[j] - e.x, e.py[j] - e.y, c.planet_r, c.two_over_world, obs[7 + 2 * j], obs[8 + 2 * j]);
+    obs[7 + 2 * N] = (e.gx - e.x) * c.two_over_world;
+    obs[8 + 2 * N] = (e.gy - e.y) * c.two_over_world;
+}
+template <int N, typename CFG>
 SG_FN void goal_observe(const CFG &c, const GoalEnv<N> &e, float (&obs)[7 + 2 * N + 2]) {
     float s, co;
     sincos_acc(e.th, s, co);
+    goal_observe<N>(c, e, s, co, obs);
+}
+
+template <typename CFG>
+SG_FN void kepler_observe(const CFG &c, const KeplerEnv &e, float s, float co, float (&obs)[10]) {
     obs[0] = e.x; obs[1] = e.y; obs[2] = co; obs[3] = s; obs[4] = e.vx; obs[5] = e.vy; obs[6] = e.om;
-#pragma unroll
-    for (int j = 0; j < N; j++) lidar(e.px[j] - e.x, e.py[j] - e.y, c.planet_r, c.two_over_world, obs[7 + 2 * j], obs[8 + 2 * j]);
-    obs[7 + 2 * N] = (e.gx - e.x) * c.two_over_world;
-    obs[8 + 2 * N] = (e.gy - e.y) * c.two_over_world;
-}
-
+    obs[7] = c.randomize_orbit ? e.phi : (float)c.k_phi;
+    obs[8] = c.randomize_orbit ? e.ecc : (float)c.k_ecc;
+    obs[9] = (float)c.k_a;
+}
 template <typename CFG>
 SG_FN void kepler_observe(const CFG &c, const KeplerEnv &e, float (&obs)[10]) {
     float s, co;
     sincos_acc(e.th, s, co);
-    obs[0] = e.x; obs[1] = e.y; obs[2] = co; obs[3] = s; obs[4] = e.vx; obs[5] = e.vy; obs[6] = e.om;
-    obs[7] = c.randomize_orbit ? e.phi : (float)c.k_phi;
-    obs[8] = c.randomize_orbit ? e.ecc : (float)c.k_ecc;
-    obs[9] = (float)c.k_a;
+    kepler_observe(c, e, s, co, obs);
 }
 
 template <int N, bool ACCEL = false>
-SG_FN void goal_env_begin(const SgDev &c, const GoalEnv<N> &e, float a0, float a1, Integrator<N, N, true, ACCEL> &I,
-                          bool use_probe = true) {
+SG_FN void goal_env_begin(const SgDev &c, const GoalEnv<N> &e, float S0, float C0, float a0, float a1,
+                          Integrator<N, N, true, ACCEL> &I, bool use_probe = true) {
     float engine, F, om, om0, alpha;
     translate_action(a0, a1, c.max_engine_force, engine, F, om);
     steering<ACCEL>(c, a1, om, e.om, om0, alpha);
@@ -1193,7 +1204,14 @@
     double cRd[N];
 #pragma unroll
     for (int j = 0; j < N; j++) { cR[j] = c.planet_r; cRd[j] = c.planet_r_d; }
-    I.begin(c.h, c.half_world, c.gm, F, om0, alpha, c.omega_limit, e.x, e.y, e.th, e.vx, e.vy, e.px, e.py, cR, cRd, use_probe);
+    I.begin(c.h, c.half_world, c.gm, F, om0, alpha, c.omega_limit, e.x, e.y, e.th, S0, C0, e.vx, e.vy, e.px, e.py, cR, cRd, use_probe);
+}
+template <int N, bool ACCEL = false>
+SG_FN void goal_env_begin(const SgDev &c, const GoalEnv<N> &e, float a0, float a1, Integrator<N, N, true, ACCEL> &I,
+                          bool use_probe = true) {
+    float S0, C0;
+    sincos_acc(e.th, S0, C0);
+    goal_env_begin<N, ACCEL>(c, e, S0, C0, a0, a1, I, use_probe);
 }
 
 struct GoalStepConsts {
@@ -1258,8 +1276,8 @@
     return k;
 }
 template <int N, bool ACCEL = false>
-SG_FN void goal_env_begin(const StepConsts &k, const GoalEnv<N> &e, float a0, float a1, Integrator<N, N, true, ACCEL> &I,
-                          bool use_probe = true) {
+SG_FN void goal_env_begin(const StepConsts &k, const GoalEnv<N> &e, float S0, float C0, float a0, float a1,
+                          Integrator<N, N, true, ACCEL> &I, bool use_probe = true) {
     float engine, F, om, om0, alpha;
     translate_action(a0, a1, k.max_engine_force, engine, F, om);
     if (ACCEL && k.steering_acceleration) { om0 = e.om; alpha = (a1 * k.max_thruster_force) * k.inv_moi; }
@@ -1268,7 +1286,14 @@
     double cRd[N];
 #pragma unroll
     for (int j = 0; j < N; j++) { cR[j] = k.planet_r; cRd[j] = k.planet_r_d; }
-    I.begin(k.h, k.half_world, k.gm, F, om0, alpha, k.omega_limit, e.x, e.y, e.th, e.vx, e.vy, e.px, e.py, cR, cRd, use_probe);
+    I.begin(k.h, k.half_world, k.gm, F, om0, alpha, k.omega_limit, e.x, e.y, e.th, S0, C0, e.vx, e.vy, e.px, e.py, cR, cRd, use_probe);
+}
+template <int N, bool ACCEL = false>
+SG_FN void goal_env_begin(const StepConsts &k, const GoalEnv<N> &e, float a0, float a1, Integrator<N, N, true, ACCEL> &I,
+                          bool use_probe = true) {
+    float S0, C0;
+    sincos_acc(e.th, S0, C0);
+    goal_env_begin<N, ACCEL>(k, e, S0, C0, a0, a1, I, use_probe);
 }
 
 template <int N, typename RC>
diff --git a/space_gym_amd/csrc/sg_engine.hip b/space_gym_amd/csrc/sg_engine.hip
--- a/space_gym_amd/csrc/sg_engine.hip
+++ b/space_gym_amd/csrc/sg_engine.hip
@@ -790,7 +790,8 @@
 
 template <int N>
 struct SpareEpisode {
-    static constexpr int kFields = 6 + 2 * N + 2 + 7;
+    static constexpr int kFields = 6 + 2 * N + 2 + 7 + 2;
+    static constexpr int kSin = kFields - 2, kCos = kFields - 1;
     __device__ __forceinline__ static void put(float *base, int slot, int tid, const ShipInit &s, const float (&px)[N],
                                                const float (&py)[N], float gx, float gy, const Tiling &T) {
         float *p = base + (slot * kFields) * kBlock + tid;
@@ -802,6 +803,9 @@
         const uint4 a = pack_aux(T);
         w(__uint_as_float(a.y)); w(__uint_as_float(a.z)); w(__uint_as_float(a.w));
         w(T.cs0); w(T.cs1); w(T.cs2); w(T.cs3);
+        float sn, co;
+        sincos_acc(s.th, sn, co);
+        w(sn); w(co);
     }
     __device__ __forceinline__ static void put_record(float *base, int slot, int tid, const float4 (&r)[6]) {
         float *p = base + (slot * kFields) * kBlock + tid;
@@ -813,8 +817,12 @@
         if constexpr (N > 3) { w(r[3].z); w(r[3].w); }
         w(r[4].x); w(r[4].y); w(r[4].z);
         w(r[5].x); w(r[5].y); w(r[5].z); w(r[5].w);
-    }
-    __device__ __forceinline__ static void get(const float *base, int slot, int tid, GoalEnv<N> &e, uint4 &aux, float4 &cs) {
+        float sn, co;
+        sincos_acc(r[0].z, sn, co);
+        w(sn); w(co);
+    }
+    __device__ __forceinline__ static void get(const float *base, int slot, int tid, GoalEnv<N> &e, uint4 &aux, float4 &cs,
+                                               float &sn, float &co) {
         const float *p = base + (slot * kFields) * kBlock + tid;
         int f = 0;
         auto r = [&]() { return p[(f++) * kBlock]; };
@@ -824,6 +832,7 @@
         aux.x = 0u;
         aux.y = __float_as_uint(r()); aux.z = __float_as_uint(r()); aux.w = __float_as_uint(r());
         cs.x = r(); cs.y = r(); cs.z = r(); cs.w = r();
+        sn = r(); co = r();
     }
 };
 
@@ -858,13 +867,15 @@
     uint4 aux = b.aux[ii];
     float4 cs = b.cshift[ii];
     float2 a_next = load_action_raw(discrete, actions, ii);
+    float hs, hc;
+    sincos_acc(e.th, hs, hc);
     for (int t = 0; t < n_steps; t++) {
         const float2 a = decode_action(discrete, a_next);
         if (t + 1 < n_steps) a_next = load_action_raw(discrete, actions, (int64_t)(t + 1) * B + ii);
         StepResult sr;
         {
             Integrator<N, N, true, ACCEL> I;
-            goal_env_begin<N, ACCEL>(c, e, a.x, a.y, I);
+            goal_env_begin<N, ACCEL>(c, e, hs, hc, a.x, a.y, I);
             I.run(sr);
         }
         float o[D], r;
@@ -873,22 +884,23 @@
         count_hits(b.cnt, live && hit);
         e.x = (float)((double)e.x + sr.dXd); e.y = (float)((double)e.y + sr.dYd); e.vx = sr.vx; e.vy = sr.vy; e.om = sr.om;
         e.th = wrap_two_pi(e.th + sr.dth);
+        sincos_acc(e.th, hs, hc);
         const uint32_t el = ct.x + 1u;
         const int trunc = !sr.done && (int)el >= c.max_episode_steps;
         const int fin = sr.done | trunc;
         const bool restart = live && fin && c.auto_reset;
         if (live) ct.x = el;
         if (tl.count && __any(restart)) {
-            goal_observe<N>(c, e, o);
+            goal_observe<N>(c, e, hs, hc, o);
             term_append<D>(tl, restart, t, i, o);
         }
         if (__any(restart && n_spare == 0)) refill();
         if (restart) {
             ct = make_uint2(0u, ct.y + 1u);
-            SpareEpisode<N>::get(spare, (int)(ct.y % (uint32_t)kSpare), tid, e, aux, cs);
+            SpareEpisode<N>::get(spare, (int)(ct.y % (uint32_t)kSpare), tid, e, aux, cs, hs, hc);
             n_spare--;
         }
-        goal_observe<N>(c, e, o);
+        goal_observe<N>(c, e, hs, hc, o);
         if (live) {
             const int64_t row = (int64_t)t * B + i;
             store_row(obs, row, o);
@@ -921,6 +933,9 @@
 #endif
 constexpr int kRing = SG_RING;
 constexpr int kHand = 9;
+constexpr int kRollHand = 10;
+template <int N>
+constexpr int goal_ring_depth() { return N > 3 && kRing > 4 ? 4 : kRing; }
 constexpr int kReplayCap = 128;
 #ifndef SG_REPLAY_AT
 #define SG_REPLAY_AT 56
@@ -1821,7 +1836,7 @@
     }
 }
 
-constexpr int kKeplerSpareFields = 12;
+constexpr int kKeplerSpareFields = 14;
 constexpr int kKeplerReplayWords = 15;
 
 template <bool ACCEL, typename RS = NoProfileSource>
diff --git a/space_gym_amd/csrc/sg_goal_pair_rollout.inc b/space_gym_amd/csrc/sg_goal_pair_rollout.inc
--- a/space_gym_amd/csrc/sg_goal_pair_rollout.inc
+++ b/space_gym_amd/csrc/sg_goal_pair_rollout.inc
@@ -5,7 +5,8 @@
     using Integ = Integrator<N, N, true, ACCEL>;
     using Replay = GoalReplay<N>;
     __shared__ float spare[kSpare * Spare::kFields * kBlock];
-    __shared__ float ring[kRing * kHand * kBlock];
+    constexpr int kRingN = goal_ring_depth<N>();
+    __shared__ float ring[kRingN * kRollHand * kBlock];
     __shared__ float rbuf[(kBlock / 64) * Replay::kWords * kReplayCap];
     __shared__ uint32_t spare_hi[kBlock];
     __shared__ uint32_t handed[kBlock / 64], taken[kBlock / 64];
@@ -51,20 +52,22 @@
         float2 a_next = load_action_raw(discrete, actions, ii);
         uint32_t taken_seen = 0u;
         uint32_t head = 0u, tail_seen = 0u;
+        float hs, hc;
+        sincos_acc(e.th, hs, hc);
         for (int t = 0; t < n_steps; t++) {
             const float2 a = decode_action(discrete, a_next);
             if (t + 1 < n_steps) a_next = load_action_raw(discrete, actions, (int64_t)(t + 1) * B + ii);
-            if (t - (int)taken_seen >= kRing && !wait_flag<SG_PILOT_SLEEP>(&taken[pair], (uint32_t)(t - kRing + 1), &taken_seen)) { *status = 1; break; }
+            if (t - (int)taken_seen >= kRingN && !wait_flag<SG_PILOT_SLEEP>(&taken[pair], (uint32_t)(t - kRingN + 1), &taken_seen)) { *status = 1; break; }
             if (head + 64u - tail_seen > (uint32_t)kReplayCap) tail_seen = lds_flag_load_uniform(&rp_tail[pair]);
             const bool defer = hand_over && head + 64u - tail_seen <= (uint32_t)kReplayCap;
 
-            const int slot = t % kRing;
+            const int slot = t % kRingN;
             StepResult r;
             int rk;
             {
                 Integ I;
                 SG_ACC(0);
-                goal_env_begin<N, ACCEL>(kc, e, a.x, a.y, I);
+                goal_env_begin<N, ACCEL>(kc, e, hs, hc, a.x, a.y, I);
                 SG_ACC(1);
                 rk = I.run(r, [&]() __attribute__((always_inline)) -> bool { return defer; });
                 SG_ACC_ADD(7, __any(r.done) ? 1 : 0);
@@ -84,15 +87,16 @@
             }
             e.x = (float)((double)e.x + r.dXd); e.y = (float)((double)e.y + r.dYd); e.vx = r.vx; e.vy = r.vy; e.om = r.om;
             e.th = wrap_two_pi(e.th + r.dth);
+            sincos_acc(e.th, hs, hc);
             SG_ACC(3);
             SG_ACC(4);
             {
-                float *q = ring + (slot * kHand) * kBlock + tid;
+                float *q = ring + (slot * kRollHand) * kBlock + tid;
                 const uint64_t ux = __double_as_longlong(r.dXd), uy = __double_as_longlong(r.dYd);
                 q[0 * kBlock] = __uint_as_float((uint32_t)ux); q[1 * kBlock] = __uint_as_float((uint32_t)(ux >> 32));
                 q[2 * kBlock] = __uint_as_float((uint32_t)uy); q[3 * kBlock] = __uint_as_float((uint32_t)(uy >> 32));
-                q[4 * kBlock] = e.th; q[5 * kBlock] = e.vx; q[6 * kBlock] = e.vy; q[7 * kBlock] = e.om;
-                q[8 * kBlock] = __uint_as_float((uint32_t)r.done | (replayed ? 2u | (rslot << 8) : 0u));
+                q[4 * kBlock] = hc; q[5 * kBlock] = hs; q[6 * kBlock] = e.vx; q[7 * kBlock] = e.vy; q[8 * kBlock] = e.om;
+                q[9 * kBlock] = __uint_as_float((uint32_t)r.done | (replayed ? 2u | (rslot << 8) : 0u));
             }
             lds_flag_store(&handed[pair], (uint32_t)(t + 1));
             SG_ACC(5);
@@ -106,6 +110,7 @@
                     const float *q = spare + ((int)(k % (uint32_t)kSpare) * Spare::kFields) * kBlock + tid;
                     e.x = q[0 * kBlock]; e.y = q[1 * kBlock]; e.th = q[2 * kBlock]; e.vx = q[3 * kBlock];
                     e.vy = q[4 * kBlock]; e.om = q[5 * kBlock];
+                    hs = q[Spare::kSin * kBlock]; hc = q[Spare::kCos * kBlock];
 #pragma unroll
                     for (int j = 0; j < N; j++) { e.px[j] = q[(8 + 2 * j) * kBlock]; e.py[j] = q[(9 + 2 * j) * kBlock]; }
                 } else {
@@ -115,6 +120,7 @@
                     float gx, gy;
                     goal_reset<N>(c, c.env_index_base + (uint32_t)i, T, s, e.px, e.py, gx, gy);
                     e.x = s.x; e.y = s.y; e.th = s.th; e.vx = s.vx; e.vy = s.vy; e.om = s.om;
+                    sincos_acc(e.th, hs, hc);
                 }
                 ct = make_uint2(0u, k);
             }
@@ -210,17 +216,17 @@
         if (!wait_flag(&handed[pair], (uint32_t)(t + 1))) { *status = 2; break; }
         SG_ACC(1);
         double dXd, dYd;
-        float th, vx, vy, om;
+        float hc, hs, vx, vy, om;
         int dn;
         bool replayed;
         {
-            const int slot = t % kRing;
-            const float *q = ring + (slot * kHand) * kBlock + tid;
+            const int slot = t % kRingN;
+            const float *q = ring + (slot * kRollHand) * kBlock + tid;
             const uint64_t ux = (uint64_t)__float_as_uint(q[0 * kBlock]) | ((uint64_t)__float_as_uint(q[1 * kBlock]) << 32);
             const uint64_t uy = (uint64_t)__float_as_uint(q[2 * kBlock]) | ((uint64_t)__float_as_uint(q[3 * kBlock]) << 32);
             dXd = __longlong_as_double((long long)ux); dYd = __longlong_as_double((long long)uy);
-            th = q[4 * kBlock]; vx = q[5 * kBlock]; vy = q[6 * kBlock]; om = q[7 * kBlock];
-            const uint32_t w8 = __float_as_uint(q[8 * kBlock]);
+            hc = q[4 * kBlock]; hs = q[5 * kBlock]; vx = q[6 * kBlock]; vy = q[7 * kBlock]; om = q[8 * kBlock];
+            const uint32_t w8 = __float_as_uint(q[9 * kBlock]);
             dn = (int)(w8 & 1u);
             replayed = (w8 & 2u) != 0u;
             if (replayed) Replay::put_goal(rb, w8 >> 8, e.gx, e.gy);
@@ -232,7 +238,7 @@
         int hit;
         r = goal_reward<N>(fc, e.x, e.y, dXd, dYd, e.px, e.py, e.gx, e.gy, hit);
         count_hits(cnt, live && hit && !replayed);
-        e.x = (float)((double)e.x + dXd); e.y = (float)((double)e.y + dYd); e.vx = vx; e.vy = vy; e.om = om; e.th = th;
+        e.x = (float)((double)e.x + dXd); e.y = (float)((double)e.y + dYd); e.vx = vx; e.vy = vy; e.om = om;
         const uint32_t el = ct.x + 1u;
         const int trunc = !dn && (int)el >= max_steps;
         const int fin = dn | trunc;
@@ -241,7 +247,7 @@
         SG_ACC(4);
         if constexpr (TOBS) {
             if (__any(restart && !replayed)) {
-                goal_observe<N>(fc, e, o);
+                goal_observe<N>(fc, e, hs, hc, o);
                 term_append<D>(tl, restart && !replayed, t, i, o);
             }
         }
@@ -250,10 +256,10 @@
         SG_ACC(6);
         if (restart) {
             ct = make_uint2(0u, ct.y + 1u);
-            Spare::get(spare, (int)(ct.y % (uint32_t)kSpare), tid, e, aux, cs);
+            Spare::get(spare, (int)(ct.y % (uint32_t)kSpare), tid, e, aux, cs, hs, hc);
         }
         SG_ACC(12);
-        goal_observe<N>(fc, e, o);
+        goal_observe<N>(fc, e, hs, hc, o);
         SG_ACC(13);
         if (live) {
 #pragma unroll
diff --git a/space_gym_amd/csrc/sg_kepler_pair_rollout.inc b/space_gym_amd/csrc/sg_kepler_pair_rollout.inc
--- a/space_gym_amd/csrc/sg_kepler_pair_rollout.inc
+++ b/space_gym_amd/csrc/sg_kepler_pair_rollout.inc
@@ -1,7 +1,7 @@
 
     using Integ = Integrator<2, 1, false, ACCEL>;
     __shared__ float spare[kSpare * kKeplerSpareFields * kBlock];
-    __shared__ float ring[kRing * kHand * kBlock];
+    __shared__ float ring[kRing * kRollHand * kBlock];
     __shared__ float rbuf[(kBlock / 64) * kKeplerReplayWords * kReplayCap];
     __shared__ uint32_t spare_hi[kBlock];
     __shared__ uint32_t handed[kBlock / 64], taken[kBlock / 64];
@@ -36,6 +36,8 @@
         float2 a_next = load_action_raw(discrete, actions, ii);
         uint32_t taken_seen = 0u;
         uint32_t head = 0u, tail_seen = 0u;
+        float hs, hc;
+        sincos_acc(e.th, hs, hc);
         for (int t = 0; t < n_steps; t++) {
             const float2 a_raw = decode_action(discrete, a_next);
             float a0 = a_raw.x, a1 = a_raw.y;
@@ -54,7 +56,7 @@
                 const float cax[2] = {0.0f, 0.0f}, cay[2] = {0.0f, 0.0f}, cR[2] = {kc.planet_r, border_r};
                 const double cRd[2] = {kc.planet_r_d, (double)border_r};
                 Integ I;
-                I.begin(kc.h, kc.half_world, kc.gm, F, om0, alpha, kc.omega_limit, e.x, e.y, e.th, e.vx, e.vy, cax, cay, cR, cRd);
+                I.begin(kc.h, kc.half_world, kc.gm, F, om0, alpha, kc.omega_limit, e.x, e.y, e.th, hs, hc, e.vx, e.vy, cax, cay, cR, cRd);
                 rk = I.run(r, [&]() __attribute__((always_inline)) -> bool { return defer; });
             }
             const bool replayed = rk == kRkEventDeferred;
@@ -76,13 +78,14 @@
             }
             e.x = (float)((double)e.x + r.dXd); e.y = (float)((double)e.y + r.dYd); e.vx = r.vx; e.vy = r.vy; e.om = r.om;
             e.th = wrap_two_pi(e.th + r.dth);
+            sincos_acc(e.th, hs, hc);
             {
-                float *q = ring + (slot * kHand) * kBlock + tid;
+                float *q = ring + (slot * kRollHand) * kBlock + tid;
                 const uint64_t ux = __double_as_longlong(r.dXd), uy = __double_as_longlong(r.dYd);
                 q[0 * kBlock] = __uint_as_float((uint32_t)ux); q[1 * kBlock] = __uint_as_float((uint32_t)(ux >> 32));
                 q[2 * kBlock] = __uint_as_float((uint32_t)uy); q[3 * kBlock] = __uint_as_float((uint32_t)(uy >> 32));
-                q[4 * kBlock] = e.th; q[5 * kBlock] = e.vx; q[6 * kBlock] = e.vy; q[7 * kBlock] = e.om;
-                q[8 * kBlock] = __uint_as_float((uint32_t)r.done | (replayed ? 2u : 0u));
+                q[4 * kBlock] = hc; q[5 * kBlock] = hs; q[6 * kBlock] = e.vx; q[7 * kBlock] = e.vy; q[8 * kBlock] = e.om;
+                q[9 * kBlock] = __uint_as_float((uint32_t)r.done | (replayed ? 2u : 0u));
             }
             lds_flag_store(&handed[pair], (uint32_t)(t + 1));
             const uint32_t el = ct.x + 1u;
@@ -95,6 +98,7 @@
                     const float *q = spare + ((int)(k % (uint32_t)kSpare) * kKeplerSpareFields) * kBlock + tid;
                     e.x = q[0 * kBlock]; e.y = q[1 * kBlock]; e.th = q[2 * kBlock]; e.vx = q[3 * kBlock];
                     e.vy = q[4 * kBlock]; e.om = q[5 * kBlock];
+                    hs = q[12 * kBlock]; hc = q[13 * kBlock];
                     if (rnd_orbit) {
                         e.phi = q[6 * kBlock]; e.ecc = q[7 * kBlock];
                         const uint64_t uc = (uint64_t)__float_as_uint(q[8 * kBlock]) | ((uint64_t)__float_as_uint(q[9 * kBlock]) << 32);
@@ -106,6 +110,7 @@
                     kepler_reset(c, c.env_index_base + (uint32_t)i, k, s, e.phi, e.ecc);
                     e.x = s.x; e.y = s.y; e.th = s.th; e.vx = s.vx; e.vy = s.vy; e.om = s.om;
                     if (rnd_orbit) orb = make_double2(cos((double)e.phi), sin((double)e.phi));
+                    sincos_acc(e.th, hs, hc);
                 }
                 ct = make_uint2(0u, k);
             }
@@ -161,6 +166,9 @@
                 q[8 * kBlock] = __uint_as_float((uint32_t)uc); q[9 * kBlock] = __uint_as_float((uint32_t)(uc >> 32));
                 q[10 * kBlock] = __uint_as_float((uint32_t)us); q[11 * kBlock] = __uint_as_float((uint32_t)(us >> 32));
             }
+            float sn, co;
+            sincos_acc(s.th, sn, co);
+            q[12 * kBlock] = sn; q[13 * kBlock] = co;
             hi += 1u;
             lds_flag_store(&spare_hi[tid], hi);
         }
@@ -174,17 +182,17 @@
         load_action(discrete, actions, (int64_t)t * B + ii, a0, a1);
         if (!wait_flag(&handed[pair], (uint32_t)(t + 1))) { *status = 2; break; }
         double dXd, dYd;
-        float th, vx, vy, om;
+        float hc, hs, vx, vy, om;
         int dn;
         bool replayed;
         {
             const int slot = t % kRing;
-            const float *q = ring + (slot * kHand) * kBlock + tid;
+            const float *q = ring + (slot * kRollHand) * kBlock + tid;
             const uint64_t ux = (uint64_t)__float_as_uint(q[0 * kBlock]) | ((uint64_t)__float_as_uint(q[1 * kBlock]) << 32);
             const uint64_t uy = (uint64_t)__float_as_uint(q[2 * kBlock]) | ((uint64_t)__float_as_uint(q[3 * kBlock]) << 32);
             dXd = __longlong_as_double((long long)ux); dYd = __longlong_as_double((long long)uy);
-            th = q[4 * kBlock]; vx = q[5 * kBlock]; vy = q[6 * kBlock]; om = q[7 * kBlock];
-            const uint32_t w8 = __float_as_uint(q[8 * kBlock]);
+            hc = q[4 * kBlock]; hs = q[5 * kBlock]; vx = q[6 * kBlock]; vy = q[7 * kBlock]; om = q[8 * kBlock];
+            const uint32_t w8 = __float_as_uint(q[9 * kBlock]);
             dn = (int)(w8 & 1u);
             replayed = (w8 & 2u) != 0u;
             complete += (uint32_t)__popcll(__ballot(replayed));
@@ -195,7 +203,7 @@
         Orbit ob = ob_fixed;
         if (rnd_orbit) ob = make_orbit(fc.k_a, (double)e.ecc, orb.x, orb.y);
         const float r = kepler_reward(fc, ob, e.x, e.y, dXd, dYd, vx, vy, engine, a1);
-        e.x = (float)((double)e.x + dXd); e.y = (float)((double)e.y + dYd); e.vx = vx; e.vy = vy; e.om = om; e.th = th;
+        e.x = (float)((double)e.x + dXd); e.y = (float)((double)e.y + dYd); e.vx = vx; e.vy = vy; e.om = om;
         const uint32_t el = ct.x + 1u;
         const int trunc = !dn && (int)el >= max_steps;
         const int fin = dn | trunc;
@@ -203,7 +211,7 @@
         ct.x = el;
         if (tl.count && __any(restart && !replayed)) {
             float ot[10];
-            kepler_observe(fc, e, ot);
+            kepler_observe(fc, e, hs, hc, ot);
             term_append<10>(tl, restart && !replayed, t, i, ot);
         }
         if (auto_reset && __any(live && hi - ct.y < (restart ? kKeep + 1u : kKeep))) refill();
@@ -212,6 +220,7 @@
             const float *q = spare + ((int)(ct.y % (uint32_t)kSpare) * kKeplerSpareFields) * kBlock + tid;
             e.x = q[0 * kBlock]; e.y = q[1 * kBlock]; e.th = q[2 * kBlock]; e.vx = q[3 * kBlock]; e.vy = q[4 * kBlock];
             e.om = q[5 * kBlock]; e.phi = q[6 * kBlock]; e.ecc = q[7 * kBlock];
+            hs = q[12 * kBlock]; hc = q[13 * kBlock];
             if (rnd_orbit) {
                 const uint64_t uc = (uint64_t)__float_as_uint(q[8 * kBlock]) | ((uint64_t)__float_as_uint(q[9 * kBlock]) << 32);
                 const uint64_t us = (uint64_t)__float_as_uint(q[10 * kBlock]) | ((uint64_t)__float_as_uint(q[11 * kBlock]) << 32);
@@ -219,7 +228,7 @@
             }
         }
         float o[10];
-        kepler_observe(fc, e, o);
+        kepler_observe(fc, e, hs, hc, o);
         if (live) {
             const int64_t row = (int64_t)t * B + i;
             store_row(obs, row, o);
```
